# jurgisp/pydreamer

Hardware: AMD Instinct MI355X
Metric: grad-steps/sec (world-model+AC) at B=50,T=50,H=15, 64×64 obs, 1/2/4/8 GPU (higher is better)
Workload: dtype f32

## Files before the change

pydreamer_amd/csrc/common.h:

```cpp
#pragma once
#include <hip/hip_runtime.h>
#include <stdint.h>
#include <stddef.h>
#include "dreamer_hip.h"

int dm_fail(int code, const char* fmt, ...);

#define DM_MAX_DEVICES 16

#ifndef DM_CHAIN_SETPRIO
#define DM_CHAIN_SETPRIO 0
#endif
#define DM_CHAIN_PRIO() do { if (DM_CHAIN_SETPRIO > 0) __builtin_amdgcn_s_setprio(DM_CHAIN_SETPRIO); } while (0)
#define DM_LAUNCH_CHECK()                                                                      \
  do {                                                                                         \
    hipError_t e__ = hipGetLastError();                                                        \
    if (e__ != hipSuccess) return dm_fail(DM_E_HIP, "%s:%d: %s", __FILE__, __LINE__, hipGetErrorString(e__)); \
  } while (0)

#define DM_TRY(expr)                 \
  do {                               \
    int rc__ = (expr);               \
    if (rc__ != DM_OK) return rc__;  \
  } while (0)

#define DM_REQUIRE(cond, code, ...)                     \
  do {                                                  \
    if (!(cond)) return dm_fail(code, __VA_ARGS__);     \
  } while (0)

static inline int dm_cdiv(int64_t a, int64_t b) { return (int)((a + b - 1) / b); }
static inline size_t dm_align_up(size_t x, size_t a) { return (x + a - 1) / a * a; }

struct DmArena {
  float* base;
  size_t cap;
  size_t off;
  bool ok;
  DmArena(void* p, size_t bytes) : base((float*)p), cap(bytes / sizeof(float)), off(0), ok(true) {}
  float* take(size_t nfloats) {
    size_t n = dm_align_up(nfloats, 64);
    if (base == nullptr || off + n > cap) { ok = false; off += n; return nullptr; }
    float* r = base + off;
    off += n;
    return r;
  }
};

hipStream_t dm_wgrad_side_stream(hipStream_t st);
int dm_wgrad_side_fork(hipStream_t st, hipStream_t sw);
int dm_wgrad_side_mark(hipStream_t sw, hipStream_t st);

int dm_cur_precision();
struct DmPrecisionScope {
  int prev;
  explicit DmPrecisionScope(int p);
  ~DmPrecisionScope();
};

struct DmTwinScope {
  bool active, opened;
  explicit DmTwinScope(bool bf16_mode);
  ~DmTwinScope();
};
bool dm_twins_on();
void dm_twin_add(const float* base, size_t n, unsigned short* twin, bool valid);
void dm_twin_mark(const float* p);
unsigned short* dm_twin_of(const float* p, bool need_valid);
void dm_twin_arena_note(const void* acts, bool written);
bool dm_twin_arena_valid(const void* acts);
struct DmCvtSeg { const float* src; unsigned short* dst; size_t n; };
int dm_to_bf16_multi_launch(const DmCvtSeg* segs, int count, hipStream_t st);
static inline size_t dm_half_floats(size_t elems) { return (elems + 1) / 2; }
constexpr int DM_HSTORE_MIN_K = 1024;
constexpr int DM_HSTORE_MIN_K_DENSE = 400;

struct DmGatesBwd;
struct DmGemm {
  int bf16 = dm_cur_precision();
  int a_layout = 0, b_layout = 0;
  int M = 0, N = 0, K = 0;
  const float* A = nullptr; int lda = 0;
  const float* B = nullptr; int ldb = 0;
  float* C = nullptr; int ldc = 0;
  const float* bias = nullptr;
  const float* add = nullptr; int ldadd = 0;
  const float* mulref = nullptr; int ldmul = 0;
  const uint8_t* row_zero = nullptr;
  const int* a_maj = nullptr; const int* a_min = nullptr; int a_tab_vec = 0;
  const int* b_maj = nullptr; const int* b_min = nullptr; int b_tab_vec = 0;
  int a_tab_vec8 = 0, b_tab_vec8 = 0;
  int flags = 0;
  const int2* c_tab = nullptr; int sc_cout = 0, sc_wpitch = 0;
  int bias_mod = 0;
  const float* ln_g = nullptr; const float* ln_b = nullptr; float ln_eps = 1e-3f;
  const float* lnb_x = nullptr; int lnb_ldx = 0; const float* lnb_stats = nullptr;
  const float* eg_x = nullptr; int eg_ldx = 0; const float* eg_stats = nullptr; const float* eg_gamma = nullptr; const float* eg_beta = nullptr;
  float* eg_G = nullptr; int eg_ldg = 0; float* eg_Gf = nullptr; float* eg_ps = nullptr;
  const float* lnf_ps = nullptr; int lnf_nps = 0; const float* lnf_stats = nullptr;
  const float* lnf_xw = nullptr; int lnf_ldxw = 0; const float* lnf_cs = nullptr;
  const float* sm_logits = nullptr; int sm_ld = 0; float* sm_dlogits = nullptr; int sm_ldd = 0;
  const struct DmGatesBwd* gates = nullptr;
  const float* A_frag = nullptr;
  float* C_frag = nullptr;
  const unsigned short* A_h = nullptr;
  const unsigned short* B_h = nullptr;
  unsigned short* C_h = nullptr;
  bool no_twin = false;
};
__host__ __device__ __forceinline__ size_t dm_frag_off(int row, int k) {
  return ((((size_t)(k >> 4) * 4 + (row >> 4)) * 4 + ((k >> 2) & 3)) * 16 + (row & 15)) * 4 + (k & 3);
}
static inline size_t dm_frag_floats(int K) { return (size_t)dm_cdiv(K, 16) * 1024; }
int dm_frag_pack_launch(int rows, int K, const float* X, int ldx, float* Xf, hipStream_t st);
struct DmRssmLds {
  int B, D, Hd, S, C, F, t_begin, t_end;
  const float *wzt, *zb, *wih, *bih, *whh, *bhh, *wph, *bph, *wpo, *bpo, *in_g, *in_b, *post_g, *post_b, *ea, *ee;
  const uint8_t* reset; const float* u; const int32_t* forced;
  float *x1, *gi, *gh, *hin, *zin, *feat, *x2, *post; int32_t* idx;
  float* ws; size_t ws_floats;
};
bool dm_rssm_lds_ok(int B, int D, int Hd, int S, int C);
size_t dm_rssm_lds_ws_floats(int B, int D, int Hd, int S, int C, int steps);
int dm_rssm_lds_launch(const DmRssmLds& q, hipStream_t st);
extern "C" int dm_rssm_lds_enable(int on);
bool dm_z_embed_ok(int n);
int dm_sparse_rows_launch(int rows, int n, int Zc, const float* z, int ldz, const float* Wt, float* x, int ldx,
                          hipStream_t st);
int dm_z_embed_launch(int rows, int n, int S, int C, const int32_t* idx, const uint8_t* row_zero, const float* Wt,
                      const float* bias, const float* add, int ldadd, const int32_t* idx2, const float* Wt2, float* x, int ldx,
                      float* x_frag, const float* gamma, const float* beta, float eps, float* y, int ldy, hipStream_t st,
                      float* y_frag = nullptr, float* stats = nullptr);
struct DmGatesBwd {
  const float* gi; const float* gh; const float* h_in; int ldh, D;
  float* dgi; float* dgh; float* dprev; int ldp; const uint8_t* row_zero;
  float* dgi_frag = nullptr; float* dgh_frag = nullptr;
};
struct DmSample {
  const float* u = nullptr; const int32_t* forced = nullptr;
  float* onehot = nullptr; int ldo = 0;
  int32_t* idx = nullptr;
  float* z_next = nullptr; const uint8_t* next_reset = nullptr;
  float* z_next_frag = nullptr;
};
bool dm_skinny_ln_ok(int M, int N, int K);
int dm_gemm_sample_launch(const DmGemm& q, const DmSample& sm, hipStream_t stream);
int dm_gemm_launch(const DmGemm& g, void* ws, size_t ws_bytes, hipStream_t stream);
int dm_gemm_skinny_try(const DmGemm& g, hipStream_t stream);
int dm_gemm_pair_launch(const DmGemm& g0, const DmGemm& g1, void* ws, size_t ws_bytes, hipStream_t stream);

int dm_colsum_launch(int rows, int n, const float* x, int ld, float* out, void* ws, size_t ws_bytes, hipStream_t st);
int dm_elu_fwd_launch(int rows, int n, const float* x, int ldx, float* y, int ldy, hipStream_t st);
int dm_elu_bwd_launch(int rows, int n, const float* y, int ldy, const float* dy, int lddy, float* dx, int lddx,
                      hipStream_t st);
int dm_ln_elu_fwd_launch(int rows, int n, const float* x, int ldx, const float* gamma, const float* beta, float eps,
                         float* y, int ldy, float* stats, hipStream_t st);
int dm_ln_elu_bwd_dx_launch(int rows, int n, const float* x, int ldx, const float* y, int ldy, const float* stats,
                            const float* gamma, const float* dy, int lddy, float* dx, int lddx, hipStream_t st);
int dm_ln_elu_bwd_params_launch(int rows, int n, const float* x, int ldx, const float* y, int ldy, const float* stats,
                                const float* dy, int lddy, float* dgamma, float* dbeta, void* ws, size_t ws_bytes,
                                hipStream_t st);
int dm_gru_norm_fwd_launch(int kind, int rows, int D, const float* gi, const float* gh, const float* h_in, int ldh,
                           const float* const* ln_g, const float* const* ln_b, float* h_out, int ldo, float* gs, float* gst,
                           float* h_next, const uint8_t* next_reset, hipStream_t st, int ldg = 0, int ldst = 0, int ldn = 0);
int dm_gru_norm_bwd_launch(int kind, int rows, int D, const float* gh, const float* h_in, int ldh, const float* gs,
                           const float* gst, const float* const* ln_g, const float* const* ln_b, const float* dh_out, int lddh,
                           float* dgi, float* dgh, float* dg, float* dh_in, int lddi, const uint8_t* row_zero, hipStream_t st,
                           int ldg = 0, int ldst = 0);
int dm_gru_norm_param_grads_launch(int kind, int rows, int D, const float* gs, const float* gst, const float* dg, float* dgam,
                                   float* dbet, hipStream_t st, int ldg = 0, int ldst = 0);
int dm_gru_gates_fwd_launch(int rows, int D, const float* gi, const float* gh, const float* h_in, int ldh, float* h_out,
                            int ldo, float* h_next, const uint8_t* next_reset, float* h_frag, float* h_next_frag,
                            hipStream_t st, int ldg = 0, int ldn = 0);
int dm_gru_gates_bwd_launch(int rows, int D, const float* gi, const float* gh, const float* h_in, int ldh,
                            const float* dh_out, int lddh, float* dgi, float* dgh, float* dh_in, int lddi, int accum,
                            const uint8_t* row_zero, hipStream_t st, int ldg = 0);
int dm_sample_onehot_launch(int rows, int groups, int C, const float* logits, int ldl, const float* u,
                            const int32_t* forced, float* onehot, int ldo, int32_t* idx, float* z_next,
                            const uint8_t* next_reset, hipStream_t st);
int dm_gauss_sample_bwd_launch(int rows, int S, const float* par, int ldp, const float* z, int ldz, const float* dz,
                               int lddz, float* dpar, int lddp, int accum, hipStream_t st);
int dm_kl_fwd_launch(int rows, int S, int C, const float* post, const float* prior, float* kl, float* ep, float* eq,
                     hipStream_t st);
int dm_kl_bwd_launch(int rows, int S, int C, const float* post, const float* prior, float sp, float sq, float* dpost,
                     float* dprior, hipStream_t st);
int dm_st_softmax_bwd_launch(int rows, int groups, int C, const float* logits, int ldl, const float* dz, int lddz,
                             float* dlogits, int lddl, int accum, hipStream_t st);
int dm_mask_rows_launch(int rows, int n, const float* x, int ldx, const uint8_t* reset, float* y, int ldy, hipStream_t st);
int dm_mask_rows2_launch(int rows, int n1, const float* x1, int ldx1, float* y1, int ldy1, int n2, const float* x2,
                         int ldx2, float* y2, int ldy2, const uint8_t* reset, hipStream_t st);
int dm_sample_continuous_launch(int kind, int rows, int A, const float* params, const float* eps, float* action,
                                hipStream_t st);
int dm_mul_elu_grad_launch(size_t n, const float* dy, const float* yact, float* out, hipStream_t st);

int dm_im2col_s2_launch(int n, int hb, int wb, int c, int k, const float* big, int big_nchw, float* col, hipStream_t st);
int dm_col2im_s2_launch(int n, int hb, int wb, int c, int k, const float* col, const float* bias, int flags,
                        const float* elu_ref, float* big, hipStream_t st);
int dm_permute4_launch(const float* src, float* dst, int d0, int d1, int d2, int d3, int p0, int p1, int p2, int p3,
                       hipStream_t st);

bool dm_enc_l1_direct_ok(int ch, int d, int img);
int dm_enc_l1_fwd_launch(int frames, int d, int u8, const void* image, const float* w, const float* bias, float* wt, float* y,
                         unsigned short* y_h, hipStream_t st);
size_t dm_enc_l1_wgrad_part_floats(int frames, int d);
int dm_enc_l1_wgrad_launch(int frames, int d, int u8, const void* image, const float* G, float* part, float* dW, void* ws,
                           size_t ws_bytes, hipStream_t st);
bool dm_dec_l4_direct_ok(int ch, int d, int hs, int k);
size_t dm_dec_l4_w4_floats(int d);
int dm_dec_l4_fwd_launch(int frames, int d, const float* x, const float* w, const float* bias, float* w4, float* out,
                         hipStream_t st);
bool dm_dec_l4_bwd_direct_ok(int ch, int d, int hs, int k);
size_t dm_dec_l4_wp_floats(int d);
size_t dm_dec_l4_wgrad_part_floats(int frames, int d);
int dm_dec_l4_dgrad_launch(int frames, int d, const float* G4, const float* w, float* wp, const float* x3, float* dx,
                           unsigned short* dx_h, hipStream_t st);
int dm_dec_l4_wgrad_launch(int frames, int d, const float* G4, const float* x3, float* part, float* dW, void* ws,
                           size_t ws_bytes, hipStream_t st);

struct DmChainSample {
  const float* u;
  float* onehot;
  int ldo;
  int32_t* idx;
};
int dm_mlp_fwd_launch(int rows, int in_dim, int hidden, int layers, int out_dim, const float* x, int ldx,
                      const dm_mlp_params* p, float* acts, int acts_total_rows, int acts_row_off, float* out, int ldout,
                      void* ws, size_t ws_bytes, hipStream_t st, const float* chain_wpack = nullptr, int sparse_cols = 0,
                      const float* chain_add0 = nullptr, const DmChainSample* chain_sample = nullptr);

bool dm_panel_ok(int rows, int hidden);
int dm_panel_count(int rows);
int dm_panel_ln_fwd_launch(int rows, int hidden, int kin, const float* x, int ldx, const float* W, const float* b,
                           const float* gamma, const float* beta, float eps, float* xpre, float* stats, float* y,
                           const float* wout, const float* bout, float* out, int out_dim, int ldout, hipStream_t st,
// ... 51 lines not shown
```

pydreamer_amd/csrc/conv.hip:

```cpp
#include "common.h"
#include <stdlib.h>

template <int VEC>
__global__ void __launch_bounds__(256) im2col_s2_nhwc_kernel(int n, int hb, int wb, int c, int k, int hs, int ws,
                                                             const float* __restrict__ big, float* __restrict__ col) {
  const int cv = c / VEC;
  const size_t total = (size_t)n * hs * ws * k * k * cv;
  for (size_t e = (size_t)blockIdx.x * 256 + threadIdx.x; e < total; e += (size_t)gridDim.x * 256) {
    size_t t = e;
    const int c4 = (int)(t % cv); t /= cv;
    const int kx = (int)(t % k); t /= k;
    const int ky = (int)(t % k); t /= k;
    const int xs = (int)(t % ws); t /= ws;
    const int ys = (int)(t % hs); t /= hs;
    const int i = (int)t;
    const size_t src = (((size_t)i * hb + (2 * ys + ky)) * wb + (2 * xs + kx)) * c + (size_t)c4 * VEC;
    if constexpr (VEC == 4) {
      reinterpret_cast<float4*>(col)[e] = *reinterpret_cast<const float4*>(big + src);
    } else {
      col[e] = big[src];
    }
  }
}

// ... 457 lines not shown
        hipLaunchKernelGGL(im2col_s2_u8hwc_kernel, dim3(grid_for(total)), dim3(256), 0, st, g.N, g.hb[0], g.hb[0], g.cin[0], 4,
                           g.hs[0], g.hs[0], (const uint8_t*)image, a.xcol[0]);
        DM_LAUNCH_CHECK();
      } else {
        DM_TRY(dm_im2col_s2_launch(g.N, g.hb[0], g.hb[0], g.cin[0], 4, image, 1, a.xcol[0], st));
      }
    }
    DmGemm q;
    q.a_layout = 0; q.b_layout = 0;
    q.M = g.N * g.hs[l] * g.hs[l]; q.N = g.cout[l]; q.K = (int)g.kdim[l];
    if (l == 0) { q.A = a.xcol[0]; q.lda = q.K; }
    else {
      q.A = a.y[l - 1]; q.a_maj = a.rowoff[l]; q.a_min = a.koff[l];
      q.a_tab_vec = (g.cin[l] & 3) == 0; q.a_tab_vec8 = (g.cin[l] & 7) == 0;
    }
    q.B = l == 0 ? p->w[0] : a.wr[l]; q.ldb = q.K;
    q.C = a.y[l]; q.ldc = q.N;
    q.bias = p->b[l];
    q.flags = DM_GEMM_ELU;
    DM_TRY(dm_gemm_launch(q, ws, DM_SPLITK_FLOATS * sizeof(float), st));
  }
  const size_t tot = (size_t)g.N * 4 * g.cout[3];
  hipLaunchKernelGGL(nhwc_to_chw_flat_kernel, dim3(grid_for(tot)), dim3(256), 0, st, (size_t)g.N, 4, g.cout[3], a.y[3], embed, 1);
  DM_LAUNCH_CHECK();
  return DM_OK;
}

extern "C" int dm_conv_encoder_bwd(const dm_shape* shp, const float* image, const dm_conv_params* p, const float* acts,
                                   const float* dembed, const dm_conv_grads* gr, void* ws, size_t ws_bytes, void* stream) {
  DM_REQUIRE(shp && p && acts && dembed && gr && ws, DM_E_NULL, "conv_encoder_bwd: null pointer");
  DmPrecisionScope prec(shp->flags & DM_FLAG_BF16);
  EncGeom g(shp);
  DM_REQUIRE(g.valid(shp), DM_E_SHAPE, "conv_encoder: unsupported geometry");
  hipStream_t st = (hipStream_t)stream;
  EncActs a;
  enc_carve(g, const_cast<float*>(acts), (size_t)1 << 60, &a);
  DmArena ar(ws, ws_bytes);
  float* splitk = ar.take(DM_SPLITK_FLOATS);
  const size_t gmax = g.rows[0] * g.cout[0];
  float* ga = ar.take(gmax);
  float* gb = ar.take(g.rows[1] * g.cout[1]);
  float* dwr = ar.take((size_t)g.cout[3] * g.kdim[3]);
  size_t xcmax = 0;
  for (int l = 1; l < 4; ++l) if (g.rows[l] * g.kdim[l] > xcmax) xcmax = g.rows[l] * g.kdim[l];
  float* dxcol = ar.take(xcmax);
  size_t padmax = 0, tabmax = 0, wcmax = 0;
  for (int l = 1; l < 4; ++l)
    if (convt_gather_ok(4, g.cout[l], g.cin[l], g.hs[l], (size_t)g.N)) {
      const size_t hp = g.hs[l] + 2, Hc = g.hs[l] + 1;
      if ((size_t)g.N * hp * hp * g.cout[l] > padmax) padmax = (size_t)g.N * hp * hp * g.cout[l];
      if ((size_t)g.N * Hc * Hc > tabmax) tabmax = (size_t)g.N * Hc * Hc;
      if ((size_t)16 * g.cin[l] * g.cout[l] > wcmax) wcmax = (size_t)16 * g.cin[l] * g.cout[l];
    }
  float* gpad = ar.take(padmax);
  int* t_rowoff = (int*)ar.take(tabmax);
  int2* t_ctab = (int2*)ar.take(2 * tabmax);
  int* t_koff = (int*)ar.take(wcmax ? 4 * 1024 : 0);
  float* wcat = ar.take(wcmax);
  DmTwinScope tw((shp->flags & DM_FLAG_BF16) != 0);
  const bool tw_on = dm_twins_on();
  unsigned short* ga_h = (unsigned short*)ar.take(tw_on ? dm_half_floats(gmax) : 0);
  unsigned short* gb_h = (unsigned short*)ar.take(tw_on ? dm_half_floats(g.rows[1] * g.cout[1]) : 0);
  unsigned short* wcat_h = (unsigned short*)ar.take(tw_on ? dm_half_floats(wcmax) : 0);
  DM_REQUIRE(ar.ok, DM_E_WORKSPACE, "conv_encoder_bwd: workspace too small (need %zu floats)", ar.off);
  const size_t skb = DM_SPLITK_FLOATS * sizeof(float);
  const bool arena_tw = dm_twin_arena_valid(acts);
  enc_register_twins(g, a, arena_tw, arena_tw);
  dm_twin_add(ga, gmax, ga_h, false);
  dm_twin_add(gb, g.rows[1] * g.cout[1], gb_h, false);

  float* G = gb;
  const size_t tot3 = (size_t)g.N * 4 * g.cout[3];
  hipLaunchKernelGGL(nhwc_to_chw_flat_kernel, dim3(grid_for(tot3)), dim3(256), 0, st, (size_t)g.N, 4, g.cout[3], dembed, G,
                     0);
  DM_LAUNCH_CHECK();
  DM_TRY(dm_mul_elu_grad_launch(tot3, G, a.y[3], G, st));
  if (tw_on) {
    const DmCvtSeg sg = {G, dm_twin_of(G, false), tot3};
    DM_TRY(dm_to_bf16_multi_launch(&sg, 1, st));
    dm_twin_mark(G);
  }
  for (int l = 3; l >= 0; --l) {
    const int rows = (int)g.rows[l], co = g.cout[l], kd = (int)g.kdim[l];
    DM_TRY(dm_colsum_launch(rows, co, G, co, gr->b[l], splitk, skb, st));
    if (l == 0 && g.direct0) {
      DM_REQUIRE(image, DM_E_NULL, "conv_encoder_bwd: the direct layer-1 weight gradient reads the image");
      DM_REQUIRE(dm_enc_l1_wgrad_part_floats(g.N, g.d) <= xcmax, DM_E_WORKSPACE, "conv_encoder_bwd: partial buffer too small");
      DM_TRY(dm_enc_l1_wgrad_launch(g.N, g.d, shape_u8(shp) ? 1 : 0, image, G, dxcol, gr->w[0], splitk, skb, st));
      continue;
    }
    DmGemm q;
    q.a_layout = 1; q.b_layout = 1;
    q.M = co; q.N = kd; q.K = rows;
    q.A = G; q.lda = co;
    if (l == 0) { q.B = a.xcol[0]; q.ldb = kd; }
    else {
      q.B = a.y[l - 1]; q.b_maj = a.rowoff[l]; q.b_min = a.koff[l];
      q.b_tab_vec = (g.cin[l] & 3) == 0; q.b_tab_vec8 = (g.cin[l] & 7) == 0;
    }
    q.C = (l == 0) ? gr->w[0] : dwr; q.ldc = kd;
    DM_TRY(dm_gemm_launch(q, splitk, skb, st));
    if (l > 0 && convt_gather_ok(4, co, g.cin[l], g.hs[l], (size_t)g.N)) {
      DM_TRY(dm_permute4_launch(dwr, gr->w[l], co, 4, 4, g.cin[l], 0, 3, 1, 2, st));
      const int hs = g.hs[l], hb = g.hb[l], Hc = hs + 1, kdim4 = 4 * co, ci = g.cin[l];
      DM_REQUIRE(kdim4 <= 4 * 1024, DM_E_SHAPE, "conv_encoder_bwd: gather-form K %d exceeds the offset table", kdim4);
      float* Gn = (G == ga) ? gb : ga;
      if (l == 1) Gn = ga;
      const size_t padn = (size_t)g.N * (hs + 2) * (hs + 2) * (co / 4);
      const bool hpath = tw_on && (co & 7) == 0 && kdim4 >= DM_HSTORE_MIN_K;
      if (hpath) hipLaunchKernelGGL(convt_pad_h_kernel, dim3(grid_for(padn)), dim3(256), 0, st, g.N, hs, hs, co / 4, 1, (const float4*)G,
                                    (uint2*)gpad);
      else hipLaunchKernelGGL(convt_pad_kernel, dim3(grid_for(padn)), dim3(256), 0, st, g.N, hs, hs, co / 4, 1, (const float4*)G,
                              (float4*)gpad);
      DM_LAUNCH_CHECK();
      hipLaunchKernelGGL(convt_tables_kernel, dim3(grid_for((size_t)g.N * Hc * Hc + kdim4)), dim3(256), 0, st, g.N, hs, hs, co, 2,
                         hb, hb, ci, t_rowoff, t_koff, t_ctab);
      DM_LAUNCH_CHECK();
      hipLaunchKernelGGL(convt_repack_kernel, dim3(grid_for((size_t)4 * ci * kdim4)), dim3(256), 0, st, co, ci, 4, p->w[l], wcat);
      DM_LAUNCH_CHECK();
      if (hpath) {
        const DmCvtSeg sg = {wcat, wcat_h, (size_t)4 * ci * kdim4};
        DM_TRY(dm_to_bf16_multi_launch(&sg, 1, st));
      }
      if (2 * Hc != hb) {
        hipError_t e = hipMemsetAsync(Gn, 0, (size_t)g.N * hb * hb * ci * sizeof(float), st);
        if (e == hipSuccess && dm_twin_of(Gn, false))
          e = hipMemsetAsync(dm_twin_of(Gn, false), 0, (size_t)g.N * hb * hb * ci * sizeof(unsigned short), st);
        if (e != hipSuccess) return dm_fail(DM_E_HIP, "conv_encoder_bwd: %s", hipGetErrorString(e));
      }
      DmGemm d;
      d.M = g.N * Hc * Hc; d.N = 4 * ci; d.K = kdim4;
      d.A = gpad; d.a_maj = t_rowoff; d.a_min = t_koff; d.a_tab_vec = 1; d.a_tab_vec8 = 1;
      if (hpath) { d.A = nullptr; d.A_h = (const unsigned short*)gpad; d.B_h = wcat_h; }
      d.B = wcat; d.ldb = kdim4;
      d.C = Gn;
      d.c_tab = t_ctab; d.sc_cout = ci; d.sc_wpitch = hb * ci;
      d.mulref = a.y[l - 1];
      d.no_twin = l == 1;
      DM_TRY(dm_gemm_launch(d, splitk, skb, st));
      G = Gn;
    } else if (l > 0) {
      DM_TRY(dm_permute4_launch(dwr, gr->w[l], co, 4, 4, g.cin[l], 0, 3, 1, 2, st));
      DmGemm d;
      d.a_layout = 0; d.b_layout = 1;
      d.M = rows; d.N = kd; d.K = co;
      d.A = G; d.lda = co;
      d.B = a.wr[l]; d.ldb = kd;
      d.C = dxcol; d.ldc = kd;
      DM_TRY(dm_gemm_launch(d, splitk, skb, st));
      float* Gn = (G == ga) ? gb : ga;
      if (l == 1) Gn = ga;
      DM_TRY(dm_col2im_s2_launch(g.N, g.hb[l], g.hb[l], g.cin[l], 4, dxcol, nullptr, 0, a.y[l - 1], Gn, st));
      G = Gn;
    }
  }
  return DM_OK;
}

__global__ void __launch_bounds__(256) convt_pad_cout_kernel(int I, int O, int O4, int k, const float* __restrict__ src,
                                                             float* __restrict__ dst) {
  const int total = I * k * k * O4;
  for (int e = blockIdx.x * 256 + threadIdx.x; e < total; e += gridDim.x * 256) {
    const int o = e % O4, kx = (e / O4) % k, ky = (e / (O4 * k)) % k, i = e / (O4 * k * k);
    dst[e] = o < O ? src[(((size_t)i * O + o) * k + ky) * k + kx] : 0.f;
  }
}
__global__ void __launch_bounds__(256) convt_unpad_cout_kernel(int I, int O, int O4, int k, const float* __restrict__ src,
                                                               float* __restrict__ dst) {
  const int total = I * O * k * k;
  for (int e = blockIdx.x * 256 + threadIdx.x; e < total; e += gridDim.x * 256) {
    const int kx = e % k, ky = (e / k) % k, o = (e / (k * k)) % O, i = e / (k * k * O);
    dst[e] = src[(((size_t)i * k + ky) * k + kx) * O4 + o];
  }
}

struct DecActs {
  float* wr[5];
// ... 236 lines not shown
  float* G = Gl[4];
  DM_TRY(mse_launch(shape_u8(shp), g.N, g.hbg[4] * g.hbg[4], g.ch, a.x[4], (const void*)target, shp->I > 0 ? shp->I : 1, scale,
                    row_scale, nullptr, G, co4[4], nullptr, st));
  for (int l = 4; l >= 1; --l) {
    const int kk = g.k[l] * g.k[l];
    const int co = co4[l];
    const bool padded = co != g.cout[l];
    const int ncol = kk * co;
    const int rows_s = (int)g.rows_s[l];
    int* rowoff = rowoff_l[l];
    int* koff = koff_l[l];
    float* Gn = Gl[l - 1];
    if (direct4 && l == 4) {
      DM_TRY(dm_wgrad_side_fork(st, sw));
      unsigned short* gnh = dm_twin_of(Gn, false);
      DM_TRY(dm_dec_l4_dgrad_launch(g.N, g.d, G, p->w[4], l4_wp, a.x[3], Gn, gnh, st));
      if (gnh) dm_twin_mark(Gn);
      DM_TRY(dm_colsum_launch((int)g.rows_b[l], co, G, co, bsum, splitk_w, skb, sw));
      hipError_t e = hipMemcpyAsync(gr->b[l], bsum, (size_t)g.cout[l] * sizeof(float), hipMemcpyDeviceToDevice, sw);
      if (e != hipSuccess) return dm_fail(DM_E_HIP, "conv_decoder_bwd: %s", hipGetErrorString(e));
      DM_TRY(dm_dec_l4_wgrad_launch(g.N, g.d, G, a.x[3], l4_part, gr->w[4], splitk_w, skb, sw));
      G = Gn;
      continue;
    }
    DM_TRY(conv_tables_launch(g.N, g.hbg[l], g.hbg[l], co, g.k[l], rowoff, koff, st));
    DM_TRY(dm_wgrad_side_fork(st, sw));
    if (padded) {
      hipLaunchKernelGGL(convt_pad_cout_kernel, dim3(grid_for((size_t)g.cin[l] * ncol)), dim3(256), 0, st, g.cin[l], g.cout[l], co,
                         g.k[l], p->w[l], wpad);
      DM_LAUNCH_CHECK();
      if (tw_on) {
        const DmCvtSeg sg = {wpad, wpad_h, (size_t)g.cin[l] * ncol};
        DM_TRY(dm_to_bf16_multi_launch(&sg, 1, st));
        dm_twin_mark(wpad);
      }
    }
    {
      DmGemm d;
      d.a_layout = 0; d.b_layout = 0;
      d.M = rows_s; d.N = g.cin[l]; d.K = ncol;
      d.A = G; d.a_maj = rowoff; d.a_min = koff; d.a_tab_vec = 1;
      d.a_tab_vec8 = (co & 7) == 0 || (co == 4 && (g.k[l] & 1) == 0);
      d.B = padded ? wpad : a.wr[l]; d.ldb = ncol;
      d.C = Gn; d.ldc = g.cin[l];
      if (l - 1 >= 1) { d.mulref = a.x[l - 1]; d.ldmul = g.cin[l]; }
      DM_TRY(dm_gemm_launch(d, splitk, skb, st));
    }
    if (padded) {
      DM_TRY(dm_colsum_launch((int)g.rows_b[l], co, G, co, bsum, splitk_w, skb, sw));
      hipError_t e = hipMemcpyAsync(gr->b[l], bsum, (size_t)g.cout[l] * sizeof(float), hipMemcpyDeviceToDevice, sw);
      if (e != hipSuccess) return dm_fail(DM_E_HIP, "conv_decoder_bwd: %s", hipGetErrorString(e));
    } else {
      DM_TRY(dm_colsum_launch((int)g.rows_b[l], co, G, co, gr->b[l], splitk_w, skb, sw));
    }
    DmGemm q;
    q.a_layout = 1; q.b_layout = 1;
    q.M = g.cin[l]; q.N = ncol; q.K = rows_s;
    q.A = a.x[l - 1]; q.lda = g.cin[l];
    q.B = G; q.b_maj = rowoff; q.b_min = koff; q.b_tab_vec = 1;
    q.b_tab_vec8 = (co & 7) == 0 || (co == 4 && (g.k[l] & 1) == 0);
    q.C = dwr; q.ldc = ncol;
    DM_TRY(dm_gemm_launch(q, splitk_w, skb, sw));
    if (padded) {
      hipLaunchKernelGGL(convt_unpad_cout_kernel, dim3(grid_for((size_t)g.cin[l] * kk * g.cout[l])), dim3(256), 0, sw, g.cin[l],
                         g.cout[l], co, g.k[l], dwr, gr->w[l]);
      DM_LAUNCH_CHECK();
    } else {
      DM_TRY(dm_permute4_launch(dwr, gr->w[l], g.cin[l], g.k[l], g.k[l], g.cout[l], 0, 3, 1, 2, sw));
    }
    G = Gn;
  }
  const int O = g.cin[1];
  DM_TRY(dm_wgrad_side_fork(st, sw));
  if (dfeat) {
    DmGemm d;
    d.a_layout = 0; d.b_layout = 1;
    d.M = g.N; d.N = g.F; d.K = O;
    d.A = G; d.lda = O;
    d.B = p->w[0]; d.ldb = g.F;
    d.C = dfeat; d.ldc = lddf;
    d.flags = DM_GEMM_ACCUM;
    DM_TRY(dm_gemm_launch(d, splitk, skb, st));
  }
  DM_TRY(dm_colsum_launch(g.N, O, G, O, gr->b[0], splitk_w, skb, sw));
  {
    DmGemm q;
    q.a_layout = 1; q.b_layout = 1;
    q.M = O; q.N = g.F; q.K = g.N;
    q.A = G; q.lda = O;
    q.B = feat; q.ldb = ldf;
    q.C = gr->w[0]; q.ldc = g.F;
    DM_TRY(dm_gemm_launch(q, splitk_w, skb, sw));
  }
  DM_TRY(dm_wgrad_side_mark(sw, st));
  return DM_OK;
}
```

pydreamer_amd/csrc/elementwise.hip:

```cpp
#include "common.h"

template <bool CACHE>
__global__ void __launch_bounds__(256) ln_elu_fwd_kernel(int rows, int n, const float* __restrict__ x, int ldx,
                                                         const float* __restrict__ gamma, const float* __restrict__ beta,
                                                         float eps, float* __restrict__ y, int ldy, float* __restrict__ stats,
                                                         unsigned short* __restrict__ y_h) {
  const int row = blockIdx.x * 4 + (threadIdx.x >> 6);
  const int lane = threadIdx.x & 63;
  if (row >= rows) return;
  const float* xr = x + (size_t)row * ldx;
  unsigned short* yh = y_h ? y_h + (size_t)row * ldy : nullptr;
  float xc[16];
  float s = 0.f;
  if (CACHE) {
#pragma unroll
    for (int j = 0; j < 16; ++j) {
      const int c = lane + 64 * j;
      xc[j] = c < n ? xr[c] : 0.f;
      s += xc[j];
    }
  } else {
    for (int c = lane; c < n; c += 64) s += xr[c];
  }
  const float mean = dm_wave_sum(s) / (float)n;
// ... 84 lines not shown
    for (int c = lane; c < n; c += 64) {
      const float g = dyr[c] * dm_elu_grad_from_y(yr[c]) * gamma[c];
      const float xh = (xr[c] - mean) * rstd;
      dxr[c] = rstd * (g - sg - xh * sgx);
    }
  }
}

template <int MODE>
__global__ void __launch_bounds__(256) colsum_partial_kernel(int rows, int n, int rows_per_chunk,
                                                             const float* __restrict__ x, int ldx,
                                                             const float* __restrict__ y, int ldy,
                                                             const float* __restrict__ stats,
                                                             const float* __restrict__ dy, int lddy,
                                                             float* __restrict__ partial) {
  __shared__ float red[2][4][64];
  const int cx = threadIdx.x & 63, ry = threadIdx.x >> 6;
  const int col = blockIdx.x * 64 + cx;
  const int chunk = blockIdx.y;
  const int r0 = chunk * rows_per_chunk;
  const int r1 = min(rows, r0 + rows_per_chunk);
  float a0 = 0.f, a1 = 0.f;
  if (col < n) {
    if (MODE == 0) {
      float b0 = 0.f, b1 = 0.f, b2 = 0.f, b3 = 0.f;
      int r = r0 + ry;
      for (; r + 12 < r1; r += 16) {
        b0 += x[(size_t)r * ldx + col];
        b1 += x[(size_t)(r + 4) * ldx + col];
        b2 += x[(size_t)(r + 8) * ldx + col];
        b3 += x[(size_t)(r + 12) * ldx + col];
      }
      for (; r < r1; r += 4) b0 += x[(size_t)r * ldx + col];
      a0 = (b0 + b1) + (b2 + b3);
    } else {
      for (int r = r0 + ry; r < r1; r += 4) {
        const float dl = dy[(size_t)r * lddy + col] * dm_elu_grad_from_y(y[(size_t)r * ldy + col]);
        const float xh = (x[(size_t)r * ldx + col] - stats[2 * r]) * stats[2 * r + 1];
        a0 += dl * xh;
        a1 += dl;
      }
    }
  }
  red[0][ry][cx] = a0;
  red[1][ry][cx] = a1;
  __syncthreads();
  if (ry == 0 && col < n) {
    const int nq = (MODE == 0) ? 1 : 2;
    float s0 = red[0][0][cx] + red[0][1][cx] + red[0][2][cx] + red[0][3][cx];
    partial[((size_t)chunk * nq + 0) * n + col] = s0;
    if (MODE == 1) {
      float s1 = red[1][0][cx] + red[1][1][cx] + red[1][2][cx] + red[1][3][cx];
      partial[((size_t)chunk * nq + 1) * n + col] = s1;
    }
  }
}

__global__ void __launch_bounds__(256) colsum_flat_kernel(long long total, int n, int W, long long chunk_elems,
                                                          const float* __restrict__ x, float* __restrict__ partial) {
  __shared__ float sh[256];
  const long long base = (long long)blockIdx.x * chunk_elems;
  const long long end = min(total, base + chunk_elems);
  float b0 = 0.f, b1 = 0.f, b2 = 0.f, b3 = 0.f;
  if ((int)threadIdx.x < W) {
    long long i = base + threadIdx.x;
    for (; i + 3LL * W < end; i += 4LL * W) {
      b0 += x[i];
      b1 += x[i + W];
      b2 += x[i + 2LL * W];
      b3 += x[i + 3LL * W];
    }
    for (; i < end; i += W) b0 += x[i];
  }
  sh[threadIdx.x] = (b0 + b1) + (b2 + b3);
  __syncthreads();
  if ((int)threadIdx.x < n) {
    float s = 0.f;
    for (int t = threadIdx.x; t < W; t += n) s += sh[t];
    partial[(size_t)blockIdx.x * n + threadIdx.x] = s;
  }
}

__global__ void __launch_bounds__(256) colsum_final_kernel(int n, int chunks, int nq, const float* __restrict__ partial,
                                                           float* __restrict__ out0, float* __restrict__ out1) {
  __shared__ float red[8][32];
  const int cx = threadIdx.x & 31, cy = threadIdx.x >> 5;
  const int col = blockIdx.x * 32 + cx;
  for (int q = 0; q < nq; ++q) {
    float s = 0.f;
    if (col < n) {
      const float* p = partial + (size_t)q * n + col;
      const size_t st = (size_t)nq * n;
      int c = cy;
      for (; c + 24 < chunks; c += 32) {
        const float v0 = p[(size_t)c * st], v1 = p[(size_t)(c + 8) * st], v2 = p[(size_t)(c + 16) * st], v3 = p[(size_t)(c + 24) * st];
        s += v0; s += v1; s += v2; s += v3;
      }
      for (; c < chunks; c += 8) s += p[(size_t)c * st];
    }
    red[cy][cx] = s;
    __syncthreads();
    if (cy == 0 && col < n) {
      float t = 0.f;
#pragma unroll
      for (int k = 0; k < 8; ++k) t += red[k][cx];
      (q == 0 ? out0 : out1)[col] = t;
    }
    __syncthreads();
  }
}

static int colsum_plan(int rows, size_t budget_floats, int n, int nq, int* rows_per_chunk) {
  int chunks = dm_cdiv(rows, 64);
  if (chunks > 1024) chunks = 1024;
  const size_t per = (size_t)n * nq;
  if (per > 0 && (size_t)chunks * per > budget_floats) chunks = (int)(budget_floats / per);
  if (chunks < 1) chunks = 1;
  *rows_per_chunk = dm_cdiv(rows, chunks);
  return dm_cdiv(rows, *rows_per_chunk);
}

int dm_colsum_launch(int rows, int n, const float* x, int ld, float* out, void* ws, size_t ws_bytes, hipStream_t st) {
  if (n <= 0) return DM_OK;
  if (rows <= 0) {
    (void)hipMemsetAsync(out, 0, (size_t)n * sizeof(float), st);
    return DM_OK;
  }
  DM_REQUIRE(ws && ws_bytes >= (size_t)n * sizeof(float), DM_E_WORKSPACE, "colsum: workspace too small");
  const size_t budget = ws_bytes / sizeof(float);
  int chunks;
  if (n <= 64 && ld == n && (long long)rows * n >= (1 << 16)) {
    const long long total = (long long)rows * n;
    const int W = 256 - 256 % n;
    long long want = total / ((long long)W * 16);
    if (want > 2048) want = 2048;
    if (want < 1) want = 1;
    if ((size_t)want * n > budget) want = (long long)(budget / n);
    long long chunk_elems = (total + want - 1) / want;
    chunk_elems = (chunk_elems + W - 1) / W * W;
    chunks = (int)((total + chunk_elems - 1) / chunk_elems);
    hipLaunchKernelGGL(colsum_flat_kernel, dim3(chunks), dim3(256), 0, st, total, n, W, chunk_elems, x, (float*)ws);
  } else {
    int rpc;
    chunks = colsum_plan(rows, budget, n, 1, &rpc);
    hipLaunchKernelGGL((colsum_partial_kernel<0>), dim3(dm_cdiv(n, 64), chunks), dim3(256), 0, st, rows, n, rpc, x, ld,
                       nullptr, 0, nullptr, nullptr, 0, (float*)ws);
  }
  DM_LAUNCH_CHECK();
  hipLaunchKernelGGL(colsum_final_kernel, dim3(dm_cdiv(n, 32)), dim3(256), 0, st, n, chunks, 1, (const float*)ws, out,
                     nullptr);
  DM_LAUNCH_CHECK();
  return DM_OK;
}

int dm_ln_elu_fwd_launch(int rows, int n, const float* x, int ldx, const float* gamma, const float* beta, float eps,
                         float* y, int ldy, float* stats, hipStream_t st) {
  if (rows <= 0) return DM_OK;
  unsigned short* y_h = dm_twin_of(y, false);
  if (y_h) dm_twin_mark(y);
  if (n <= 1024)
    hipLaunchKernelGGL((ln_elu_fwd_kernel<true>), dim3(dm_cdiv(rows, 4)), dim3(256), 0, st, rows, n, x, ldx, gamma, beta,
                       eps, y, ldy, stats, y_h);
  else
    hipLaunchKernelGGL((ln_elu_fwd_kernel<false>), dim3(dm_cdiv(rows, 4)), dim3(256), 0, st, rows, n, x, ldx, gamma, beta,
                       eps, y, ldy, stats, y_h);
  DM_LAUNCH_CHECK();
  return DM_OK;
}

__global__ void __launch_bounds__(256) elu_fwd_kernel(int rows, int n, const float* __restrict__ x, int ldx,
                                                      float* __restrict__ y, int ldy) {
  const size_t total = (size_t)rows * n;
  for (size_t i = (size_t)blockIdx.x * 256 + threadIdx.x; i < total; i += (size_t)gridDim.x * 256) {
    const size_t r = i / n, c = i % n;
    y[r * ldy + c] = dm_elu(x[r * ldx + c]);
  }
}
__global__ void __launch_bounds__(256) elu_bwd_kernel(int rows, int n, const float* __restrict__ y, int ldy,
                                                      const float* __restrict__ dy, int lddy, float* __restrict__ dx,
                                                      int lddx) {
  const size_t total = (size_t)rows * n;
  for (size_t i = (size_t)blockIdx.x * 256 + threadIdx.x; i < total; i += (size_t)gridDim.x * 256) {
    const size_t r = i / n, c = i % n;
    dx[r * lddx + c] = dy[r * lddy + c] * dm_elu_grad_from_y(y[r * ldy + c]);
  }
}
int dm_elu_fwd_launch(int rows, int n, const float* x, int ldx, float* y, int ldy, hipStream_t st) {
  if (rows <= 0) return DM_OK;
  const size_t total = (size_t)rows * n;
  hipLaunchKernelGGL(elu_fwd_kernel, dim3((unsigned)((total + 255) / 256 < 65536 ? (total + 255) / 256 : 65536)), dim3(256), 0,
                     st, rows, n, x, ldx, y, ldy);
  DM_LAUNCH_CHECK();
  return DM_OK;
}
int dm_elu_bwd_launch(int rows, int n, const float* y, int ldy, const float* dy, int lddy, float* dx, int lddx,
                      hipStream_t st) {
  if (rows <= 0) return DM_OK;
  const size_t total = (size_t)rows * n;
  hipLaunchKernelGGL(elu_bwd_kernel, dim3((unsigned)((total + 255) / 256 < 65536 ? (total + 255) / 256 : 65536)), dim3(256), 0,
                     st, rows, n, y, ldy, dy, lddy, dx, lddx);
  DM_LAUNCH_CHECK();
  return DM_OK;
}

int dm_ln_elu_bwd_dx_launch(int rows, int n, const float* x, int ldx, const float* y, int ldy, const float* stats,
                            const float* gamma, const float* dy, int lddy, float* dx, int lddx, hipStream_t st) {
  if (rows <= 0) return DM_OK;
  if (n <= 1024)
    hipLaunchKernelGGL((ln_elu_bwd_dx_kernel<true>), dim3(dm_cdiv(rows, 4)), dim3(256), 0, st, rows, n, x, ldx, y, ldy,
                       stats, gamma, dy, lddy, dx, lddx);
  else
    hipLaunchKernelGGL((ln_elu_bwd_dx_kernel<false>), dim3(dm_cdiv(rows, 4)), dim3(256), 0, st, rows, n, x, ldx, y, ldy,
                       stats, gamma, dy, lddy, dx, lddx);
  DM_LAUNCH_CHECK();
  return DM_OK;
}

int dm_ln_elu_bwd_params_launch(int rows, int n, const float* x, int ldx, const float* y, int ldy, const float* stats,
                                const float* dy, int lddy, float* dgamma, float* dbeta, void* ws, size_t ws_bytes,
                                hipStream_t st) {
  int rpc;
  DM_REQUIRE(ws && ws_bytes >= (size_t)2 * n * sizeof(float), DM_E_WORKSPACE, "ln_bwd: workspace too small");
  const int chunks = colsum_plan(rows, ws_bytes / sizeof(float), n, 2, &rpc);
  hipLaunchKernelGGL((colsum_partial_kernel<1>), dim3(dm_cdiv(n, 64), chunks), dim3(256), 0, st, rows, n, rpc, x, ldx, y,
                     ldy, stats, dy, lddy, (float*)ws);
  DM_LAUNCH_CHECK();
  hipLaunchKernelGGL(colsum_final_kernel, dim3(dm_cdiv(n, 32)), dim3(256), 0, st, n, chunks, 2, (const float*)ws, dgamma,
                     dbeta);
  DM_LAUNCH_CHECK();
  return DM_OK;
}

extern "C" int dm_ln_elu_fwd(int rows, int n, const float* x, int ldx, const float* gamma, const float* beta, float eps,
                             float* y, int ldy, float* stats, void* stream) {
  DM_REQUIRE(x && gamma && beta && y && stats, DM_E_NULL, "ln_elu_fwd: null pointer");
  return dm_ln_elu_fwd_launch(rows, n, x, ldx, gamma, beta, eps, y, ldy, stats, (hipStream_t)stream);
}

extern "C" int dm_ln_elu_bwd(int rows, int n, const float* x, int ldx, const float* y, int ldy, const float* stats,
                             const float* gamma, const float* dy, int lddy, float* dx, int lddx, float* dgamma,
                             float* dbeta, void* ws, size_t ws_bytes, void* stream) {
  DM_REQUIRE(x && y && stats && gamma && dy && dx && dgamma && dbeta, DM_E_NULL, "ln_elu_bwd: null pointer");
  DM_TRY(dm_ln_elu_bwd_dx_launch(rows, n, x, ldx, y, ldy, stats, gamma, dy, lddy, dx, lddx, (hipStream_t)stream));
  return dm_ln_elu_bwd_params_launch(rows, n, x, ldx, y, ldy, stats, dy, lddy, dgamma, dbeta, ws, ws_bytes,
                                     (hipStream_t)stream);
}

extern "C" int dm_colsum(int rows, int n, const float* x, int ld, float* out, void* ws, size_t ws_bytes, void* stream) {
  DM_REQUIRE(x && out, DM_E_NULL, "colsum: null pointer");
  return dm_colsum_launch(rows, n, x, ld, out, ws, ws_bytes, (hipStream_t)stream);
}

__device__ __forceinline__ float dm_sigmoid(float v) { return 1.0f / (1.0f + expf(-v)); }

__global__ void __launch_bounds__(256) gru_gates_fwd_kernel(int rows, int D, const float* __restrict__ gi,
                                                            const float* __restrict__ gh, const float* __restrict__ h_in,
                                                            int ldh, float* __restrict__ h_out, int ldo,
                                                            float* __restrict__ h_next,
                                                            const uint8_t* __restrict__ next_reset,
                                                            float* __restrict__ h_frag, float* __restrict__ h_next_frag,
                                                            int ldg, int ldn, unsigned short* __restrict__ h_out_h) {
  const size_t total = (size_t)rows * D;
  for (size_t i = (size_t)blockIdx.x * 256 + threadIdx.x; i < total; i += (size_t)gridDim.x * 256) {
    const int r = (int)(i / D), d = (int)(i % D);
    const float* gir = gi + (size_t)r * ldg;
    const float* ghr = gh + (size_t)r * ldg;
    const float rg = dm_sigmoid(gir[d] + ghr[d]);
    const float ug = dm_sigmoid(gir[D + d] + ghr[D + d]);
    const float ng = tanhf(gir[2 * D + d] + rg * ghr[2 * D + d]);
    const float h = h_in[(size_t)r * ldh + d];
    const float ho = (h - ng) * ug + ng;
    h_out[(size_t)r * ldo + d] = ho;
    if (h_out_h) h_out_h[(size_t)r * ldo + d] = (unsigned short)dm_f2bf(ho);
    const float hn = (next_reset && next_reset[r]) ? 0.f : ho;
    if (h_next) h_next[(size_t)r * ldn + d] = hn;
    if (h_frag) h_frag[dm_frag_off(r, d)] = ho;
    if (h_next_frag) h_next_frag[dm_frag_off(r, d)] = hn;
  }
}
__global__ void __launch_bounds__(256) frag_pack_kernel(int rows, int K, const float* __restrict__ X, int ldx,
                                                        float* __restrict__ Xf) {
  const int total = rows * K;
  for (int i = blockIdx.x * 256 + threadIdx.x; i < total; i += gridDim.x * 256) {
    const int r = i / K, k = i % K;
    Xf[dm_frag_off(r, k)] = X[(size_t)r * ldx + k];
  }
}

__global__ void __launch_bounds__(256) gru_gates_bwd_kernel(int rows, int D, const float* __restrict__ gi,
                                                            const float* __restrict__ gh, const float* __restrict__ h_in,
                                                            int ldh, const float* __restrict__ dh_out, int lddh,
                                                            float* __restrict__ dgi, float* __restrict__ dgh,
                                                            float* __restrict__ dh_in, int lddi, int accum,
                                                            const uint8_t* __restrict__ row_zero, int ldg) {
  const size_t total = (size_t)rows * D;
  for (size_t i = (size_t)blockIdx.x * 256 + threadIdx.x; i < total; i += (size_t)gridDim.x * 256) {
    const int r = (int)(i / D), d = (int)(i % D);
    const size_t g0 = (size_t)r * ldg;
    const float ghn = gh[g0 + 2 * D + d];
    const float rg = dm_sigmoid(gi[g0 + d] + gh[g0 + d]);
    const float ug = dm_sigmoid(gi[g0 + D + d] + gh[g0 + D + d]);
    const float ng = tanhf(gi[g0 + 2 * D + d] + rg * ghn);
    const float h = h_in[(size_t)r * ldh + d];
    const float dh = dh_out[(size_t)r * lddh + d];
    const float dn = dh * (1.f - ug);
    const float du = dh * (h - ng);
    const float dpn = dn * (1.f - ng * ng);
    const float dpr = dpn * ghn * rg * (1.f - rg);
    const float dpu = du * ug * (1.f - ug);
    dgi[g0 + d] = dpr;
    dgi[g0 + D + d] = dpu;
// ... 1566 lines not shown
```

pydreamer_amd/csrc/gemm.hip:

```cpp
#include "common.h"
#include "dma_loop.h"
#include <stdlib.h>
#include <math.h>
#include <type_traits>
#include <mutex>
#include <atomic>


struct GemmKArgs {
  const float* A;
  const float* B;
  float* C;
  const float* bias;
  const float* add;
  const float* mulref;
  const uint8_t* row_zero;
  const int* a_maj; const int* a_min;
  const int* b_maj; const int* b_min;
  float* partial;
  const int2* c_tab;
  int sc_cout, sc_wpitch;
  int bias_mod;
  int M, N, K;
  int lda, ldb, ldc, ldadd, ldmul;
  int flags;
  int k_per_split;
  int nsplit;
  int tiles_m;
  int n_tiles, n_items;
  int tiles_n, n_fast;
  int n_groups;
  int a_vec, b_vec;
  unsigned short* Ch;
  int use_dma;
};

template <int ROWS, int LAYOUT, int NF4, bool GATHER, bool VEC, bool KSEQ = false>
__device__ __forceinline__ void gemm_load_tile(float4 (&r)[NF4], const float* __restrict__ P, int ld, int row0,
                                               int nrows, int k0, int kend, const int* __restrict__ tmaj,
                                               const int* __restrict__ tmin, int tid, unsigned& mask) {
  mask = 0u;
#pragma unroll
  for (int i = 0; i < NF4; ++i) {
    const int f = tid + i * 256;
    int major, minor, major_end, minor_end;
    if (LAYOUT == 0) {
      major = row0 + (f >> 3);
      minor = k0 + ((f & 7) << 2);
      major_end = nrows;
      minor_end = kend;
    } else {
      constexpr int F4_PER_K = ROWS / 4;
      if (KSEQ) {
        major = k0 + (tid / F4_PER_K) * NF4 + i;
        minor = row0 + ((tid % F4_PER_K) << 2);
      } else {
        major = k0 + f / F4_PER_K;
        minor = row0 + ((f % F4_PER_K) << 2);
      }
      major_end = kend;
      minor_end = nrows;
    }
    const bool okm = major < major_end;
    const int mj = okm ? major : 0;
    float4 v;
    if (VEC) {
      const bool ok = okm && minor < minor_end;
      const int mn = ok ? minor : 0;
      const size_t off = GATHER ? (size_t)(tmaj[mj] + tmin[mn]) : (size_t)mj * ld + mn;
      v = *reinterpret_cast<const float4*>(P + (ok ? off : 0));
      mask |= ok ? (0xFu << (4 * i)) : 0u;
    } else {
      float e[4];
#pragma unroll
      for (int j = 0; j < 4; ++j) {
        const bool ok = okm && minor + j < minor_end;
        const int mn = ok ? minor + j : 0;
        const size_t off = GATHER ? (size_t)(tmaj[mj] + tmin[mn]) : (size_t)mj * ld + mn;
        e[j] = P[ok ? off : 0];
        mask |= ok ? (1u << (4 * i + j)) : 0u;
      }
      v = make_float4(e[0], e[1], e[2], e[3]);
    }
    r[i] = v;
  }
}

template <int ROWS, int LAYOUT, int NF4>
__device__ __forceinline__ void gemm_store_tile(const float4 (&rr)[NF4], unsigned mask, float* S, int tid) {
  constexpr int LDK = 36;
  constexpr int LDM = ROWS + 4;
  float4 r[NF4];
#pragma unroll
  for (int i = 0; i < NF4; ++i) {
    r[i].x = (mask >> (4 * i + 0)) & 1u ? rr[i].x : 0.f;
    r[i].y = (mask >> (4 * i + 1)) & 1u ? rr[i].y : 0.f;
    r[i].z = (mask >> (4 * i + 2)) & 1u ? rr[i].z : 0.f;
    r[i].w = (mask >> (4 * i + 3)) & 1u ? rr[i].w : 0.f;
  }
#pragma unroll
  for (int i = 0; i < NF4; ++i) {
    const int f = tid + i * 256;
    if (LAYOUT == 0) {
      const int row = f >> 3;
      const int kq = (f & 7) << 2;
      *reinterpret_cast<float4*>(&S[row * LDK + kq]) = r[i];
    } else {
      constexpr int F4_PER_K = ROWS / 4;
      const int kr = f / F4_PER_K;
      const int r4 = (f % F4_PER_K) << 2;
      *reinterpret_cast<float4*>(&S[kr * LDM + r4]) = r[i];
    }
  }
}

constexpr int LDKB = 40;
template <int ROWS, int LAYOUT, int NF4, bool KSEQ = false>
// ... 84 lines not shown
    it.n0 = fast * BN;
    it.m0 = slow * BM;
  } else {
    it.m0 = fast * BM;
    it.n0 = slow * BN;
  }
  it.kbeg = it.split * g.k_per_split;
  it.kend = min(g.K, it.kbeg + g.k_per_split);
  it.nkt = (it.kend > it.kbeg) ? (it.kend - it.kbeg + 31) / 32 : 0;
  return it;
}

constexpr int EPI_STAGE_LD = 40;
template <int BM, int BN, int WGM, int WGN, bool SC, int MB, int NB>
__device__ __forceinline__ void gemm_epilogue(f32x16 (&acc)[MB][NB], const GemmKArgs& g, const GemmItem& cur, int wm, int wn,
                                              int l31, int half, unsigned short* stage = nullptr) {
  const bool staged = !SC && stage && g.Ch && g.nsplit <= 1 && (g.ldc & 7) == 0 && (((uintptr_t)g.Ch) & 15) == 0;
#pragma unroll
  for (int mb = 0; mb < MB; ++mb) {
#pragma unroll
    for (int nb = 0; nb < NB; ++nb) {
      const int col = cur.n0 + wn * (BN / WGN) + nb * 32 + l31;
      int sc_off = 0, sc_need = 0, sc_o = 0;
      if (SC) {
        const int cls = col / g.sc_cout;
        sc_o = col - cls * g.sc_cout;
        sc_off = (cls >> 1) * g.sc_wpitch + (cls & 1) * g.sc_cout + sc_o;
        sc_need = cls;
      }
#pragma unroll
      for (int r = 0; r < 16; ++r) {
        const int row = cur.m0 + wm * (BM / WGM) + mb * 32 + (r & 3) + 8 * (r >> 2) + 4 * half;
        if (row < g.M && col < g.N) {
          float v = acc[mb][nb][r];
          if (SC) {
            const int2 ct = g.c_tab[row];
            if ((sc_need & ~ct.y) == 0) {
              const size_t at = (size_t)ct.x + sc_off;
              if (g.bias) v += g.bias[sc_o];
              if (g.flags & DM_GEMM_ELU) v = dm_elu(v);
              if (g.mulref) v *= dm_elu_grad_from_y(g.mulref[at]);
              g.C[at] = v;
              if (g.Ch) g.Ch[at] = (unsigned short)dm_f2bf(v);
            }
          } else if (g.nsplit > 1) {
            g.partial[((size_t)cur.split * g.M + row) * g.N + col] = v;
          } else {
            if (g.row_zero && g.row_zero[row]) v = 0.f;
            if (g.bias) v += g.bias[g.bias_mod > 0 ? col % g.bias_mod : col];
            if (g.add) v += g.add[(size_t)row * g.ldadd + col];
            float* c = g.C + (size_t)row * g.ldc + col;
            if (g.flags & DM_GEMM_ACCUM) v += *c;
            if (g.flags & DM_GEMM_ELU) v = dm_elu(v);
            if (g.mulref) v *= dm_elu_grad_from_y(g.mulref[(size_t)row * g.ldmul + col]);
            *c = v;
            if (staged) stage[((r & 3) + 8 * (r >> 2) + 4 * half) * EPI_STAGE_LD + l31] = (unsigned short)dm_f2bf(v);
            else if (g.Ch) g.Ch[(size_t)row * g.ldc + col] = (unsigned short)dm_f2bf(v);
          }
        }
      }
      if (staged) {
        __builtin_amdgcn_wave_barrier();
        const int lane = half * 32 + l31;
        const int rl = lane >> 1, c0 = (lane & 1) * 16;
        const int row = cur.m0 + wm * (BM / WGM) + mb * 32 + rl;
        const int colb = cur.n0 + wn * (BN / WGN) + nb * 32 + c0;
        if (row < g.M) {
#pragma unroll
          for (int h8 = 0; h8 < 2; ++h8) {
            const int cc = colb + h8 * 8;
            const unsigned short* sp = &stage[rl * EPI_STAGE_LD + c0 + h8 * 8];
            unsigned short* dp = g.Ch + (size_t)row * g.ldc + cc;
            if (cc + 8 <= g.N) *reinterpret_cast<uint4*>(dp) = *reinterpret_cast<const uint4*>(sp);
            else
              for (int j = 0; j < 8 && cc + j < g.N; ++j) dp[j] = sp[j];
          }
        }
        __builtin_amdgcn_wave_barrier();
      }
    }
  }
}

template <int BM, int BN, int AL, int BL, bool VEC, bool GA = false, bool GB = false, int WGM = 2, int WGN = 2,
          int BF = 0, bool SC = false>
__global__ void __launch_bounds__(256) gemm_f32_kernel(const GemmKArgs g) {
  static_assert(WGM * WGN == 4 && BM % (32 * WGM) == 0 && BN % (32 * WGN) == 0, "wave grid must tile the block tile");
  constexpr int BK = 32;
  constexpr int LDK = 36;
  constexpr int LDMA = BM + 4, LDMB = BN + 4;
  constexpr int A_FLOATS = (AL == 0) ? BM * LDK : BK * LDMA;
  constexpr int B_FLOATS = (BL == 0) ? BN * LDK : BK * LDMB;
  constexpr int MB = BM / (32 * WGM), NB = BN / (32 * WGN);
  constexpr int A_F4 = BM * BK / 4 / 256, B_F4 = BN * BK / 4 / 256;
  constexpr bool A_KSEQ = BF != 0 && AL == 1 && 256 % (BM / 4) == 0, B_KSEQ = BF != 0 && BL == 1 && 256 % (BN / 4) == 0;
  constexpr int SMEM_FLOATS = A_FLOATS + B_FLOATS;
  __shared__ __attribute__((aligned(16))) float smem[SMEM_FLOATS];
  float* As = smem;
  float* Bs = smem + A_FLOATS;

  const int tid = threadIdx.x;
  const int lane = tid & 63;
  const int wave = tid >> 6;
  const int half = lane >> 5;
  const int l31 = lane & 31;
  const int wm = wave / WGN, wn = wave % WGN;

  const GemmItem cur = gemm_decode<BM, BN>(g, blockIdx.x);

  f32x16 acc[MB][NB];
#pragma unroll
  for (int i = 0; i < MB; ++i)
#pragma unroll
    for (int j = 0; j < NB; ++j)
#pragma unroll
      for (int r = 0; r < 16; ++r) acc[i][j][r] = 0.f;

  float4 ra[A_F4], rb[B_F4];
  unsigned ma = 0u, mb_ = 0u;
  if (cur.nkt > 0) {
    gemm_load_tile<BM, AL, A_F4, GA, VEC, A_KSEQ>(ra, g.A, g.lda, cur.m0, g.M, cur.kbeg, cur.kend, g.a_maj, g.a_min, tid, ma);
    gemm_load_tile<BN, BL, B_F4, GB, VEC, B_KSEQ>(rb, g.B, g.ldb, cur.n0, g.N, cur.kbeg, cur.kend, g.b_maj, g.b_min, tid, mb_);
  }
  for (int kt = 0; kt < cur.nkt; ++kt) {
    unsigned short* Ah = reinterpret_cast<unsigned short*>(smem);
    unsigned short* Bh = Ah + BM * LDKB;
    if (BF == 1) {
      gemm_store_tile_bf16<BM, AL, A_F4, A_KSEQ>(ra, ma, Ah, tid);
      gemm_store_tile_bf16<BN, BL, B_F4, B_KSEQ>(rb, mb_, Bh, tid);
    } else {
      gemm_store_tile<BM, AL, A_F4>(ra, ma, As, tid);
      gemm_store_tile<BN, BL, B_F4>(rb, mb_, Bs, tid);
    }
    __syncthreads();
    if (kt + 1 < cur.nkt) {
      const int k0 = cur.kbeg + (kt + 1) * BK;
      gemm_load_tile<BM, AL, A_F4, GA, VEC, A_KSEQ>(ra, g.A, g.lda, cur.m0, g.M, k0, cur.kend, g.a_maj, g.a_min, tid, ma);
      gemm_load_tile<BN, BL, B_F4, GB, VEC, B_KSEQ>(rb, g.B, g.ldb, cur.n0, g.N, k0, cur.kend, g.b_maj, g.b_min, tid, mb_);
    }
    __builtin_amdgcn_sched_barrier(0);
    if (BF == 1) {
#pragma unroll
      for (int ks = 0; ks < 2; ++ks) {
        bf16x8 a8[MB], b8[NB];
#pragma unroll
        for (int mb = 0; mb < MB; ++mb)
          a8[mb] = *reinterpret_cast<const bf16x8*>(&Ah[(wm * (BM / WGM) + mb * 32 + l31) * LDKB + ks * 16 + half * 8]);
#pragma unroll
        for (int nb = 0; nb < NB; ++nb)
          b8[nb] = *reinterpret_cast<const bf16x8*>(&Bh[(wn * (BN / WGN) + nb * 32 + l31) * LDKB + ks * 16 + half * 8]);
#pragma unroll
        for (int mb = 0; mb < MB; ++mb)
#pragma unroll
          for (int nb = 0; nb < NB; ++nb)
            acc[mb][nb] = __builtin_amdgcn_mfma_f32_32x32x16_bf16(a8[mb], b8[nb], acc[mb][nb], 0, 0, 0);
      }
    } else
#pragma unroll
    for (int kg = 0; kg < 4; ++kg) {
      float a[MB][4], b[NB][4];
#pragma unroll
      for (int mb = 0; mb < MB; ++mb) {
        const int row = wm * (BM / WGM) + mb * 32 + l31;
        if (AL == 0) {
          const float4 t = *reinterpret_cast<const float4*>(&As[row * LDK + kg * 8 + half * 4]);
          a[mb][0] = t.x; a[mb][1] = t.y; a[mb][2] = t.z; a[mb][3] = t.w;
        } else {
#pragma unroll
          for (int j = 0; j < 4; ++j) a[mb][j] = As[(kg * 8 + half * 4 + j) * LDMA + row];
        }
      }
#pragma unroll
      for (int nb = 0; nb < NB; ++nb) {
        const int row = wn * (BN / WGN) + nb * 32 + l31;
        if (BL == 0) {
          const float4 t = *reinterpret_cast<const float4*>(&Bs[row * LDK + kg * 8 + half * 4]);
          b[nb][0] = t.x; b[nb][1] = t.y; b[nb][2] = t.z; b[nb][3] = t.w;
        } else {
#pragma unroll
          for (int j = 0; j < 4; ++j) b[nb][j] = Bs[(kg * 8 + half * 4 + j) * LDMB + row];
        }
      }
#pragma unroll
      for (int j = 0; j < 4; ++j)
#pragma unroll
        for (int mb = 0; mb < MB; ++mb)
#pragma unroll
          for (int nb = 0; nb < NB; ++nb)
            acc[mb][nb] = __builtin_amdgcn_mfma_f32_32x32x2f32(a[mb][j], b[nb][j], acc[mb][nb], 0, 0, 0);
    }
    __syncthreads();
  }

  gemm_epilogue<BM, BN, WGM, WGN, SC, MB, NB>(acc, g, cur, wm, wn, l31, half,
                                              reinterpret_cast<unsigned short*>(smem) + wave * 32 * EPI_STAGE_LD);
}

template <int BM, int BN, int AL, int BL, bool GA, bool GB, int WGM, int WGN, bool SC, int NS>
__global__ void __launch_bounds__(256) gemm_dma_kernel(const GemmKArgs g) {
  static_assert(WGM * WGN == 4 && BM % (32 * WGM) == 0 && BN % (32 * WGN) == 0, "wave grid must tile the block tile");
  static_assert(NS >= 2 && NS <= 3, "two or three LDS stages");
  constexpr int WM = BM / WGM, WN = BN / WGN;
  constexpr int MB = WM / 32, NB = WN / 32;
  constexpr int A_BYTES = BM * 128, B_BYTES = BN * 128, STAGE = A_BYTES + B_BYTES;
  constexpr int RD = MB * DmaFrag<AL>::READS + NB * DmaFrag<BL>::READS;
  static_assert(RD <= 15, "lgkmcnt is a 4-bit counter");
  static_assert((AL == 0 || (MB - 1) * 32 + BM <= 255) && (BL == 0 || (NB - 1) * 32 + BN <= 255), "ds_read2_b32 offsets are 8 bits");
  extern __shared__ __attribute__((aligned(1024))) unsigned char dma_smem[];
  const unsigned lds0 = (unsigned)(size_t)(__attribute__((address_space(3))) unsigned char*)dma_smem;

  const int tid = threadIdx.x;
  const int lane = tid & 63, wave = tid >> 6, half = lane >> 5, l31 = lane & 31;
  const int wm = wave / WGN, wn = wave % WGN;
  const GemmItem cur = gemm_decode<BM, BN>(g, blockIdx.x);

  f32x16 acc[MB][NB];
#pragma unroll
  for (int i = 0; i < MB; ++i)
#pragma unroll
    for (int j = 0; j < NB; ++j)
#pragma unroll
      for (int r = 0; r < 16; ++r) acc[i][j][r] = 0.f;

  if (cur.nkt > 0) {
    DmaOperand<BM, AL, GA> sa;
    DmaOperand<BN, BL, GB> sb;
    sa.init(g.A, g.lda, cur.m0, g.M, g.a_maj, g.a_min, wave, lane);
    sb.init(g.B, g.ldb, cur.n0, g.N, g.b_maj, g.b_min, wave, lane);
    constexpr int NPT = DmaOperand<BM, AL, GA>::NP + DmaOperand<BN, BL, GB>::NP;

    const int swz = (l31 >> 1) & 7;
    unsigned fa[4], fb[4];
#pragma unroll
    for (int kg = 0; kg < 4; ++kg) {
      fa[kg] = AL == 0 ? lds0 + (wm * WM + l31) * 128 + (((2 * kg + half) ^ swz) << 4)
                       : lds0 + (((8 * kg + 4 * half) * BM + wm * WM + l31) << 2);
      fb[kg] = BL == 0 ? lds0 + A_BYTES + (wn * WN + l31) * 128 + (((2 * kg + half) ^ swz) << 4)
                       : lds0 + A_BYTES + (((8 * kg + 4 * half) * BN + wn * WN + l31) << 2);
    }
    auto read_frags = [&](DmaFrag<AL> (&a)[MB], DmaFrag<BL> (&b)[NB], int kg, unsigned so) {
#pragma unroll
      for (int mb = 0; mb < MB; ++mb) {
        if constexpr (AL == 0) {
          asm volatile("ds_read_b128 %0, %1 offset:%2" : "=v"(a[mb].v) : "v"(fa[kg] + so), "n"(mb * 32 * 128));
        } else {
          asm volatile("ds_read2_b32 %0, %1 offset0:%2 offset1:%3" : "=v"(a[mb].lo) : "v"(fa[kg] + so), "n"(mb * 32), "n"(mb * 32 + BM));
          asm volatile("ds_read2_b32 %0, %1 offset0:%2 offset1:%3" : "=v"(a[mb].hi) : "v"(fa[kg] + so + 8 * BM), "n"(mb * 32), "n"(mb * 32 + BM));
        }
      }
#pragma unroll
      for (int nb = 0; nb < NB; ++nb) {
        if constexpr (BL == 0) {
          asm volatile("ds_read_b128 %0, %1 offset:%2" : "=v"(b[nb].v) : "v"(fb[kg] + so), "n"(nb * 32 * 128));
        } else {
          asm volatile("ds_read2_b32 %0, %1 offset0:%2 offset1:%3" : "=v"(b[nb].lo) : "v"(fb[kg] + so), "n"(nb * 32), "n"(nb * 32 + BN));
          asm volatile("ds_read2_b32 %0, %1 offset0:%2 offset1:%3" : "=v"(b[nb].hi) : "v"(fb[kg] + so + 8 * BN), "n"(nb * 32), "n"(nb * 32 + BN));
        }
      }
    };

    static_assert(!(GA || GB) || NS == 2, "gathered operands take the two-stage ring");
    sa.fetch_tab(cur.kbeg, cur.kend);
    sb.fetch_tab(cur.kbeg, cur.kend);
#pragma unroll
    for (int s = 0; s < NS - 1; ++s) {
      if (s < cur.nkt) {
        sa.issue(cur.kbeg + s * 32, cur.kend, dma_smem + s * STAGE, wave);
        sb.issue(cur.kbeg + s * 32, cur.kend, dma_smem + s * STAGE + A_BYTES, wave);
      }
    }
    sa.fetch_tab(cur.kbeg + 32, cur.kend);
    sb.fetch_tab(cur.kbeg + 32, cur.kend);

    int stage = 0;
    for (int kt = 0; kt < cur.nkt; ++kt) {
      if (NS == 3 && kt + 1 < cur.nkt) dma_wait_vm<NPT>();
      else dma_wait_vm<0>();
      __builtin_amdgcn_s_barrier();
      const unsigned so = (unsigned)stage * STAGE;
      DmaFrag<AL> a[2][MB];
      DmaFrag<BL> b[2][NB];
      read_frags(a[0], b[0], 0, so);
      const int nt = kt + NS - 1;
      int ns = stage + NS - 1;
      if (ns >= NS) ns -= NS;
      if (nt < cur.nkt) {
        sa.issue(cur.kbeg + nt * 32, cur.kend, dma_smem + ns * STAGE, wave);
        sb.issue(cur.kbeg + nt * 32, cur.kend, dma_smem + ns * STAGE + A_BYTES, wave);
      }
#pragma unroll
      for (int kg = 0; kg < 4; ++kg) {
        const int c = kg & 1, n = c ^ 1;
        if (kg < 3) {
          read_frags(a[n], b[n], kg + 1, so);
          dma_wait_lgkm<RD>();
        } else dma_wait_lgkm<0>();
        __builtin_amdgcn_sched_barrier(0);
#pragma unroll
        for (int j = 0; j < 4; ++j)
#pragma unroll
          for (int mb = 0; mb < MB; ++mb)
#pragma unroll
            for (int nb = 0; nb < NB; ++nb)
              acc[mb][nb] = __builtin_amdgcn_mfma_f32_32x32x2f32(a[c][mb].get(j), b[c][nb].get(j), acc[mb][nb], 0, 0, 0);
        __builtin_amdgcn_sched_barrier(0);
      }
      if ((GA || GB) && nt + 1 < cur.nkt) {
        sa.fetch_tab(cur.kbeg + (nt + 1) * 32, cur.kend);
        sb.fetch_tab(cur.kbeg + (nt + 1) * 32, cur.kend);
      }
      if (++stage == NS) stage = 0;
    }
  }
  unsigned short* stg = nullptr;
  if (g.Ch) {
    __syncthreads();
    stg = reinterpret_cast<unsigned short*>(dma_smem) + wave * 32 * EPI_STAGE_LD;
  }
  gemm_epilogue<BM, BN, WGM, WGN, SC, MB, NB>(acc, g, cur, wm, wn, l31, half, stg);
}

template <int ROWS, int LAYOUT, int NF4, bool GATHER, bool KSEQ>
struct PipeOperand {
  const float* P;
  const int* tvar;
  int ld;
  int off[NF4];
  int kin[NF4];
  __device__ __forceinline__ void init(const float* P_, int ld_, int row0, int nrows, const int* tmaj, const int* tmin, int tid) {
    P = P_; ld = ld_;
    tvar = LAYOUT == 0 ? tmin : tmaj;
#pragma unroll
    for (int i = 0; i < NF4; ++i) {
      const int f = tid + i * 256;
      if (LAYOUT == 0) {
        const int row = min(row0 + (f >> 3), nrows - 1);
        kin[i] = (f & 7) << 2;
        off[i] = GATHER ? tmaj[row] : row * ld + kin[i];
      } else {
        constexpr int F4_PER_K = ROWS / 4;
        kin[i] = KSEQ ? (tid / F4_PER_K) * NF4 + i : f / F4_PER_K;
        const int col = min(row0 + (((KSEQ ? tid : f) % F4_PER_K) << 2), nrows - 4);
        off[i] = GATHER ? tmin[col] : kin[i] * ld + col;
      }
    }
  }
  __device__ __forceinline__ void load(float4 (&r)[NF4], int k0, int kend) const {
#pragma unroll
    for (int i = 0; i < NF4; ++i) {
      const bool ok = k0 + kin[i] < kend;
      size_t at;
      if (LAYOUT == 0) at = GATHER ? (size_t)off[i] + (size_t)tvar[ok ? k0 + kin[i] : 0] : (size_t)off[i] + (size_t)k0;
      else at = GATHER ? (size_t)off[i] + (size_t)tvar[ok ? k0 + kin[i] : 0] : (size_t)k0 * ld + (size_t)off[i];
      typedef float f32x4n __attribute__((ext_vector_type(4)));
      typedef const __attribute__((address_space(1))) f32x4n* gptr4;
      const uintptr_t src = ok ? (uintptr_t)(P + at) : (uintptr_t)dm_zero_page;
      const f32x4n v = *reinterpret_cast<gptr4>(src);
      r[i] = make_float4(v.x, v.y, v.z, v.w);
    }
  }
};

template <int ROWS, int LAYOUT, int NF4, bool KSEQ>
struct PipeStash {
  static constexpr bool ROWWISE = LAYOUT == 1 && KSEQ;
  static constexpr int UNITS = ROWWISE ? (NF4 == 4 ? 8 : 4) : 2 * NF4;
  static __device__ __forceinline__ float comp(const float4& v, int j) { return j == 0 ? v.x : j == 1 ? v.y : j == 2 ? v.z : v.w; }
  static __device__ __forceinline__ unsigned pack(float x, float y) { return dm_pack_bf16x2(x, y); }
  static __device__ __forceinline__ void unit(const float4 (&rr)[NF4], int u, unsigned short* S, int tid, unsigned& hold) {
    if (ROWWISE) {
      static_assert(!ROWWISE || NF4 == 4 || NF4 == 2, "row-wise packing covers 64- and 128-row operands");
      constexpr int F4_PER_K = ROWS / 4;
      const int kq = (tid / F4_PER_K) * NF4, r4 = (tid % F4_PER_K) << 2;
      if (NF4 == 4) {
        const int j = u >> 1;
        if ((u & 1) == 0) { hold = pack(comp(rr[0], j), comp(rr[1], j)); return; }
        const unsigned q = pack(comp(rr[NF4 > 2 ? 2 : 0], j), comp(rr[NF4 - 1], j));
        unsigned short* d = &S[(r4 + j) * LDKB + kq];
        *reinterpret_cast<uint2*>(d) = make_uint2(hold, q);
      } else {
        const unsigned q = pack(comp(rr[0], u), comp(rr[NF4 - 1], u));
        unsigned short* d = &S[(r4 + u) * LDKB + kq];
        *reinterpret_cast<unsigned*>(d) = q;
      }
      return;
    }
    const int i = u >> 1, f = tid + i * 256;
    if (LAYOUT == 0) {
      if ((u & 1) == 0) { hold = pack(rr[i].x, rr[i].y); return; }
      const unsigned q = pack(rr[i].z, rr[i].w);
      unsigned short* d = &S[(f >> 3) * LDKB + ((f & 7) << 2)];
      *reinterpret_cast<uint2*>(d) = make_uint2(hold, q);
    } else {
      constexpr int F4_PER_K = ROWS / 4;
      const int kr = f / F4_PER_K, r4 = ((f % F4_PER_K) << 2) + 2 * (u & 1);
      const unsigned q = (u & 1) ? pack(rr[i].z, rr[i].w) : pack(rr[i].x, rr[i].y);
// ... 201 lines not shown
};

template <int BM, int BN, int AL, int BL, bool GA, bool GB, int WGM, int WGN, bool SC>
__global__ void __launch_bounds__(256, 2) gemm_h_kernel(const GemmKArgs g) {
  static_assert(WGM * WGN == 4 && BM % (32 * WGM) == 0 && BN % (32 * WGN) == 0, "wave grid must tile the block tile");
  constexpr int BK = 64;
  constexpr int MB = BM / (32 * WGM), NB = BN / (32 * WGN);
  constexpr int SLOT = (BM + BN) * LDH;
  __shared__ __attribute__((aligned(16))) unsigned short smem[2 * SLOT];
  const int tid = threadIdx.x;
  const int lane = tid & 63, wave = tid >> 6, half = lane >> 5, l31 = lane & 31;
  const int wm = wave / WGN, wn = wave % WGN;
  const GemmItem cur = gemm_decode<BM, BN>(g, blockIdx.x);
  const int nkt = cur.kend > cur.kbeg ? (cur.kend - cur.kbeg + BK - 1) / BK : 0;

  f32x16 acc[MB][NB];
#pragma unroll
  for (int i = 0; i < MB; ++i)
#pragma unroll
    for (int j = 0; j < NB; ++j)
#pragma unroll
      for (int r = 0; r < 16; ++r) acc[i][j][r] = 0.f;

  if (nkt > 0) {
    typedef HOperand<BM, AL, GA> OA;
    typedef HOperand<BN, BL, GB> OB;
    OA sa;
    OB sb;
    sa.init(reinterpret_cast<const unsigned short*>(g.A), g.lda, cur.m0, g.M, g.a_maj, g.a_min, tid);
    sb.init(reinterpret_cast<const unsigned short*>(g.B), g.ldb, cur.n0, g.N, g.b_maj, g.b_min, tid);
    dm_u32x4 ra[OA::NCH], rb[OB::NCH];
    const bool nt = (g.flags & (1 << 20)) != 0;
    sa.load(ra, cur.kbeg, cur.kend, nt);
    sb.load(rb, cur.kbeg, cur.kend, nt);
    sa.stash(ra, smem, tid);
    sb.stash(rb, smem + BM * LDH, tid);
    if (nkt > 1) {
      sa.load(ra, cur.kbeg + BK, cur.kend, nt);
      sb.load(rb, cur.kbeg + BK, cur.kend, nt);
    }
    __syncthreads();
    for (int kt = 0; kt < nkt; ++kt) {
      const unsigned short* Ah = smem + (kt & 1) * SLOT;
      const unsigned short* Bh = Ah + BM * LDH;
      unsigned short* Aw = smem + ((kt & 1) ^ 1) * SLOT;
      unsigned short* Bw = Aw + BM * LDH;
#pragma unroll
      for (int ks = 0; ks < 4; ++ks) {
        bf16x8 a8[MB], b8[NB];
#pragma unroll
        for (int mb = 0; mb < MB; ++mb)
          a8[mb] = *reinterpret_cast<const bf16x8*>(&Ah[(wm * (BM / WGM) + mb * 32 + l31) * LDH +
                                                        hswz(wm * (BM / WGM) + mb * 32 + l31, ks * 16 + half * 8)]);
#pragma unroll
        for (int nb = 0; nb < NB; ++nb)
          b8[nb] = *reinterpret_cast<const bf16x8*>(&Bh[(wn * (BN / WGN) + nb * 32 + l31) * LDH +
                                                        hswz(wn * (BN / WGN) + nb * 32 + l31, ks * 16 + half * 8)]);
#pragma unroll
        for (int mb = 0; mb < MB; ++mb)
#pragma unroll
          for (int nb = 0; nb < NB; ++nb)
            acc[mb][nb] = __builtin_amdgcn_mfma_f32_32x32x16_bf16(a8[mb], b8[nb], acc[mb][nb], 0, 0, 0);
        if (ks == 1) {
          __builtin_amdgcn_sched_barrier(0);
          if (kt + 1 < nkt) {
            sa.stash(ra, Aw, tid);
            sb.stash(rb, Bw, tid);
          }
          if (kt + 2 < nkt) {
            sa.load(ra, cur.kbeg + (kt + 2) * BK, cur.kend, nt);
            sb.load(rb, cur.kbeg + (kt + 2) * BK, cur.kend, nt);
          }
          __builtin_amdgcn_sched_barrier(0);
        }
      }
      __syncthreads();
    }
  }
  gemm_epilogue<BM, BN, WGM, WGN, SC, MB, NB>(acc, g, cur, wm, wn, l31, half, smem + wave * 32 * EPI_STAGE_LD);
}

__global__ void __launch_bounds__(256) gemm_splitk_reduce_kernel(const GemmKArgs g) {
  const size_t total = (size_t)g.M * g.N;
  for (size_t i = (size_t)blockIdx.x * 256 + threadIdx.x; i < total; i += (size_t)gridDim.x * 256) {
    const int row = (int)(i / g.N);
    const int col = (int)(i % g.N);
    const float* __restrict__ pp = g.partial + i;
    float v = 0.f;
    int s = 0;
    for (; s + 8 <= g.nsplit; s += 8) {
      float t[8];
#pragma unroll
      for (int u = 0; u < 8; ++u) t[u] = pp[(size_t)(s + u) * total];
#pragma unroll
      for (int u = 0; u < 8; ++u) v += t[u];
    }
    for (; s < g.nsplit; ++s) v += pp[(size_t)s * total];
    if (g.row_zero && g.row_zero[row]) v = 0.f;
    if (g.bias) v += g.bias[g.bias_mod > 0 ? col % g.bias_mod : col];
    if (g.add) v += g.add[(size_t)row * g.ldadd + col];
    float* c = g.C + (size_t)row * g.ldc + col;
    if (g.flags & DM_GEMM_ACCUM) v += *c;
    if (g.flags & DM_GEMM_ELU) v = dm_elu(v);
    if (g.mulref) v *= dm_elu_grad_from_y(g.mulref[(size_t)row * g.ldmul + col]);
    *c = v;
    if (g.Ch) g.Ch[(size_t)row * g.ldc + col] = (unsigned short)dm_f2bf(v);
  }
}

#include <vector>
struct GemmProf {
  bool on = false;
  size_t cap = 0, n = 0;
  std::vector<hipEvent_t> ev;
  std::vector<long long> shape;
  std::vector<double> flops, bytes;
  std::vector<int> kind;
};
static GemmProf g_prof;
static int prof_before(int kind, double flops, double bytes, hipStream_t st) {
  if (!g_prof.on || g_prof.n >= g_prof.cap) return -1;
  const int slot = (int)g_prof.n++;
  g_prof.flops[slot] = flops;
  g_prof.bytes[slot] = bytes;
  g_prof.kind[slot] = kind;
  (void)hipEventRecord(g_prof.ev[2 * slot], st);
  return slot;
}
static void prof_after(int slot, hipStream_t st) {
  if (slot >= 0) (void)hipEventRecord(g_prof.ev[2 * slot + 1], st);
}
bool dm_prof_active() { return g_prof.on; }
int dm_prof_slot_begin(int kind, double flops, double bytes, hipStream_t st) { return prof_before(kind, flops, bytes, st); }
void dm_prof_slot_end(int slot, hipStream_t st) { prof_after(slot, st); }
extern "C" int dm_prof_begin(int max_launches) {
  DM_REQUIRE(max_launches > 0 && max_launches <= (1 << 20), DM_E_SHAPE, "prof_begin: max_launches %d", max_launches);
  if ((size_t)max_launches > g_prof.ev.size() / 2) {
    const size_t have = g_prof.ev.size();
    g_prof.ev.resize(2 * (size_t)max_launches);
    for (size_t i = have; i < g_prof.ev.size(); ++i)
      if (hipEventCreate(&g_prof.ev[i]) != hipSuccess) return dm_fail(DM_E_HIP, "prof_begin: hipEventCreate failed");
  }
  g_prof.flops.assign(max_launches, 0.0);
  g_prof.bytes.assign(max_launches, 0.0);
  g_prof.kind.assign(max_launches, 0);
  g_prof.shape.assign(5 * (size_t)max_launches, 0);
  g_prof.cap = max_launches;
  g_prof.n = 0;
  g_prof.on = true;
  return DM_OK;
}
extern "C" int dm_prof_rows(double* rows, int max_rows) {
  DM_REQUIRE(rows && max_rows > 0, DM_E_NULL, "prof_rows: null output");
  int n = 0;
  for (size_t i = 0; i < g_prof.n && n < max_rows; ++i, ++n) {
    if (hipEventSynchronize(g_prof.ev[2 * i + 1]) != hipSuccess) return dm_fail(DM_E_HIP, "prof_rows: event sync failed");
    float ms = 0.f;
    if (hipEventElapsedTime(&ms, g_prof.ev[2 * i], g_prof.ev[2 * i + 1]) != hipSuccess)
      return dm_fail(DM_E_HIP, "prof_rows: hipEventElapsedTime failed");
    double* r = rows + 8 * (size_t)n;
    r[0] = g_prof.kind[i];
    for (int j = 0; j < 5; ++j) r[1 + j] = (double)g_prof.shape[5 * i + j];
    r[6] = g_prof.flops[i]; r[7] = ms;
  }
  return n;
}
extern "C" int dm_prof_end(double* out, int nkinds) {
  DM_REQUIRE(out && nkinds >= 44, DM_E_SHAPE, "prof_end: need room for 44 kinds");
  g_prof.on = false;
  for (int i = 0; i < nkinds * 4; ++i) out[i] = 0.0;
  for (size_t i = 0; i < g_prof.n; ++i) {
    if (hipEventSynchronize(g_prof.ev[2 * i + 1]) != hipSuccess) return dm_fail(DM_E_HIP, "prof_end: event sync failed");
    float ms = 0.f;
    if (hipEventElapsedTime(&ms, g_prof.ev[2 * i], g_prof.ev[2 * i + 1]) != hipSuccess)
      return dm_fail(DM_E_HIP, "prof_end: hipEventElapsedTime failed");
    const int k = g_prof.kind[i];
    out[k * 4 + 0] += 1.0;
    out[k * 4 + 1] += g_prof.flops[i];
    out[k * 4 + 2] += ms;
    out[k * 4 + 3] += g_prof.bytes[i];
  }
  return (int)g_prof.n;
}

template <int BM, int BN, int WGM, int WGN>
static int gemm_pipe_dispatch(const GemmKArgs& a, int al, int bl, int gather, dim3 grid, hipStream_t stream) {
  if (a.c_tab) {
    if (gather != 1 || al != 0 || bl != 0) return dm_fail(DM_E_SHAPE, "gemm: the scatter epilogue is built for a gathered A, layout (0,0), 16-byte loads");
    hipLaunchKernelGGL((gemm_pipe_kernel<BM, BN, 0, 0, true, false, WGM, WGN, true>), grid, dim3(256), 0, stream, a);
  } else if (gather == 1) {
    if (al != 0 || bl != 0) return dm_fail(DM_E_SHAPE, "gemm: gathered A is built for layout (0,0) only");
    hipLaunchKernelGGL((gemm_pipe_kernel<BM, BN, 0, 0, true, false, WGM, WGN, false>), grid, dim3(256), 0, stream, a);
  } else if (gather == 2) {
    if (al != 1 || bl != 1) return dm_fail(DM_E_SHAPE, "gemm: gathered B is built for layout (1,1) only");
    hipLaunchKernelGGL((gemm_pipe_kernel<BM, BN, 1, 1, false, true, WGM, WGN, false>), grid, dim3(256), 0, stream, a);
  } else if (al == 0 && bl == 0) hipLaunchKernelGGL((gemm_pipe_kernel<BM, BN, 0, 0, false, false, WGM, WGN, false>), grid, dim3(256), 0, stream, a);
  else if (al == 0 && bl == 1) hipLaunchKernelGGL((gemm_pipe_kernel<BM, BN, 0, 1, false, false, WGM, WGN, false>), grid, dim3(256), 0, stream, a);
  else if (al == 1 && bl == 0) hipLaunchKernelGGL((gemm_pipe_kernel<BM, BN, 1, 0, false, false, WGM, WGN, false>), grid, dim3(256), 0, stream, a);
  else hipLaunchKernelGGL((gemm_pipe_kernel<BM, BN, 1, 1, false, false, WGM, WGN, false>), grid, dim3(256), 0, stream, a);
  return DM_OK;
}
static int gemm_pipe_tiles(int tc, const GemmKArgs& a, int al, int bl, int gather, dim3 grid, hipStream_t stream) {
  if (tc == 0) return gemm_pipe_dispatch<128, 128, 2, 2>(a, al, bl, gather, grid, stream);
  if (tc == 1) return gemm_pipe_dispatch<128, 64, 2, 2>(a, al, bl, gather, grid, stream);
  if (tc == 3) return gemm_pipe_dispatch<128, 96, 4, 1>(a, al, bl, gather, grid, stream);
  if (tc == 4) return gemm_pipe_dispatch<96, 128, 1, 4>(a, al, bl, gather, grid, stream);
  return gemm_pipe_dispatch<64, 64, 2, 2>(a, al, bl, gather, grid, stream);
}

template <int BM, int BN, int WGM, int WGN>
static int gemm_h_dispatch(const GemmKArgs& a, int al, int bl, int gather, dim3 grid, hipStream_t stream) {
  if (a.c_tab) {
    if (gather != 1 || al != 0 || bl != 0) return dm_fail(DM_E_SHAPE, "gemm: the scatter epilogue is built for a gathered A, layout (0,0)");
    hipLaunchKernelGGL((gemm_h_kernel<BM, BN, 0, 0, true, false, WGM, WGN, true>), grid, dim3(256), 0, stream, a);
  } else if (gather == 1) {
    if (al != 0 || bl != 0) return dm_fail(DM_E_SHAPE, "gemm: gathered A is built for layout (0,0) only");
    hipLaunchKernelGGL((gemm_h_kernel<BM, BN, 0, 0, true, false, WGM, WGN, false>), grid, dim3(256), 0, stream, a);
  } else if (gather == 2) {
    if (al != 1 || bl != 1) return dm_fail(DM_E_SHAPE, "gemm: gathered B is built for layout (1,1) only");
    hipLaunchKernelGGL((gemm_h_kernel<BM, BN, 1, 1, false, true, WGM, WGN, false>), grid, dim3(256), 0, stream, a);
  } else if (al == 0 && bl == 0) hipLaunchKernelGGL((gemm_h_kernel<BM, BN, 0, 0, false, false, WGM, WGN, false>), grid, dim3(256), 0, stream, a);
  else if (al == 0 && bl == 1) hipLaunchKernelGGL((gemm_h_kernel<BM, BN, 0, 1, false, false, WGM, WGN, false>), grid, dim3(256), 0, stream, a);
  else if (al == 1 && bl == 0) hipLaunchKernelGGL((gemm_h_kernel<BM, BN, 1, 0, false, false, WGM, WGN, false>), grid, dim3(256), 0, stream, a);
  else hipLaunchKernelGGL((gemm_h_kernel<BM, BN, 1, 1, false, false, WGM, WGN, false>), grid, dim3(256), 0, stream, a);
  return DM_OK;
}
static int gemm_h_tiles(int tc, const GemmKArgs& a, int al, int bl, int gather, dim3 grid, hipStream_t stream) {
  if (tc == 0) return gemm_h_dispatch<128, 128, 2, 2>(a, al, bl, gather, grid, stream);
  if (tc == 1) return gemm_h_dispatch<128, 64, 2, 2>(a, al, bl, gather, grid, stream);
  if (tc == 3) return gemm_h_dispatch<128, 96, 4, 1>(a, al, bl, gather, grid, stream);
  if (tc == 4) return gemm_h_dispatch<96, 128, 1, 4>(a, al, bl, gather, grid, stream);
  return gemm_h_dispatch<64, 64, 2, 2>(a, al, bl, gather, grid, stream);
}

static int g_dma_enabled = getenv("DM_GEMM_DMA") ? atoi(getenv("DM_GEMM_DMA")) : 1;
extern "C" int dm_gemm_dma_enable(int on) {
  if (on >= 0) g_dma_enabled = on > 2 ? 2 : on;
  return g_dma_enabled;
}
template <void (*KERN)(const GemmKArgs)>
static int dma_launch(int lds_bytes, const GemmKArgs& a, dim3 grid, hipStream_t stream) {
  static std::atomic<int> done[DM_MAX_DEVICES];
  int dev = 0;
  if (hipGetDevice(&dev) != hipSuccess || dev < 0 || dev >= DM_MAX_DEVICES) return dm_fail(DM_E_DEVICE, "gemm: hipGetDevice failed / device %d", dev);
  if (!done[dev].load(std::memory_order_acquire)) {
    hipError_t rc = hipFuncSetAttribute((const void*)KERN, hipFuncAttributeMaxDynamicSharedMemorySize, lds_bytes);
    if (rc != hipSuccess) return dm_fail(DM_E_HIP, "gemm: hipFuncSetAttribute(%d B of LDS): %s", lds_bytes, hipGetErrorString(rc));
    done[dev].store(1, std::memory_order_release);
  }
  hipLaunchKernelGGL(KERN, grid, dim3(256), (size_t)lds_bytes, stream, a);
  DM_LAUNCH_CHECK();
  return DM_OK;
}
template <int BM, int BN, int WGM, int WGN>
static int gemm_dma_dispatch(const GemmKArgs& a, int al, int bl, int gather, dim3 grid, hipStream_t stream) {
  constexpr int NS = (BM + BN) * 128 * 3 <= 72 * 1024 ? 3 : 2;
  constexpr int LDS = NS * (BM + BN) * 128;
  constexpr int LDS2 = 2 * (BM + BN) * 128;
  if (a.c_tab) {
    if (gather != 1 || al != 0 || bl != 0) return dm_fail(DM_E_SHAPE, "gemm: the scatter epilogue is built for a gathered A, layout (0,0), 16-byte loads");
    return dma_launch<gemm_dma_kernel<BM, BN, 0, 0, true, false, WGM, WGN, true, 2>>(LDS2, a, grid, stream);
  }
  if (gather == 1) {
    if (al != 0 || bl != 0) return dm_fail(DM_E_SHAPE, "gemm: gathered A is built for layout (0,0) only");
    return dma_launch<gemm_dma_kernel<BM, BN, 0, 0, true, false, WGM, WGN, false, 2>>(LDS2, a, grid, stream);
  }
  if (gather == 2) {
    if (al != 1 || bl != 1) return dm_fail(DM_E_SHAPE, "gemm: gathered B is built for layout (1,1) only");
    return dma_launch<gemm_dma_kernel<BM, BN, 1, 1, false, true, WGM, WGN, false, 2>>(LDS2, a, grid, stream);
  }
  if (al == 0 && bl == 0) return dma_launch<gemm_dma_kernel<BM, BN, 0, 0, false, false, WGM, WGN, false, NS>>(LDS, a, grid, stream);
  if (al == 0 && bl == 1) return dma_launch<gemm_dma_kernel<BM, BN, 0, 1, false, false, WGM, WGN, false, NS>>(LDS, a, grid, stream);
  if (al == 1 && bl == 0) return dma_launch<gemm_dma_kernel<BM, BN, 1, 0, false, false, WGM, WGN, false, NS>>(LDS, a, grid, stream);
  return dma_launch<gemm_dma_kernel<BM, BN, 1, 1, false, false, WGM, WGN, false, NS>>(LDS, a, grid, stream);
}

template <int BM, int BN, bool V, int WGM = 2, int WGN = 2, int BF = 0>
static int gemm_dispatch(const GemmKArgs& a, int al, int bl, int gather, dim3 grid, hipStream_t stream) {
  if constexpr (V && BF == 0) {
    if (a.use_dma) return gemm_dma_dispatch<BM, BN, WGM, WGN>(a, al, bl, gather, grid, stream);
  }
  if (a.c_tab) {
    if (gather != 1 || al != 0 || bl != 0 || !V) return dm_fail(DM_E_SHAPE, "gemm: the scatter epilogue is built for a gathered A, layout (0,0), 16-byte loads");
    hipLaunchKernelGGL((gemm_f32_kernel<BM, BN, 0, 0, true, true, false, WGM, WGN, BF, true>), grid, dim3(256), 0, stream, a);
  } else if (gather == 1) {
    if (al != 0 || bl != 0) return dm_fail(DM_E_SHAPE, "gemm: gathered A is built for layout (0,0) only");
    hipLaunchKernelGGL((gemm_f32_kernel<BM, BN, 0, 0, V, true, false, WGM, WGN, BF>), grid, dim3(256), 0, stream, a);
  } else if (gather == 2) {
    if (al != 1 || bl != 1) return dm_fail(DM_E_SHAPE, "gemm: gathered B is built for layout (1,1) only");
    hipLaunchKernelGGL((gemm_f32_kernel<BM, BN, 1, 1, V, false, true, WGM, WGN, BF>), grid, dim3(256), 0, stream, a);
  } else if (al == 0 && bl == 0) hipLaunchKernelGGL((gemm_f32_kernel<BM, BN, 0, 0, V, false, false, WGM, WGN, BF>), grid, dim3(256), 0, stream, a);
  else if (al == 0 && bl == 1) hipLaunchKernelGGL((gemm_f32_kernel<BM, BN, 0, 1, V, false, false, WGM, WGN, BF>), grid, dim3(256), 0, stream, a);
  else if (al == 1 && bl == 0) hipLaunchKernelGGL((gemm_f32_kernel<BM, BN, 1, 0, V, false, false, WGM, WGN, BF>), grid, dim3(256), 0, stream, a);
  else hipLaunchKernelGGL((gemm_f32_kernel<BM, BN, 1, 1, V, false, false, WGM, WGN, BF>), grid, dim3(256), 0, stream, a);
  return DM_OK;
}

struct TwinRange { const float* base; size_t n; unsigned short* twin; bool valid; };
static thread_local TwinRange tl_twins[48];
static thread_local int tl_ntwins = 0;
static thread_local bool tl_twins_on = false;
static int g_twins_enabled = getenv("DM_BF16_NO_TWINS") ? 0 : 1;
extern "C" int dm_bf16_twins_enable(int on) {
  if (on >= 0) g_twins_enabled = on ? 1 : 0;
  return g_twins_enabled;
}
DmTwinScope::DmTwinScope(bool bf16_mode) {
  opened = !tl_twins_on;
  active = bf16_mode && g_twins_enabled;
  if (opened) { tl_twins_on = active; tl_ntwins = 0; }
}
DmTwinScope::~DmTwinScope() {
  if (opened) { tl_twins_on = false; tl_ntwins = 0; }
}
bool dm_twins_on() { return tl_twins_on; }
void dm_twin_add(const float* base, size_t n, unsigned short* twin, bool valid) {
  if (!tl_twins_on || !base || !twin || n == 0 || tl_ntwins >= 48) return;
  tl_twins[tl_ntwins++] = TwinRange{base, n, twin, valid};
}
static TwinRange* twin_find(const float* p) {
  if (!tl_twins_on || !p) return nullptr;
  for (int i = tl_ntwins - 1; i >= 0; --i)
    if (p >= tl_twins[i].base && p < tl_twins[i].base + tl_twins[i].n) return &tl_twins[i];
  return nullptr;
}
void dm_twin_mark(const float* p) {
  TwinRange* r = twin_find(p);
  if (r) r->valid = true;
}
unsigned short* dm_twin_of(const float* p, bool need_valid) {
  TwinRange* r = twin_find(p);
  if (!r || (need_valid && !r->valid)) return nullptr;
  return r->twin + (p - r->base);
}

#include <mutex>
#include <unordered_map>
static std::mutex g_arena_mu;
static std::unordered_map<const void*, bool> g_arena_twins;
void dm_twin_arena_note(const void* acts, bool written) {
  std::lock_guard<std::mutex> lk(g_arena_mu);
  if (g_arena_twins.size() > 4096) g_arena_twins.clear();
  g_arena_twins[acts] = written;
}
bool dm_twin_arena_valid(const void* acts) {
  std::lock_guard<std::mutex> lk(g_arena_mu);
  auto it = g_arena_twins.find(acts);
  return it != g_arena_twins.end() && it->second;
}

static thread_local int tl_precision = 0;
int dm_cur_precision() { return tl_precision; }
DmPrecisionScope::DmPrecisionScope(int p) : prev(tl_precision) { tl_precision = p ? 1 : 0; }
DmPrecisionScope::~DmPrecisionScope() { tl_precision = prev; }


int dm_gemm_launch(const DmGemm& q, void* ws, size_t ws_bytes, hipStream_t stream) {
  DM_REQUIRE(q.M >= 0 && q.N >= 0 && q.K >= 1, DM_E_SHAPE, "gemm: bad dims M=%d N=%d K=%d (K must be >= 1)", q.M, q.N, q.K);
  if (q.M == 0 || q.N == 0) return DM_OK;
  DM_REQUIRE(((q.A && q.B) || (q.A_h && q.B_h)) && q.C, DM_E_NULL, "gemm: null operand");
  DM_REQUIRE((q.A_h == nullptr) == (q.B_h == nullptr), DM_E_NULL, "gemm: bf16-storage operands come in pairs");
  DM_REQUIRE((unsigned)q.a_layout < 2 && (unsigned)q.b_layout < 2, DM_E_SHAPE, "gemm: bad layout");
  DM_REQUIRE(q.a_maj || q.lda >= (q.a_layout == 0 ? q.K : q.M), DM_E_SHAPE, "gemm: lda %d too small", q.lda);
  DM_REQUIRE(q.b_maj || q.ldb >= (q.b_layout == 0 ? q.K : q.N), DM_E_SHAPE, "gemm: ldb %d too small", q.ldb);
  DM_REQUIRE((q.a_maj == nullptr) == (q.a_min == nullptr) && (q.b_maj == nullptr) == (q.b_min == nullptr), DM_E_NULL,
             "gemm: gather tables must come in (major, minor) pairs");
  DM_REQUIRE(q.c_tab || q.ldc >= q.N, DM_E_SHAPE, "gemm: ldc %d < N %d", q.ldc, q.N);
  DM_REQUIRE(!q.add || q.ldadd >= q.N, DM_E_SHAPE, "gemm: ldadd %d < N %d", q.ldadd, q.N);

  {
    const int sk = (q.A_h || q.C_h) ? 0 : dm_gemm_skinny_try(q, stream);
    if (sk < 0) return sk;
    if (sk == 1) {
      unsigned short* t = (q.bf16 && dm_twins_on()) ? dm_twin_of(q.C, false) : nullptr;
      if (t && q.ldc == q.N) {
        const DmCvtSeg sg = {q.C, t, (size_t)q.M * q.N};
        DM_TRY(dm_to_bf16_multi_launch(&sg, 1, stream));
        dm_twin_mark(q.C);
      }
      return DM_OK;
    }
  }
  DM_REQUIRE(!q.ln_g && !q.lnb_x && !q.gates && !q.eg_x && !q.lnf_ps && !q.sm_logits, DM_E_SHAPE,
             "gemm: LayerNorm prologues / the gates epilogue are built for the <= 64-row skinny products only (M=%d K=%d)", q.M, q.K);
  const unsigned short* Ah = q.A_h;
  const unsigned short* Bh = q.B_h;
  unsigned short* Chh = q.C_h;
  if (q.bf16 && dm_twins_on()) {
    if (!Ah && !Bh) {
      const unsigned short* ta = dm_twin_of(q.A, true);
      const unsigned short* tb = dm_twin_of(q.B, true);
      const bool fits = ta && tb && ((((uintptr_t)ta | (uintptr_t)tb) & 15) == 0) &&
                        ((q.K & 7) == 0 || (q.a_layout == 1 && q.b_layout == 1)) &&
                        (q.a_maj ? q.a_tab_vec8 != 0 : (q.lda & 7) == 0) && (q.b_maj ? q.b_tab_vec8 != 0 : (q.ldb & 7) == 0) &&
                        (q.a_layout == 0 || ((q.M & 7) == 0 && q.M >= 8)) && (q.b_layout == 0 || ((q.N & 7) == 0 && q.N >= 8));
      const int min_k = (q.a_maj || q.b_maj || q.c_tab) ? DM_HSTORE_MIN_K : DM_HSTORE_MIN_K_DENSE;
      if (fits && ((q.a_layout == 1 && q.b_layout == 1) || q.K >= min_k)) { Ah = ta; Bh = tb; }
    }
    if (!Chh && !q.no_twin) Chh = dm_twin_of(q.C, false);
    if (Chh) dm_twin_mark(q.C);
  }
  const bool hstore = Ah && Bh;
  DM_REQUIRE(!hstore || ((((uintptr_t)Ah | (uintptr_t)Bh) & 15) == 0 && ((q.K & 7) == 0 || (q.a_layout == 1 && q.b_layout == 1)) &&
                         (q.a_maj ? q.a_tab_vec8 != 0 : (q.lda & 7) == 0) && (q.b_maj ? q.b_tab_vec8 != 0 : (q.ldb & 7) == 0) &&
                         (q.a_layout == 0 || ((q.M & 7) == 0 && q.M >= 8)) && (q.b_layout == 0 || ((q.N & 7) == 0 && q.N >= 8))),
             DM_E_SHAPE, "gemm: bf16-storage operands need 16-byte aligned rows and extents in multiples of 8 (M=%d N=%d K=%d)",
             q.M, q.N, q.K);
  GemmKArgs a;
  a.Ch = Chh;
  a.A = q.A; a.B = q.B; a.C = q.C; a.bias = q.bias; a.add = q.add; a.mulref = q.mulref; a.row_zero = q.row_zero; a.partial = nullptr;
  a.M = q.M; a.N = q.N; a.K = q.K;
  a.lda = q.lda; a.ldb = q.ldb; a.ldc = q.ldc; a.ldadd = q.ldadd; a.ldmul = q.ldmul;
  a.flags = q.flags;
  a.a_maj = q.a_maj; a.a_min = q.a_min; a.b_maj = q.b_maj; a.b_min = q.b_min;
  a.c_tab = q.c_tab; a.sc_cout = q.sc_cout; a.sc_wpitch = q.sc_wpitch; a.bias_mod = q.bias_mod;
  DM_REQUIRE(!q.c_tab || (q.sc_cout > 0 && q.N % q.sc_cout == 0 && q.N / q.sc_cout == 4 && !q.add && !(q.flags & DM_GEMM_ACCUM)),
             DM_E_SHAPE, "gemm: scatter epilogue needs N = 4 * sc_cout, no addend, no accumulate");
  if (hstore) {
    a.A = reinterpret_cast<const float*>(Ah); a.B = reinterpret_cast<const float*>(Bh);
    static const int h_nt = getenv("DM_GEMM_H_NT") ? 1 : 0;
    if (h_nt) a.flags |= 1 << 20;
  }
  a.a_vec = hstore ? 1 : (((uintptr_t)q.A & 15) == 0 && (q.a_maj ? q.a_tab_vec != 0 : (q.lda & 3) == 0) &&
             (((q.a_layout == 0 ? q.K : q.M) & 3) == 0)) ? 1 : 0;
  a.b_vec = hstore ? 1 : (((uintptr_t)q.B & 15) == 0 && (q.b_maj ? q.b_tab_vec != 0 : (q.ldb & 3) == 0) &&
             (((q.b_layout == 0 ? q.K : q.N) & 3) == 0)) ? 1 : 0;

  const int ktiles = dm_cdiv(q.K, 32);
  const double out_elems = (double)q.M * q.N;
  int max_split = (int)(0.5 * ((double)q.M + q.N) * q.K / (out_elems > 0 ? out_elems : 1));
  if (max_split > ktiles / 2) max_split = ktiles / 2;
  if (max_split > 512) max_split = 512;
  {
    const size_t per = (size_t)q.M * q.N * sizeof(float);
    if (ws == nullptr || q.c_tab) max_split = 1;
    else if ((size_t)max_split * per > ws_bytes) max_split = (int)(ws_bytes / per);
  }
  if (max_split < 1) max_split = 1;
  static const int cand[5][2] = {{128, 128}, {128, 64}, {64, 64}, {128, 96}, {96, 128}};
  static const double keq[5] = {150.0, 60.0, 45.0, 45.0, 45.0};
  static const double rate[5] = {1.0, 0.9, 0.8, 0.75, 0.75};
  static const double resid[5] = {3.0, 4.0, 7.0, 4.0, 4.0};
  const double lat_macs = 1.0e6;
  static const int force_tile = getenv("DM_GEMM_TILE") ? atoi(getenv("DM_GEMM_TILE")) : 0;
  static const int force_split = getenv("DM_GEMM_SPLIT") ? atoi(getenv("DM_GEMM_SPLIT")) : 0;
  int BM = 64, BN = 64, nsplit = 1;
  double best_cost = -1.0;
  const int kt1 = ktiles > 0 ? ktiles : 1;
  const bool dma_shape_pre = !hstore && !q.bf16 && a.a_vec && a.b_vec;
  for (int c = 0; c < 5; ++c) {
    static const int sc_tile = getenv("DM_SC_TILE") ? atoi(getenv("DM_SC_TILE")) : 0;
    if (force_tile && c != force_tile - 1) continue;
    if (sc_tile && q.c_tab && c != sc_tile - 1) continue;
    static const int plain_tile = getenv("DM_PLAIN_TILE") ? atoi(getenv("DM_PLAIN_TILE")) : 0;
    if (plain_tile && !q.c_tab && !q.a_maj && !q.b_maj && c != plain_tile - 1) continue;
    static const int ga_tile = getenv("DM_GA_TILE") ? atoi(getenv("DM_GA_TILE")) : 0;
    if (ga_tile && !q.c_tab && (q.a_maj || q.b_maj) && c != ga_tile - 1) continue;
    if (!(a.a_vec && a.b_vec) && c != 2) continue;
    const int bm = cand[c][0], bn = cand[c][1];
    const int64_t t = (int64_t)dm_cdiv(q.M, bm) * dm_cdiv(q.N, bn);
    int sp_fill = 1;
    if (t < 256) {
      sp_fill = dm_cdiv(512, t);
      if (sp_fill > max_split) sp_fill = max_split;
    }
    if (sp_fill > kt1) sp_fill = kt1;
    if (sp_fill < 1) sp_fill = 1;
    static const int no_wide = getenv("DM_GEMM_NO_WIDE_SPLIT") ? 1 : 0;
    const bool wide = t < 16 && !no_wide;
    const int sp15 = wide ? sp_fill + sp_fill / 2 : sp_fill, sp20 = wide ? 2 * sp_fill : sp_fill;
    static const int balanced = getenv("DM_GEMM_NO_BALANCED_SPLIT") ? 0 : 1;
    int sps[10] = {1, sp_fill, t >= 256 ? 2 : sp_fill, t >= 256 ? 4 : sp_fill, sp15, sp20, sp_fill, sp_fill, sp_fill, sp_fill};
    if (balanced && t < 256)
      for (int k = 2; k <= 5; ++k) sps[4 + k] = (int)((256 * k) / t) > 0 ? (int)((256 * k) / t) : 1;
    for (int pass = 0; pass < 10; ++pass) {
      int sp = force_split > 0 ? force_split : sps[pass];
      if (force_split <= 0 && sp > max_split) sp = max_split;
      if (sp > kt1) sp = kt1;
      if (sp < 1) sp = 1;
      const double avg = (double)(t * sp) / 256.0;
      const double R = resid[c];
      const double waves = avg > R ? ceil(avg / R) : 1.0;
      const double conc = avg > R ? avg / waves : (avg > 1.0 ? (balanced ? ceil(avg - 1e-9) : avg) : 1.0);
      const double nkt = (double)dm_cdiv(kt1, sp);
      const double tm = (double)bm * bn * 32.0 / rate[c];
      const double per_kt = conc * tm > lat_macs ? conc * tm : lat_macs;
      double cost = waves * (nkt * per_kt + conc * bm * bn * keq[c] / rate[c]);
      if (sp > 1) cost += 0.4 * sp * out_elems + 1.2e6;
      if (q.a_maj && !q.c_tab && q.N <= 64 && c == 2) cost *= 0.8;
      if (q.c_tab) {
        if (c == 2 && q.K <= 800) cost *= 0.8;
        if (c == 3 && q.N % 96 == 0 && q.K > 800) cost *= 0.8;
      }
      if (!q.a_maj && !q.b_maj && !q.c_tab && dma_shape_pre && g_dma_enabled) {
        if (c == 0 && q.a_layout == 0 && q.b_layout == 1) cost *= 1.3;
        if (c == 2 && q.a_layout == 1 && q.b_layout == 1 && sp > 1 && t < 256 && dm_cdiv(kt1, sp) >= 14) cost *= 0.8;
      }
      if (best_cost < 0 || cost < best_cost) { best_cost = cost; BM = bm; BN = bn; nsplit = sp; }
    }
  }
  static const int dma_min_kt = getenv("DM_GEMM_DMA_MIN_KT") ? atoi(getenv("DM_GEMM_DMA_MIN_KT")) : 14;
  const bool dma_shape = !hstore && !q.bf16 && a.a_vec && a.b_vec && (q.a_layout == 0 ? q.M >= 1 : q.M >= 4) && (q.b_layout == 0 ? q.N >= 1 : q.N >= 4);
  auto dma_for = [&](int sp) { return g_dma_enabled && dma_shape && (dm_cdiv(kt1, sp) >= dma_min_kt || g_dma_enabled >= 2); };
  const int tiles_m = dm_cdiv(q.M, BM), tiles_n = dm_cdiv(q.N, BN);
  const int64_t tiles = (int64_t)tiles_m * tiles_n;
  int k_per_split = dm_cdiv(ktiles > 0 ? ktiles : 1, nsplit) * 32;
  nsplit = q.K > 0 ? dm_cdiv(q.K, k_per_split) : 1;
  a.k_per_split = k_per_split;
  a.nsplit = nsplit;
  a.tiles_m = tiles_m;
  a.partial = nsplit > 1 ? (float*)ws : nullptr;

  DM_REQUIRE(tiles * nsplit < (int64_t)1 << 30, DM_E_SHAPE, "gemm: too many work items");
  a.n_tiles = (int)tiles;
  a.tiles_n = tiles_n;
  a.n_fast = tiles_n <= tiles_m ? 1 : 0;
  a.n_items = (int)(tiles * nsplit);
  {
    static const int grp_env = getenv("DM_GEMM_XCD_GROUPS") ? atoi(getenv("DM_GEMM_XCD_GROUPS")) : 0;
    const int F = a.n_fast ? tiles_n : tiles_m, S = a.n_fast ? tiles_m : tiles_n;
    const int bf = a.n_fast ? BN : BM, bs = a.n_fast ? BM : BN;
    int best_g = 1;
    if (nsplit == 1 && tiles >= 64 && !q.c_tab) {
      double best = -1.0;
      for (int G = 1; G <= 4; G *= 2) {
        if (grp_env > 1 && G != grp_env) continue;
        if (F / G < 2) break;
        const double width = (double)F / G;
        double srows = ((double)tiles / 8.0) / width;
        if (srows > S) srows = S;
        if (srows < 1.0) srows = 1.0;
        const double cost = srows * bs + width * bf;
        if (best < 0 || cost < best * 0.95) { best = cost; best_g = G; }
      }
    }
    a.n_groups = grp_env == 1 ? 1 : best_g;
  }
  const int tc = (BM == 128 && BN == 128) ? 0 : (BM == 128 && BN == 64) ? 1 : (BM == 64 ? 2 : (BN == 96 ? 3 : 4));
  dim3 grid((unsigned)a.n_items);
  const int gather = q.a_maj ? 1 : (q.b_maj ? 2 : 0);
  DM_REQUIRE(!(q.a_maj && q.b_maj), DM_E_SHAPE, "gemm: only one gathered operand per call");
  a.use_dma = dma_for(nsplit) ? 1 : 0;
  const int kind = tc * 4 + q.a_layout * 2 + q.b_layout + (a.use_dma ? 24 : 0);
  const int slot = prof_before(kind, 2.0 * q.M * q.N * (double)q.K,
                               4.0 * ((double)q.M * q.K + (double)q.N * q.K + (double)q.M * q.N), stream);
  if (slot >= 0) {
    long long* sh = &g_prof.shape[5 * (size_t)slot];
    sh[0] = q.M; sh[1] = q.N; sh[2] = q.K; sh[3] = nsplit; sh[4] = (q.a_maj ? 1 : 0) | (q.b_maj ? 2 : 0) | (q.c_tab ? 4 : 0) | (q.bf16 ? 8 : 0) |
            (hstore ? 32 : 0);
  }
  int rc;
  const bool vec = a.a_vec && a.b_vec;
  static const int no_pipe = getenv("DM_GEMM_NO_PIPE") ? 1 : 0;
  const bool pipe_ok = vec && !no_pipe && (q.a_layout == 0 ? q.M >= 1 : q.M >= 4) && (q.b_layout == 0 ? q.N >= 1 : q.N >= 4);
  if (hstore) rc = gemm_h_tiles(tc, a, q.a_layout, q.b_layout, gather, grid, stream);
  else if (pipe_ok && q.bf16) rc = gemm_pipe_tiles(tc, a, q.a_layout, q.b_layout, gather, grid, stream);
  else if (vec && q.bf16) {
    if (tc == 0) rc = gemm_dispatch<128, 128, true, 2, 2, 1>(a, q.a_layout, q.b_layout, gather, grid, stream);
    else if (tc == 1) rc = gemm_dispatch<128, 64, true, 2, 2, 1>(a, q.a_layout, q.b_layout, gather, grid, stream);
    else if (tc == 3) rc = gemm_dispatch<128, 96, true, 4, 1, 1>(a, q.a_layout, q.b_layout, gather, grid, stream);
    else if (tc == 4) rc = gemm_dispatch<96, 128, true, 1, 4, 1>(a, q.a_layout, q.b_layout, gather, grid, stream);
    else rc = gemm_dispatch<64, 64, true, 2, 2, 1>(a, q.a_layout, q.b_layout, gather, grid, stream);
  } else if (vec) {
    if (tc == 0) rc = gemm_dispatch<128, 128, true>(a, q.a_layout, q.b_layout, gather, grid, stream);
    else if (tc == 1) rc = gemm_dispatch<128, 64, true>(a, q.a_layout, q.b_layout, gather, grid, stream);
    else if (tc == 3) rc = gemm_dispatch<128, 96, true, 4, 1>(a, q.a_layout, q.b_layout, gather, grid, stream);
    else if (tc == 4) rc = gemm_dispatch<96, 128, true, 1, 4>(a, q.a_layout, q.b_layout, gather, grid, stream);
    else rc = gemm_dispatch<64, 64, true>(a, q.a_layout, q.b_layout, gather, grid, stream);
  } else {
    rc = gemm_dispatch<64, 64, false>(a, q.a_layout, q.b_layout, gather, grid, stream);
  }
  if (rc != DM_OK) return rc;
  prof_after(slot, stream);
  DM_LAUNCH_CHECK();
  if (nsplit > 1) {
    const size_t total = (size_t)q.M * q.N;
    int blocks = dm_cdiv(total, 256);
    if (blocks > 2048) blocks = 2048;
    hipLaunchKernelGGL(gemm_splitk_reduce_kernel, dim3(blocks), dim3(256), 0, stream, a);
    DM_LAUNCH_CHECK();
  }
  if (q.C_frag) {
    DM_REQUIRE(q.M <= 64 && !q.c_tab, DM_E_SHAPE, "gemm: a fragment-major copy of C needs M <= 64 (M=%d)", q.M);
    DM_TRY(dm_frag_pack_launch(q.M, q.N, q.C, q.ldc, q.C_frag, stream));
  }
  return DM_OK;
}

extern "C" int dm_gemm_f32(int a_layout, int b_layout, int M, int N, int K, const float* A, int lda,
                           const float* B, int ldb, float* C, int ldc, const float* bias, const float* add,
                           int ldadd, int flags, void* ws, size_t ws_bytes, void* stream) {
  DmPrecisionScope prec(flags & DM_GEMM_BF16);
  DmGemm g;
  g.a_layout = a_layout; g.b_layout = b_layout;
  g.M = M; g.N = N; g.K = K;
  g.A = A; g.lda = lda; g.B = B; g.ldb = ldb; g.C = C; g.ldc = ldc;
  g.bias = bias; g.add = add; g.ldadd = ldadd; g.flags = flags & ~DM_GEMM_BF16;
  return dm_gemm_launch(g, ws, ws_bytes, (hipStream_t)stream);
}

extern "C" int dm_gemm_bf16h(int a_layout, int b_layout, int M, int N, int K, const uint16_t* A, int lda, const uint16_t* B,
                             int ldb, float* C, int ldc, uint16_t* C_h, const float* bias, int flags, void* ws, size_t ws_bytes,
                             void* stream) {
  DmPrecisionScope prec(1);
  DmGemm g;
  g.a_layout = a_layout; g.b_layout = b_layout;
  g.M = M; g.N = N; g.K = K;
  g.A_h = A; g.lda = lda; g.B_h = B; g.ldb = ldb; g.C = C; g.ldc = ldc; g.C_h = C_h;
  g.bias = bias;
  g.flags = flags & ~DM_GEMM_BF16;
  return dm_gemm_launch(g, ws, ws_bytes, (hipStream_t)stream);
}
```

pydreamer_amd/csrc/mlp.hip:

```cpp
#include "common.h"
#include <stdlib.h>

struct MlpActs {
  float* xpre[DM_MAX_MLP_LAYERS];
  float* stats[DM_MAX_MLP_LAYERS];
  float* y[DM_MAX_MLP_LAYERS];
};
static size_t mlp_carve(int rows, int hidden, int layers, float* base, MlpActs* a) {
  DmArena ar(base, (size_t)1 << 62);
  for (int l = 0; l < layers; ++l) {
    float* xp = ar.take((size_t)rows * hidden);
    float* st = ar.take((size_t)rows * 2);
    float* yy = ar.take((size_t)rows * hidden);
    if (a) { a->xpre[l] = xp; a->stats[l] = st; a->y[l] = yy; }
  }
  return ar.off;
}
extern "C" size_t dm_mlp_acts_floats(int rows, int hidden, int layers) {
  if (rows < 0 || hidden < 0 || layers < 0 || layers > DM_MAX_MLP_LAYERS) return 0;
  return mlp_carve(rows, hidden, layers, nullptr, nullptr);
}

static size_t mlp_ws_floats(int rows, int hidden, int layers) {
  const size_t rh = dm_align_up((size_t)rows * hidden, 64);
// ... 134 lines not shown
      in = a.y[l]; ldin = hidden; kin = hidden;
    }
  }
  DmGemm q;
  q.M = rows; q.N = out_dim; q.K = hidden;
  q.A = in; q.lda = hidden;
  q.B = p->w[layers]; q.ldb = hidden;
  q.C = out; q.ldc = ldout;
  q.bias = p->b[layers];
  return dm_gemm_launch(q, ws, skb, st);
}

extern "C" int dm_mlp_head_fwd(int rows, int in_dim, int hidden, int layers, int out_dim, const float* x, int ldx,
                               const dm_mlp_params* p, float* acts, float* out, void* ws, size_t ws_bytes, void* stream) {
  DM_REQUIRE(x && p && out && ws, DM_E_NULL, "mlp_head_fwd: null pointer");
  DmPrecisionScope prec(p->precision);
  return dm_mlp_fwd_launch(rows, in_dim, hidden, layers, out_dim, x, ldx, p, acts, rows, 0, out, out_dim, ws, ws_bytes,
                           (hipStream_t)stream);
}

extern "C" int dm_mlp_head_fwd_sparse(int rows, int in_dim, int sparse_cols, int hidden, int layers, int out_dim,
                                      const float* x, int ldx, const dm_mlp_params* p, float* acts, float* out, void* ws,
                                      size_t ws_bytes, void* stream) {
  DM_REQUIRE(x && p && out && ws, DM_E_NULL, "mlp_head_fwd_sparse: null pointer");
  DmPrecisionScope prec(p->precision);
  return dm_mlp_fwd_launch(rows, in_dim, hidden, layers, out_dim, x, ldx, p, acts, rows, 0, out, out_dim, ws, ws_bytes,
                           (hipStream_t)stream, nullptr, sparse_cols);
}

extern "C" int dm_mlp_head_fwd_rows(int rows_total, int row0, int rows, int in_dim, int sparse_cols, int hidden, int layers,
                                    int out_dim, const float* x, int ldx, const dm_mlp_params* p, float* acts, float* out,
                                    void* ws, size_t ws_bytes, void* stream) {
  DM_REQUIRE(x && p && out && ws, DM_E_NULL, "mlp_head_fwd_rows: null pointer");
  DM_REQUIRE(row0 >= 0 && rows >= 1 && row0 + rows <= rows_total, DM_E_SHAPE, "mlp_head_fwd_rows: window [%d, %d) of %d rows", row0,
             row0 + rows, rows_total);
  DmPrecisionScope prec(p->precision);
  return dm_mlp_fwd_launch(rows, in_dim, hidden, layers, out_dim, x + (size_t)row0 * ldx, ldx, p, acts, rows_total, row0,
                           out + (size_t)row0 * out_dim, out_dim, ws, ws_bytes, (hipStream_t)stream, nullptr, sparse_cols);
}

extern "C" int dm_mlp_head_bwd(int rows, int in_dim, int hidden, int layers, int out_dim, const float* x, int ldx,
                               const dm_mlp_params* p, const float* acts, const float* dout, const dm_mlp_grads* g,
                               float* dx, int lddx, int dx_accum, void* ws, size_t ws_bytes, void* stream) {
  DM_REQUIRE(x && p && acts && dout && g && ws, DM_E_NULL, "mlp_head_bwd: null pointer");
  DmPrecisionScope prec(p->precision);
  DM_REQUIRE(layers >= 1 && layers <= DM_MAX_MLP_LAYERS, DM_E_SHAPE, "mlp: layers=%d", layers);
  hipStream_t st = (hipStream_t)stream;
  MlpActs a;
  mlp_carve(rows, hidden, layers, const_cast<float*>(acts), &a);
  DmArena ar(ws, ws_bytes);
  float* splitk = ar.take(DM_SPLITK_FLOATS);
  float* dy = ar.take((size_t)rows * hidden);
  float* dxp = ar.take((size_t)rows * hidden);
  const bool normed = p->ln_g[0] != nullptr;
  const bool panel = normed && dm_panel_ok(rows, hidden) && ((uintptr_t)p->w[layers] & 15) == 0;
  const int npanels = dm_panel_count(rows);
  float* colpart = ar.take(panel ? (size_t)layers * npanels * 3 * hidden : 0);
  float* wt = (panel && dm_cur_precision()) ? ar.take((size_t)hidden * hidden) : nullptr;
  DM_REQUIRE(ar.ok, DM_E_WORKSPACE, "mlp_head_bwd: workspace too small (need %zu floats)", ar.off);
  const unsigned short* wth[DM_MAX_MLP_LAYERS] = {};
  if (panel && dm_cur_precision() && (hidden & 7) == 0 && layers > 1) {
    const float* src[DM_MAX_MLP_LAYERS];
    unsigned short* dst[DM_MAX_MLP_LAYERS];
    int rws[DM_MAX_MLP_LAYERS], cls[DM_MAX_MLP_LAYERS];
    for (int l = 1; l < layers; ++l) {
      src[l - 1] = p->w[l]; rws[l - 1] = hidden; cls[l - 1] = hidden;
      dst[l - 1] = (unsigned short*)ar.take(((size_t)hidden * hidden + 1) / 2);
    }
    if (ar.ok) {
      DM_TRY(dm_panel_bf16_weights_launch(layers - 1, src, dst, rws, cls, 1, st));
      for (int l = 1; l < layers; ++l) wth[l] = dst[l - 1];
    }
  }
  const size_t skb = DM_SPLITK_FLOATS * sizeof(float);

  if (panel) {
    {
      DmGemm q;
      q.a_layout = 1; q.b_layout = 1;
      q.M = out_dim; q.N = hidden; q.K = rows;
      q.A = dout; q.lda = out_dim;
      q.B = a.y[layers - 1]; q.ldb = hidden;
      q.C = g->w[layers]; q.ldc = hidden;
      DM_TRY(dm_gemm_launch(q, splitk, skb, st));
      DM_TRY(dm_colsum_launch(rows, out_dim, dout, out_dim, g->b[layers], splitk, skb, st));
    }
    float* cur = dxp;
    float* other = dy;
    DM_TRY(dm_panel_ln_bwd_launch(rows, hidden, out_dim, dout, out_dim, p->w[layers], a.xpre[layers - 1],
                                  a.stats[layers - 1], p->ln_g[layers - 1], p->ln_b[layers - 1], cur,
                                  colpart + (size_t)(layers - 1) * npanels * 3 * hidden, nullptr, st));
    for (int l = layers - 1; l >= 0; --l) {
      const float* in = l == 0 ? x : a.y[l - 1];
      const int ldin = l == 0 ? ldx : hidden;
      const int kin = l == 0 ? in_dim : hidden;
      DmGemm q;
      q.a_layout = 1; q.b_layout = 1;
      q.M = hidden; q.N = kin; q.K = rows;
      q.A = cur; q.lda = hidden;
      q.B = in; q.ldb = ldin;
      q.C = g->w[l]; q.ldc = kin;
      DM_TRY(dm_gemm_launch(q, splitk, skb, st));
      if (l > 0) {
        DM_TRY(dm_panel_ln_bwd_launch(rows, hidden, hidden, cur, hidden, p->w[l], a.xpre[l - 1], a.stats[l - 1],
                                      p->ln_g[l - 1], p->ln_b[l - 1], other, colpart + (size_t)(l - 1) * npanels * 3 * hidden,
                                      wt, st, wth[l]));
        float* t = cur; cur = other; other = t;
      } else if (dx) {
        DmGemm d;
        d.a_layout = 0; d.b_layout = 1;
        d.M = rows; d.N = kin; d.K = hidden;
        d.A = cur; d.lda = hidden;
        d.B = p->w[0]; d.ldb = kin;
        d.C = dx; d.ldc = lddx; d.flags = dx_accum ? DM_GEMM_ACCUM : 0;
        DM_TRY(dm_gemm_launch(d, splitk, skb, st));
      }
    }
    const float* parts[3 * DM_MAX_MLP_LAYERS];
    float* outs[3 * DM_MAX_MLP_LAYERS];
    for (int l = 0; l < layers; ++l) {
      const float* base = colpart + (size_t)l * npanels * 3 * hidden;
      parts[3 * l + 0] = base;              outs[3 * l + 0] = g->b[l];
      parts[3 * l + 1] = base + hidden;     outs[3 * l + 1] = g->ln_g[l];
      parts[3 * l + 2] = base + 2 * hidden; outs[3 * l + 2] = g->ln_b[l];
    }
    return dm_panel_colsum_final_launch(3 * layers, parts, outs, hidden, npanels, 3 * hidden, st);
  }

  {
    DmGemm q;
    q.a_layout = 1; q.b_layout = 1;
    q.M = out_dim; q.N = hidden; q.K = rows;
    q.A = dout; q.lda = out_dim;
    q.B = a.y[layers - 1]; q.ldb = hidden;
    q.C = g->w[layers]; q.ldc = hidden;
    DM_TRY(dm_gemm_launch(q, splitk, skb, st));
    DM_TRY(dm_colsum_launch(rows, out_dim, dout, out_dim, g->b[layers], splitk, skb, st));
    DmGemm d;
    d.a_layout = 0; d.b_layout = 1;
    d.M = rows; d.N = hidden; d.K = out_dim;
    d.A = dout; d.lda = out_dim;
    d.B = p->w[layers]; d.ldb = hidden;
    d.C = dy; d.ldc = hidden;
    DM_TRY(dm_gemm_launch(d, splitk, skb, st));
  }
  for (int l = layers - 1; l >= 0; --l) {
    const float* in = l == 0 ? x : a.y[l - 1];
    const int ldin = l == 0 ? ldx : hidden;
    const int kin = l == 0 ? in_dim : hidden;
    if (normed) {
      DM_TRY(dm_ln_elu_bwd_dx_launch(rows, hidden, a.xpre[l], hidden, a.y[l], hidden, a.stats[l], p->ln_g[l], dy, hidden,
                                     dxp, hidden, st));
      DM_TRY(dm_ln_elu_bwd_params_launch(rows, hidden, a.xpre[l], hidden, a.y[l], hidden, a.stats[l], dy, hidden,
                                         g->ln_g[l], g->ln_b[l], splitk, skb, st));
    } else {
      DM_TRY(dm_elu_bwd_launch(rows, hidden, a.y[l], hidden, dy, hidden, dxp, hidden, st));
    }
    DmGemm q;
    q.a_layout = 1; q.b_layout = 1;
    q.M = hidden; q.N = kin; q.K = rows;
    q.A = dxp; q.lda = hidden;
    q.B = in; q.ldb = ldin;
    q.C = g->w[l]; q.ldc = kin;
    DM_TRY(dm_gemm_launch(q, splitk, skb, st));
    DM_TRY(dm_colsum_launch(rows, hidden, dxp, hidden, g->b[l], splitk, skb, st));
    if (l > 0 || dx) {
      DmGemm d;
      d.a_layout = 0; d.b_layout = 1;
      d.M = rows; d.N = kin; d.K = hidden;
      d.A = dxp; d.lda = hidden;
      d.B = p->w[l]; d.ldb = kin;
      if (l > 0) { d.C = dy; d.ldc = hidden; }
      else { d.C = dx; d.ldc = lddx; d.flags = dx_accum ? DM_GEMM_ACCUM : 0; }
      DM_TRY(dm_gemm_launch(d, splitk, skb, st));
    }
  }
  return DM_OK;
}
```

pydreamer_amd/csrc/rssm.hip:

```cpp
#include "common.h"
#include <stdlib.h>

struct RssmActs {
  float *ea, *ee, *hin, *zin, *x1, *st1, *za, *gi, *gh, *x2, *st2, *pin, *x3, *st3, *prin;
  float *gs, *gst;
};
static const int g_fwd_ln_z = getenv("DM_FWD_LN_Z") ? atoi(getenv("DM_FWD_LN_Z")) : 1;
static inline int rssm_gru_kind(const dm_shape* s) { return (s->flags & DM_FLAG_GRU_MASK) >> DM_FLAG_GRU_SHIFT; }
static inline int rssm_gru_layers(const dm_shape* s) {
  return 1 + ((s->flags & DM_FLAG_GRU_LAYERS_MASK) >> DM_FLAG_GRU_LAYERS_SHIFT);
}
static size_t rssm_carve(const dm_shape* s, float* base, RssmActs* a) {
  const size_t N = (size_t)s->T * s->B, Hd = s->Hd, D = s->D, Z = (size_t)s->S * (s->C ? s->C : 1);
  DmArena ar(base, (size_t)1 << 62);
  RssmActs t;
  t.ea = ar.take(N * Hd); t.ee = ar.take(N * Hd);
  t.hin = ar.take(N * D); t.zin = ar.take(N * Z);
  t.x1 = ar.take(N * Hd); t.st1 = ar.take(N * 2); t.za = ar.take(N * Hd);
  t.gi = ar.take(N * 3 * D); t.gh = ar.take(N * 3 * D);
  t.x2 = ar.take(N * Hd); t.st2 = ar.take(N * 2); t.pin = ar.take(N * Hd);
  t.x3 = ar.take(N * Hd); t.st3 = ar.take(N * 2); t.prin = ar.take(N * Hd);
  const bool lncell = rssm_gru_kind(s) != 0;
  t.gs = ar.take(lncell ? N * 3 * D : 0); t.gst = ar.take(lncell ? N * 6 * rssm_gru_layers(s) : 0);
  if (a) *a = t;
  return ar.off;
}
extern "C" size_t dm_rssm_acts_floats(const dm_shape* shp) {
  if (!shp) return 0;
  return rssm_carve(shp, nullptr, nullptr);
}

static int rssm_check(const dm_shape* s) {
  DM_REQUIRE(s->I == 1, DM_E_SHAPE, "rssm: iwae_samples=%d unsupported (only 1)", s->I);
  DM_REQUIRE(s->T >= 1 && s->B >= 1 && s->D >= 4 && s->Hd >= 4 && s->S >= 1 && (s->C >= 2 || s->C == 0) && s->A >= 1 && s->E >= 1,
             DM_E_SHAPE, "rssm: bad shape");
  DM_REQUIRE((s->D & 3) == 0, DM_E_SHAPE, "rssm: deter_dim must be a multiple of 4 (got %d)", s->D);
  DM_REQUIRE(rssm_gru_kind(s) <= 2, DM_E_SHAPE, "rssm: unknown recurrent cell kind %d", rssm_gru_kind(s));
  const int GL = rssm_gru_layers(s);
  DM_REQUIRE(s->D % (4 * GL) == 0, DM_E_SHAPE, "rssm: deter_dim=%d must be a multiple of 4*gru_layers (%d)", s->D, 4 * GL);
  return DM_OK;
}

struct GruStack {
  int L, ls, kind;
  const float *wih[4], *whh[4], *bih[4], *bhh[4];
  float *g_wih[4], *g_whh[4], *g_bih[4], *g_bhh[4];
  const float *lng[4][3], *lnb[4][3];
  float *g_lng[4][3], *g_lnb[4][3];
};
static int gru_stack(const dm_shape* s, const float* const* p, float* const* g, GruStack* k) {
  k->L = rssm_gru_layers(s);
  k->ls = s->D / k->L;
  k->kind = rssm_gru_kind(s);
  for (int i = 0; i < k->L; ++i) {
    const int lb = i == 0 ? DM_RSSM_GRU_LN_G0 : DM_RSSM_GRU_L1_LN_G0 + 6 * (i - 1);
    for (int q = 0; q < 3; ++q) {
      k->lng[i][q] = p[lb + 2 * q]; k->lnb[i][q] = p[lb + 2 * q + 1];
      k->g_lng[i][q] = g ? g[lb + 2 * q] : nullptr; k->g_lnb[i][q] = g ? g[lb + 2 * q + 1] : nullptr;
      const bool need = k->kind == 1 || (k->kind == 2 && q == 0);
      DM_REQUIRE(!need || (k->lng[i][q] && k->lnb[i][q]), DM_E_NULL, "rssm: LayerNorm GRU layer %d without LayerNorm parameter %d",
                 i, q);
      DM_REQUIRE(!need || !g || (k->g_lng[i][q] && k->g_lnb[i][q]), DM_E_NULL,
                 "rssm: LayerNorm GRU layer %d without LayerNorm gradient slot %d", i, q);
    }
    const int b = i == 0 ? DM_RSSM_GRU_WIH : DM_RSSM_GRU_L1_WIH + 4 * (i - 1);
    k->wih[i] = p[b]; k->whh[i] = p[b + 1]; k->bih[i] = p[b + 2]; k->bhh[i] = p[b + 3];
    const bool biased = rssm_gru_kind(s) == 0;
    DM_REQUIRE(k->wih[i] && k->whh[i] && (!biased || (k->bih[i] && k->bhh[i])), DM_E_NULL,
               "rssm: GRU layer %d has a null parameter", i);
    if (g) {
      k->g_wih[i] = g[b]; k->g_whh[i] = g[b + 1]; k->g_bih[i] = g[b + 2]; k->g_bhh[i] = g[b + 3];
      DM_REQUIRE(k->g_wih[i] && k->g_whh[i] && (!biased || (k->g_bih[i] && k->g_bhh[i])), DM_E_NULL,
                 "rssm: GRU layer %d has a null gradient slot", i);
    }
  }
  return DM_OK;
}

static int norm_elu_fwd(int rows, int n, const float* x, int ldx, const float* gamma, const float* beta, float eps, float* y,
                        int ldy, float* stats, hipStream_t st) {
  if (gamma) return dm_ln_elu_fwd_launch(rows, n, x, ldx, gamma, beta, eps, y, ldy, stats, st);
  return dm_elu_fwd_launch(rows, n, x, ldx, y, ldy, st);
}
static int norm_elu_bwd_dx(int rows, int n, const float* x, int ldx, const float* y, int ldy, const float* stats,
                           const float* gamma, const float* dy, int lddy, float* dx, int lddx, hipStream_t st) {
  if (gamma) return dm_ln_elu_bwd_dx_launch(rows, n, x, ldx, y, ldy, stats, gamma, dy, lddy, dx, lddx, st);
  return dm_elu_bwd_launch(rows, n, y, ldy, dy, lddy, dx, lddx, st);
}
static int norm_elu_bwd_params(int rows, int n, const float* x, int ldx, const float* y, int ldy, const float* stats,
                               const float* dy, int lddy, float* dgamma, float* dbeta, void* ws, size_t ws_bytes,
                               hipStream_t st) {
  if (!dgamma && !dbeta) return DM_OK;
  return dm_ln_elu_bwd_params_launch(rows, n, x, ldx, y, ldy, stats, dy, lddy, dgamma, dbeta, ws, ws_bytes, st);
}

static int linear(hipStream_t st, void* sk, size_t skb, int rows, int nout, int kin, const float* x, int ldx,
                  const float* W, const float* bias, const float* add, int ldadd, float* y, int ldy) {
  DmGemm q;
  q.M = rows; q.N = nout; q.K = kin;
  q.A = x; q.lda = ldx;
  q.B = W; q.ldb = kin;
  q.C = y; q.ldc = ldy;
  q.bias = bias; q.add = add; q.ldadd = ldadd;
  return dm_gemm_launch(q, sk, skb, st);
}
static int wgrad(hipStream_t st, void* sk, size_t skb, int rows, int nout, int kin, const float* dy, int lddy,
                 const float* x, int ldx, float* dW, int accum = 0) {
  DmGemm q;
  q.a_layout = 1; q.b_layout = 1;
  q.M = nout; q.N = kin; q.K = rows;
  q.A = dy; q.lda = lddy;
  q.B = x; q.ldb = ldx;
  q.C = dW; q.ldc = kin;
  q.flags = accum ? DM_GEMM_ACCUM : 0;
  return dm_gemm_launch(q, sk, skb, st);
}
static int dgrad(hipStream_t st, void* sk, size_t skb, int rows, int nout, int kin, const float* dy, int lddy,
                 const float* W, float* dx, int lddx, int accum, const uint8_t* row_zero) {
  DmGemm q;
  q.a_layout = 0; q.b_layout = 1;
  q.M = rows; q.N = kin; q.K = nout;
  q.A = dy; q.lda = lddy;
  q.B = W; q.ldb = kin;
  q.C = dx; q.ldc = lddx;
  q.flags = accum ? DM_GEMM_ACCUM : 0;
  q.row_zero = row_zero;
  return dm_gemm_launch(q, sk, skb, st);
}

static int dgrad_t(hipStream_t st, void* sk, size_t skb, int rows, int nout, int kin, const float* dy, int lddy,
                   const float* Wt, float* dx, int lddx, int accum, const uint8_t* row_zero) {
  DmGemm q;
  q.M = rows; q.N = kin; q.K = nout;
  q.A = dy; q.lda = lddy;
  q.B = Wt; q.ldb = nout;
  q.C = dx; q.ldc = lddx;
  q.flags = accum ? DM_GEMM_ACCUM : 0;
  q.row_zero = row_zero;
  return dm_gemm_launch(q, sk, skb, st);
}
static int transpose(hipStream_t st, const float* W, float* Wt, int rows, int cols) {
  return dm_permute4_launch(W, Wt, 1, 1, rows, cols, 0, 1, 3, 2, st);
}

static int gru_stack_fwd(hipStream_t st, void* sk, size_t skb, const GruStack& k, int rows, int Hd, int D, const float* x0,
                         const float* hin, int ldh, float* gi, float* gh, float* hout, int ldo, float* h_next,
                         const uint8_t* next_reset, float* gs, float* gst) {
  const int ls = k.ls;
  for (int i = 0; i < k.L; ++i) {
    const float* x = i == 0 ? x0 : hout + (size_t)(i - 1) * ls;
    const int ldx = i == 0 ? Hd : ldo, kin = i == 0 ? Hd : ls;
    DM_TRY(linear(st, sk, skb, rows, 3 * ls, kin, x, ldx, k.wih[i], k.bih[i], nullptr, 0, gi + 3 * ls * i, 3 * D));
    DM_TRY(linear(st, sk, skb, rows, 3 * ls, ls, hin + i * ls, ldh, k.whh[i], k.bhh[i], nullptr, 0, gh + 3 * ls * i, 3 * D));
    if (k.kind == 0)
      DM_TRY(dm_gru_gates_fwd_launch(rows, ls, gi + 3 * ls * i, gh + 3 * ls * i, hin + i * ls, ldh, hout + i * ls, ldo,
                                     h_next ? h_next + i * ls : nullptr, next_reset, nullptr, nullptr, st, 3 * D, D));
    else
      DM_TRY(dm_gru_norm_fwd_launch(k.kind, rows, ls, gi + 3 * ls * i, gh + 3 * ls * i, hin + i * ls, ldh, k.lng[i], k.lnb[i],
                                    hout + i * ls, ldo, gs + 3 * ls * i, gst + 6 * i, h_next ? h_next + i * ls : nullptr,
                                    next_reset, st, 3 * D, 6 * k.L, D));
  }
  return DM_OK;
}

extern "C" int dm_rssm_sequence_fwd(const dm_shape* s, const float* embed, const float* action, const uint8_t* reset,
                                    const float* h0, const float* z0, const float* u, const int32_t* forced_idx,
                                    const dm_rssm_params* P, float* acts, float* feat, float* post, float* prior,
                                    int32_t* idx, void* ws, size_t ws_bytes, void* stream) {
  DM_REQUIRE(s && embed && action && reset && h0 && z0 && P && acts && feat && post && prior && ws, DM_E_NULL,
             "rssm_sequence_fwd: null pointer");
  DM_REQUIRE(u || forced_idx, DM_E_NULL, "rssm_sequence_fwd: need uniforms or forced indices");
  DmPrecisionScope prec(s->flags & DM_FLAG_BF16);
  DM_TRY(rssm_check(s));
  DM_REQUIRE(ws_bytes >= DM_SPLITK_FLOATS * sizeof(float), DM_E_WORKSPACE, "rssm_sequence_fwd: workspace too small");
  hipStream_t st = (hipStream_t)stream;
  const int T = s->T, B = s->B, D = s->D, Hd = s->Hd, S = s->S, C = s->C, Z = S * (C ? C : 1), ZP = S * (C ? C : 2);
  const int F = D + Z, E = s->E, A = s->A;
  const bool gauss = C == 0;
  const int N = T * B;
  const size_t skb = DM_SPLITK_FLOATS * sizeof(float);
  RssmActs a;
  rssm_carve(s, acts, &a);
  const float* const* p = P->p;

  DM_TRY(linear(st, ws, skb, N, Hd, A, action, A, p[DM_RSSM_A_W], nullptr, nullptr, 0, a.ea, Hd));
  DM_TRY(linear(st, ws, skb, N, Hd, E, embed, E, p[DM_RSSM_POST_E_W], nullptr, nullptr, 0, a.ee, Hd));

  const int kind = rssm_gru_kind(s);
  const float* lng[3] = {p[DM_RSSM_GRU_LN_G0], p[DM_RSSM_GRU_LN_G1], p[DM_RSSM_GRU_LN_G2]};
  const float* lnb[3] = {p[DM_RSSM_GRU_LN_B0], p[DM_RSSM_GRU_LN_B1], p[DM_RSSM_GRU_LN_B2]};
  DM_REQUIRE(kind == 0 || (lng[0] && lnb[0] && (kind == 2 || (lng[1] && lnb[1] && lng[2] && lnb[2]))), DM_E_NULL,
             "rssm_sequence_fwd: LayerNorm GRU cell without its LayerNorm parameters");
  GruStack gk;
  DM_TRY(gru_stack(s, p, nullptr, &gk));
  const bool stacked = gk.L > 1;
  const bool normed = p[DM_RSSM_IN_G] != nullptr;
  DM_REQUIRE((p[DM_RSSM_POST_G] != nullptr) == normed && (p[DM_RSSM_PRIOR_G] != nullptr) == normed, DM_E_NULL,
// ... 124 lines not shown
                                   forced_idx ? forced_idx + r0 * S : nullptr, feat + r0 * F + D, F,
                                   idx ? idx + r0 * S : nullptr, zin_next, reset_next, st));
  }
  if (psync) {
    DmRssmLds pq;
    pq.B = B; pq.D = D; pq.Hd = Hd; pq.S = S; pq.C = C; pq.F = F; pq.t_begin = 1; pq.t_end = T;
    pq.wzt = wzt; pq.zb = p[DM_RSSM_Z_B];
    pq.wih = p[DM_RSSM_GRU_WIH]; pq.bih = p[DM_RSSM_GRU_BIH]; pq.whh = p[DM_RSSM_GRU_WHH]; pq.bhh = p[DM_RSSM_GRU_BHH];
    pq.wph = p[DM_RSSM_POST_H_W]; pq.bph = p[DM_RSSM_POST_H_B]; pq.wpo = p[DM_RSSM_POST_W]; pq.bpo = p[DM_RSSM_POST_OB];
    pq.in_g = p[DM_RSSM_IN_G]; pq.in_b = p[DM_RSSM_IN_B]; pq.post_g = p[DM_RSSM_POST_G]; pq.post_b = p[DM_RSSM_POST_B];
    pq.ea = a.ea; pq.ee = a.ee; pq.reset = reset; pq.u = u; pq.forced = forced_idx;
    pq.x1 = a.x1; pq.gi = a.gi; pq.gh = a.gh; pq.hin = a.hin; pq.zin = a.zin; pq.feat = feat; pq.x2 = a.x2; pq.post = post;
    pq.idx = idx; pq.ws = psync; pq.ws_floats = psync_floats;
    DM_TRY(dm_rssm_lds_launch(pq, st));
  }
  if (fuse_ln || psync) {
    DM_TRY(norm_elu_fwd(N, Hd, a.x1, Hd, p[DM_RSSM_IN_G], p[DM_RSSM_IN_B], 1e-3f, a.za, Hd, a.st1, st));
    DM_TRY(norm_elu_fwd(N, Hd, a.x2, Hd, p[DM_RSSM_POST_G], p[DM_RSSM_POST_B], 1e-3f, a.pin, Hd, a.st2, st));
  }
  DM_TRY(linear(st, ws, skb, N, Hd, D, feat, F, p[DM_RSSM_PRIOR_H_W], p[DM_RSSM_PRIOR_H_B], nullptr, 0, a.x3, Hd));
  DM_TRY(norm_elu_fwd(N, Hd, a.x3, Hd, p[DM_RSSM_PRIOR_G], p[DM_RSSM_PRIOR_B], 1e-3f, a.prin, Hd, a.st3, st));
  DM_TRY(linear(st, ws, skb, N, ZP, Hd, a.prin, Hd, p[DM_RSSM_PRIOR_W], p[DM_RSSM_PRIOR_OB], nullptr, 0, prior, ZP));
  return DM_OK;
}

static int g_bptt_fold = getenv("DM_BPTT_FOLD") ? (atoi(getenv("DM_BPTT_FOLD")) ? 1 : 0) : 1;
extern "C" int dm_bptt_fold_enable(int on) {
  const int was = g_bptt_fold;
  if (on >= 0) g_bptt_fold = on ? 1 : 0;
  return was;
}
extern "C" int dm_rssm_sequence_bwd(const dm_shape* s, const float* embed, const float* action, const uint8_t* reset,
                                    const dm_rssm_params* P, const float* acts, const float* feat, const float* post,
                                    float* dfeat, float* dpost, float* dprior, const dm_rssm_grads* G, float* dembed,
                                    void* ws, size_t ws_bytes, void* stream) {
  DM_REQUIRE(s && embed && action && reset && P && acts && feat && post && dfeat && dpost && dprior && G && ws, DM_E_NULL,
             "rssm_sequence_bwd: null pointer");
  DmPrecisionScope prec(s->flags & DM_FLAG_BF16);
  DM_TRY(rssm_check(s));
  hipStream_t st = (hipStream_t)stream;
  const int T = s->T, B = s->B, D = s->D, Hd = s->Hd, S = s->S, C = s->C, Z = S * (C ? C : 1), ZP = S * (C ? C : 2);
  const int F = D + Z, E = s->E, A = s->A;
  const bool gauss = C == 0;
  const int N = T * B;
  RssmActs a;
  rssm_carve(s, const_cast<float*>(acts), &a);
  const float* const* p = P->p;
  float* const* g = G->p;

  DmArena ar(ws, ws_bytes);
  float* sk = ar.take(DM_SPLITK_FLOATS);
  float* dprin = ar.take((size_t)N * Hd);
  float* dx3 = ar.take((size_t)N * Hd);
  float* dpin = ar.take((size_t)N * Hd);
  float* dx2 = ar.take((size_t)N * Hd);
  float* dgi = ar.take((size_t)N * 3 * D);
  float* dgh = ar.take((size_t)N * 3 * D);
  float* dza = ar.take((size_t)N * Hd);
  float* dx1 = ar.take((size_t)N * Hd);
  float* wt_post = ar.take((size_t)ZP * Hd);
  float* wt_post_h = ar.take((size_t)Hd * D);
  float* wt_ih = ar.take((size_t)3 * D * Hd);
  float* wt_hh = ar.take((size_t)3 * D * D);
  float* wt_z = ar.take((size_t)Hd * Z);
  const int kind = rssm_gru_kind(s);
  float* dgl = ar.take(kind ? (size_t)N * 3 * D : 0);
  float* lnpg = ar.take(kind ? (size_t)3 * D : 0);
  float* lnpb = ar.take(kind ? (size_t)3 * D : 0);
  float* sk_w = ar.take(DM_SPLITK_FLOATS);
  float* dx2_w = ar.take((size_t)N * Hd);
  float* dx1_w = ar.take((size_t)N * Hd);
  const float* lng[3] = {p[DM_RSSM_GRU_LN_G0], p[DM_RSSM_GRU_LN_G1], p[DM_RSSM_GRU_LN_G2]};
  const float* lnb[3] = {p[DM_RSSM_GRU_LN_B0], p[DM_RSSM_GRU_LN_B1], p[DM_RSSM_GRU_LN_B2]};
  DM_REQUIRE(ar.ok, DM_E_WORKSPACE, "rssm_sequence_bwd: workspace too small (need %zu floats)", ar.off);
  const size_t skb = DM_SPLITK_FLOATS * sizeof(float);

  hipStream_t const st_main = st;
  hipStream_t sw = st == (hipStream_t)stream ? dm_wgrad_side_stream(st) : st;

  DM_TRY(dgrad(st, sk, skb, N, ZP, Hd, dprior, ZP, p[DM_RSSM_PRIOR_W], dprin, Hd, 0, nullptr));
  DM_TRY(norm_elu_bwd_dx(N, Hd, a.x3, Hd, a.prin, Hd, a.st3, p[DM_RSSM_PRIOR_G], dprin, Hd, dx3, Hd, st));
  DM_TRY(dgrad(st, sk, skb, N, Hd, D, dx3, Hd, p[DM_RSSM_PRIOR_H_W], dfeat, F, 1, nullptr));
  DM_TRY(dm_wgrad_side_fork(st, sw));
  DM_TRY(wgrad(sw, sk_w, skb, N, ZP, Hd, dprior, ZP, a.prin, Hd, g[DM_RSSM_PRIOR_W]));
  DM_TRY(dm_colsum_launch(N, ZP, dprior, ZP, g[DM_RSSM_PRIOR_OB], sk_w, skb, sw));
  DM_TRY(norm_elu_bwd_params(N, Hd, a.x3, Hd, a.prin, Hd, a.st3, dprin, Hd, g[DM_RSSM_PRIOR_G],
                                     g[DM_RSSM_PRIOR_B], sk_w, skb, sw));
  DM_TRY(wgrad(sw, sk_w, skb, N, Hd, D, dx3, Hd, feat, F, g[DM_RSSM_PRIOR_H_W]));
  DM_TRY(dm_colsum_launch(N, Hd, dx3, Hd, g[DM_RSSM_PRIOR_H_B], sk_w, skb, sw));

  DM_TRY(transpose(st, p[DM_RSSM_POST_W], wt_post, ZP, Hd));
  DM_TRY(transpose(st, p[DM_RSSM_POST_H_W], wt_post_h, Hd, D));
  GruStack gk;
  DM_TRY(gru_stack(s, p, g, &gk));
  const bool stacked = gk.L > 1;
  if (!stacked) {
    DM_TRY(transpose(st, p[DM_RSSM_GRU_WIH], wt_ih, 3 * D, Hd));
    DM_TRY(transpose(st, p[DM_RSSM_GRU_WHH], wt_hh, 3 * D, D));
  }
  DM_TRY(transpose(st, p[DM_RSSM_Z_W], wt_z, Hd, Z));
  const bool fuse_b = p[DM_RSSM_IN_G] != nullptr && !stacked && !gauss && kind == 0 && dm_skinny_ln_ok(B, D, Hd) &&
                      dm_skinny_ln_ok(B, Z, Hd) && (F & 3) == 0;
  bool fold = fuse_b && g_bptt_fold && B <= 64 && (int64_t)Hd * ZP >= (int64_t)64 * 1024 &&
              (int64_t)Hd * 3 * D >= (int64_t)64 * 1024 && (ZP & 3) == 0 && ((3 * D) & 3) == 0 && ZP >= 16;
  float *xw2 = nullptr, *xwz = nullptr, *cs2 = nullptr, *csz = nullptr, *eps2 = nullptr, *eps1 = nullptr;
  const int nstrip = (Hd + 15) / 16;
  if (fold) {
    const size_t mark = ar.off;
    xw2 = ar.take((size_t)N * D);
    xwz = ar.take((size_t)N * Z);
    cs2 = ar.take((size_t)D);
    csz = ar.take((size_t)Z);
    eps2 = ar.take((size_t)nstrip * 128);
    eps1 = ar.take((size_t)nstrip * 128);
    if (!ar.ok) { ar.off = mark; ar.ok = true; fold = false; }
  }
  static const int no_fold_sm = getenv("DM_BPTT_NO_FOLD_SM") ? 1 : 0;
  const bool fold_sm = fold && !gauss && C == 32 && Z == ZP && !no_fold_sm;
  if (fold) {
    DM_TRY(dgrad(st, sk, skb, N, Hd, D, a.x2, Hd, p[DM_RSSM_POST_H_W], xw2, D, 0, nullptr));
    DM_TRY(dgrad(st, sk, skb, N, Hd, Z, a.x1, Hd, p[DM_RSSM_Z_W], xwz, Z, 0, nullptr));
    DM_TRY(dm_colsum_launch(Hd, D, p[DM_RSSM_POST_H_W], D, cs2, sk, skb, st));
    DM_TRY(dm_colsum_launch(Hd, Z, p[DM_RSSM_Z_W], Z, csz, sk, skb, st));
  }
  static const int no_frag = getenv("DM_SKINNY_NO_FRAG") ? 1 : 0;
  float* dgif = (fuse_b && !no_frag && B <= 64) ? ar.take(dm_frag_floats(3 * D)) : nullptr;
  float* dghf = dgif ? ar.take(dm_frag_floats(3 * D)) : nullptr;
  float* dpinf = dgif ? ar.take(dm_frag_floats(Hd)) : nullptr;
  float* dzaf = dgif ? ar.take(dm_frag_floats(Hd)) : nullptr;
  if (!ar.ok) { dgif = nullptr; dghf = nullptr; dpinf = nullptr; dzaf = nullptr; }
  const int nchunk = (stacked || B < 16) ? 1 : (T >= 16 ? 4 : T >= 8 ? 2 : 1);
  int next_chunk = nchunk - 1;
  const float* dx2s = fuse_b ? dx2_w : dx2;
  const float* dx1s = fuse_b ? dx1_w : dx1;
  auto side_chunk = [&](int t) -> int {
    if (stacked || next_chunk < 0 || t != (int)((long long)T * next_chunk / nchunk)) return DM_OK;
    const int c = next_chunk--;
    const int t0 = (int)((long long)T * c / nchunk), t1 = (int)((long long)T * (c + 1) / nchunk);
    const size_t c0 = (size_t)t0 * B;
    const int rows = (t1 - t0) * B, acc = c != nchunk - 1;
    DM_TRY(dm_wgrad_side_fork(st, sw));
    if (fuse_b) {
      DM_TRY(norm_elu_bwd_dx(rows, Hd, a.x2 + c0 * Hd, Hd, a.pin + c0 * Hd, Hd, a.st2 + c0 * 2, p[DM_RSSM_POST_G], dpin + c0 * Hd, Hd,
                             dx2_w + c0 * Hd, Hd, sw));
      DM_TRY(norm_elu_bwd_dx(rows, Hd, a.x1 + c0 * Hd, Hd, a.za + c0 * Hd, Hd, a.st1 + c0 * 2, p[DM_RSSM_IN_G], dza + c0 * Hd, Hd,
                             dx1_w + c0 * Hd, Hd, sw));
    }
    DM_TRY(wgrad(sw, sk_w, skb, rows, ZP, Hd, dpost + c0 * ZP, ZP, a.pin + c0 * Hd, Hd, g[DM_RSSM_POST_W], acc));
    DM_TRY(wgrad(sw, sk_w, skb, rows, Hd, D, dx2s + c0 * Hd, Hd, feat + c0 * F, F, g[DM_RSSM_POST_H_W], acc));
    DM_TRY(wgrad(sw, sk_w, skb, rows, Hd, E, dx2s + c0 * Hd, Hd, embed + c0 * E, E, g[DM_RSSM_POST_E_W], acc));
    DM_TRY(wgrad(sw, sk_w, skb, rows, 3 * D, Hd, dgi + c0 * 3 * D, 3 * D, a.za + c0 * Hd, Hd, g[DM_RSSM_GRU_WIH], acc));
    DM_TRY(wgrad(sw, sk_w, skb, rows, 3 * D, D, dgh + c0 * 3 * D, 3 * D, a.hin + c0 * D, D, g[DM_RSSM_GRU_WHH], acc));
    DM_TRY(wgrad(sw, sk_w, skb, rows, Hd, Z, dx1s + c0 * Hd, Hd, a.zin + c0 * Z, Z, g[DM_RSSM_Z_W], acc));
    DM_TRY(wgrad(sw, sk_w, skb, rows, Hd, A, dx1s + c0 * Hd, Hd, action + c0 * A, A, g[DM_RSSM_A_W], acc));
    return DM_OK;
  };
  for (int t = T - 1; t >= 0; --t) {
    const size_t r0 = (size_t)t * B;
    float* dft = dfeat + r0 * F;
    float* dpt = dpost + r0 * ZP;
    if (gauss) DM_TRY(dm_gauss_sample_bwd_launch(B, S, post + r0 * ZP, ZP, feat + r0 * F + D, F, dft + D, F, dpt, ZP, 1, st));
    else if (!(fold_sm && t < T - 1)) DM_TRY(dm_st_softmax_bwd_launch(B, S, C, post + r0 * ZP, ZP, dft + D, F, dpt, ZP, 1, st));
    if (fuse_b) {
      DmGemm q3;
      q3.M = B; q3.N = Hd; q3.K = ZP; q3.A = dpt; q3.lda = ZP; q3.B = wt_post; q3.ldb = ZP; q3.C = dpin + r0 * Hd; q3.ldc = Hd;
      q3.C_frag = dpinf;
      if (fold) {
        q3.C_frag = nullptr;
        q3.eg_x = a.x2 + r0 * Hd; q3.eg_ldx = Hd; q3.eg_stats = a.st2 + r0 * 2; q3.eg_gamma = p[DM_RSSM_POST_G]; q3.eg_beta = p[DM_RSSM_POST_B];
        q3.eg_G = dx2 + r0 * Hd; q3.eg_ldg = Hd; q3.eg_Gf = dpinf; q3.eg_ps = eps2;
      }
      DM_TRY(dm_gemm_launch(q3, sk, skb, st));
    } else {
      DM_TRY(dgrad_t(st, sk, skb, B, ZP, Hd, dpt, ZP, wt_post, dpin + r0 * Hd, Hd, 0, nullptr));
    }
    if (fuse_b) {
      const uint8_t* rz = reset + r0;
      float* dprev = t > 0 ? dfeat + (r0 - B) * F : nullptr;
      DmGatesBwd gb;
      gb.gi = a.gi + r0 * 3 * D; gb.gh = a.gh + r0 * 3 * D; gb.h_in = a.hin + r0 * D; gb.ldh = D; gb.D = D;
      gb.dgi = dgi + r0 * 3 * D; gb.dgh = dgh + r0 * 3 * D; gb.dprev = dprev; gb.ldp = F; gb.row_zero = rz;
      gb.dgi_frag = dgif; gb.dgh_frag = dghf;
      DmGemm q4;
      q4.M = B; q4.N = D; q4.K = Hd; q4.A = dpin + r0 * Hd; q4.lda = Hd; q4.B = wt_post_h; q4.ldb = Hd;
      q4.C = dft; q4.ldc = F; q4.flags = DM_GEMM_ACCUM;
      q4.ln_g = p[DM_RSSM_POST_G]; q4.ln_b = p[DM_RSSM_POST_B]; q4.lnb_x = a.x2 + r0 * Hd; q4.lnb_ldx = Hd;
      q4.lnb_stats = a.st2 + r0 * 2; q4.gates = &gb; q4.A_frag = dpinf;
      if (fold) {
        q4.A = dx2 + r0 * Hd; q4.ln_g = nullptr; q4.ln_b = nullptr; q4.lnb_x = nullptr; q4.lnb_stats = nullptr;
        q4.lnf_ps = eps2; q4.lnf_nps = nstrip; q4.lnf_stats = a.st2 + r0 * 2; q4.lnf_xw = xw2 + r0 * D; q4.lnf_ldxw = D; q4.lnf_cs = cs2;
      }
      DM_TRY(dm_gemm_launch(q4, sk, skb, st));
      {
        DmGemm q5;
        q5.M = B; q5.N = Hd; q5.K = 3 * D; q5.A = dgi + r0 * 3 * D; q5.lda = 3 * D; q5.B = wt_ih; q5.ldb = 3 * D;
        q5.C = dza + r0 * Hd; q5.ldc = Hd; q5.A_frag = dgif; q5.C_frag = dzaf;
        if (fold) {
          q5.C_frag = nullptr;
          q5.eg_x = a.x1 + r0 * Hd; q5.eg_ldx = Hd; q5.eg_stats = a.st1 + r0 * 2; q5.eg_gamma = p[DM_RSSM_IN_G]; q5.eg_beta = p[DM_RSSM_IN_B];
          q5.eg_G = dx1 + r0 * Hd; q5.eg_ldg = Hd; q5.eg_Gf = dzaf; q5.eg_ps = eps1;
        }
        DM_TRY(dm_gemm_launch(q5, sk, skb, st));
      }
      if (t > 0) {
        DmGemm qh, qz;
        qh.M = B; qh.N = D; qh.K = 3 * D; qh.A = dgh + r0 * 3 * D; qh.lda = 3 * D; qh.B = wt_hh; qh.ldb = 3 * D;
        qh.A_frag = dghf;
        qh.C = dprev; qh.ldc = F; qh.flags = DM_GEMM_ACCUM; qh.row_zero = rz;
        qz.M = B; qz.N = Z; qz.K = Hd; qz.A = dza + r0 * Hd; qz.lda = Hd; qz.B = wt_z; qz.ldb = Hd;
        qz.C = dprev + D; qz.ldc = F; qz.flags = DM_GEMM_ACCUM; qz.row_zero = rz;
        qz.ln_g = p[DM_RSSM_IN_G]; qz.ln_b = p[DM_RSSM_IN_B]; qz.lnb_x = a.x1 + r0 * Hd; qz.lnb_ldx = Hd;
        qz.lnb_stats = a.st1 + r0 * 2; qz.A_frag = dzaf;
        if (fold) {
          qz.A = dx1 + r0 * Hd; qz.ln_g = nullptr; qz.ln_b = nullptr; qz.lnb_x = nullptr; qz.lnb_stats = nullptr;
          if (fold_sm) { qz.sm_logits = post + (r0 - B) * ZP; qz.sm_ld = ZP; qz.sm_dlogits = dpost + (r0 - B) * ZP; qz.sm_ldd = ZP; }
          qz.lnf_ps = eps1; qz.lnf_nps = nstrip; qz.lnf_stats = a.st1 + r0 * 2; qz.lnf_xw = xwz + r0 * Z; qz.lnf_ldxw = Z; qz.lnf_cs = csz;
        }
        DM_TRY(dm_gemm_pair_launch(qh, qz, sk, skb, st));
      }
      DM_TRY(side_chunk(t));
      continue;
    }
    DM_TRY(norm_elu_bwd_dx(B, Hd, a.x2 + r0 * Hd, Hd, a.pin + r0 * Hd, Hd, a.st2 + r0 * 2, p[DM_RSSM_POST_G],
                                   dpin + r0 * Hd, Hd, dx2 + r0 * Hd, Hd, st));
    DM_TRY(dgrad_t(st, sk, skb, B, Hd, D, dx2 + r0 * Hd, Hd, wt_post_h, dft, F, 1, nullptr));
    const uint8_t* rz = reset + r0;
    float* dprev = t > 0 ? dfeat + (r0 - B) * F : nullptr;
    if (stacked) {
      const int ls = gk.ls;
      for (int i = gk.L - 1; i >= 0; --i) {
        float* dgi_i = dgi + r0 * 3 * D + 3 * ls * i;
        float* dgh_i = dgh + r0 * 3 * D + 3 * ls * i;
        if (kind == 0)
          DM_TRY(dm_gru_gates_bwd_launch(B, ls, a.gi + r0 * 3 * D + 3 * ls * i, a.gh + r0 * 3 * D + 3 * ls * i,
                                         a.hin + r0 * D + i * ls, D, dft + i * ls, F, dgi_i, dgh_i,
                                         dprev ? dprev + i * ls : nullptr, F, 1, rz, st, 3 * D));
        else
          DM_TRY(dm_gru_norm_bwd_launch(kind, B, ls, a.gh + r0 * 3 * D + 3 * ls * i, a.hin + r0 * D + i * ls, D,
                                        a.gs + r0 * 3 * D + 3 * ls * i, a.gst + r0 * 6 * gk.L + 6 * i, gk.lng[i], gk.lnb[i],
                                        dft + i * ls, F, dgi_i, dgh_i, dgl + r0 * 3 * D + 3 * ls * i,
                                        dprev ? dprev + i * ls : nullptr, F, rz, st, 3 * D, 6 * gk.L));
        if (i > 0) DM_TRY(dgrad(st, sk, skb, B, 3 * ls, ls, dgi_i, 3 * D, gk.wih[i], dft + (i - 1) * ls, F, 1, nullptr));
        else DM_TRY(dgrad(st, sk, skb, B, 3 * ls, Hd, dgi_i, 3 * D, gk.wih[0], dza + r0 * Hd, Hd, 0, nullptr));
        if (dprev) DM_TRY(dgrad(st, sk, skb, B, 3 * ls, ls, dgh_i, 3 * D, gk.whh[i], dprev + i * ls, F, 1, rz));
      }
      DM_TRY(norm_elu_bwd_dx(B, Hd, a.x1 + r0 * Hd, Hd, a.za + r0 * Hd, Hd, a.st1 + r0 * 2, p[DM_RSSM_IN_G],
                                     dza + r0 * Hd, Hd, dx1 + r0 * Hd, Hd, st));
      if (t > 0) DM_TRY(dgrad_t(st, sk, skb, B, Hd, Z, dx1 + r0 * Hd, Hd, wt_z, dprev + D, F, 1, rz));
      continue;
    }
    if (kind == 0)
      DM_TRY(dm_gru_gates_bwd_launch(B, D, a.gi + r0 * 3 * D, a.gh + r0 * 3 * D, a.hin + r0 * D, D, dft, F,
                                     dgi + r0 * 3 * D, dgh + r0 * 3 * D, dprev, F, 1, rz, st));
    else
      DM_TRY(dm_gru_norm_bwd_launch(kind, B, D, a.gh + r0 * 3 * D, a.hin + r0 * D, D, a.gs + r0 * 3 * D, a.gst + r0 * 6, lng,
                                    lnb, dft, F, dgi + r0 * 3 * D, dgh + r0 * 3 * D, dgl + r0 * 3 * D, dprev, F, rz, st));
    DM_TRY(dgrad_t(st, sk, skb, B, 3 * D, Hd, dgi + r0 * 3 * D, 3 * D, wt_ih, dza + r0 * Hd, Hd, 0, nullptr));
    DM_TRY(norm_elu_bwd_dx(B, Hd, a.x1 + r0 * Hd, Hd, a.za + r0 * Hd, Hd, a.st1 + r0 * 2, p[DM_RSSM_IN_G],
                                   dza + r0 * Hd, Hd, dx1 + r0 * Hd, Hd, st));
    if (t > 0) {
      DmGemm qh, qz;
      qh.M = B; qh.N = D; qh.K = 3 * D; qh.A = dgh + r0 * 3 * D; qh.lda = 3 * D; qh.B = wt_hh; qh.ldb = 3 * D;
      qh.C = dprev; qh.ldc = F; qh.flags = DM_GEMM_ACCUM; qh.row_zero = rz;
      qz.M = B; qz.N = Z; qz.K = Hd; qz.A = dx1 + r0 * Hd; qz.lda = Hd; qz.B = wt_z; qz.ldb = Hd;
      qz.C = dprev + D; qz.ldc = F; qz.flags = DM_GEMM_ACCUM; qz.row_zero = rz;
      DM_TRY(dm_gemm_pair_launch(qh, qz, sk, skb, st));
    }
    DM_TRY(side_chunk(t));
  }

  if (fuse_b) DM_TRY(norm_elu_bwd_dx(N, Hd, a.x2, Hd, a.pin, Hd, a.st2, p[DM_RSSM_POST_G], dpin, Hd, dx2, Hd, st));
  if (dembed) DM_TRY(dgrad(st, sk, skb, N, Hd, E, dx2, Hd, p[DM_RSSM_POST_E_W], dembed, E, 0, nullptr));
  st = sw;
  sk = sk_w;
  if (stacked) DM_TRY(dm_wgrad_side_fork(st_main, sw));
  DM_TRY(dm_colsum_launch(N, ZP, dpost, ZP, g[DM_RSSM_POST_OB], sk, skb, st));
  DM_TRY(norm_elu_bwd_params(N, Hd, a.x2, Hd, a.pin, Hd, a.st2, dpin, Hd, g[DM_RSSM_POST_G], g[DM_RSSM_POST_B],
                                     sk, skb, st));
  DM_TRY(dm_colsum_launch(N, Hd, dx2s, Hd, g[DM_RSSM_POST_H_B], sk, skb, st));
  if (stacked) {
    DM_TRY(wgrad(st, sk, skb, N, ZP, Hd, dpost, ZP, a.pin, Hd, g[DM_RSSM_POST_W]));
    DM_TRY(wgrad(st, sk, skb, N, Hd, D, dx2, Hd, feat, F, g[DM_RSSM_POST_H_W]));
    DM_TRY(wgrad(st, sk, skb, N, Hd, E, dx2, Hd, embed, E, g[DM_RSSM_POST_E_W]));
  }
  if (stacked) {
    const int ls = gk.ls;
    for (int i = 0; i < gk.L; ++i) {
      const float* x = i == 0 ? a.za : feat + (size_t)(i - 1) * ls;
      const int ldx = i == 0 ? Hd : F, kin = i == 0 ? Hd : ls;
      DM_TRY(wgrad(st, sk, skb, N, 3 * ls, kin, dgi + 3 * ls * i, 3 * D, x, ldx, gk.g_wih[i]));
      DM_TRY(wgrad(st, sk, skb, N, 3 * ls, ls, dgh + 3 * ls * i, 3 * D, a.hin + i * ls, D, gk.g_whh[i]));
      if (kind == 0) {
        DM_TRY(dm_colsum_launch(N, 3 * ls, dgi + 3 * ls * i, 3 * D, gk.g_bih[i], sk, skb, st));
        DM_TRY(dm_colsum_launch(N, 3 * ls, dgh + 3 * ls * i, 3 * D, gk.g_bhh[i], sk, skb, st));
      } else {
        DM_TRY(dm_gru_norm_param_grads_launch(kind, N, ls, a.gs + 3 * ls * i, a.gst + 6 * i, dgl + 3 * ls * i, lnpg, lnpb, st,
                                              3 * D, 6 * gk.L));
        const int parts = kind == 1 ? 3 : 1;
        const size_t len = (size_t)(kind == 1 ? ls : 3 * ls) * sizeof(float);
        for (int q = 0; q < parts; ++q)
          if (hipMemcpyAsync(gk.g_lng[i][q], lnpg + (size_t)q * ls, len, hipMemcpyDeviceToDevice, st) != hipSuccess ||
              hipMemcpyAsync(gk.g_lnb[i][q], lnpb + (size_t)q * ls, len, hipMemcpyDeviceToDevice, st) != hipSuccess)
            return dm_fail(DM_E_HIP, "rssm_sequence_bwd: gradient copy failed");
      }
    }
  }
  if (stacked) {
  } else if (kind == 0) {
    DM_TRY(dm_colsum_launch(N, 3 * D, dgi, 3 * D, g[DM_RSSM_GRU_BIH], sk, skb, st));
    DM_TRY(dm_colsum_launch(N, 3 * D, dgh, 3 * D, g[DM_RSSM_GRU_BHH], sk, skb, st));
  } else {
    DM_TRY(dm_gru_norm_param_grads_launch(kind, N, D, a.gs, a.gst, dgl, lnpg, lnpb, st));
    const int parts = kind == 1 ? 3 : 1;
    const size_t len = (kind == 1 ? (size_t)D : (size_t)3 * D) * sizeof(float);
    float* const gdst[3] = {g[DM_RSSM_GRU_LN_G0], g[DM_RSSM_GRU_LN_G1], g[DM_RSSM_GRU_LN_G2]};
    float* const bdst[3] = {g[DM_RSSM_GRU_LN_B0], g[DM_RSSM_GRU_LN_B1], g[DM_RSSM_GRU_LN_B2]};
    for (int q = 0; q < parts; ++q) {
      DM_REQUIRE(gdst[q] && bdst[q], DM_E_NULL, "rssm_sequence_bwd: missing LayerNorm-GRU gradient slot %d", q);
      if (hipMemcpyAsync(gdst[q], lnpg + (size_t)q * D, len, hipMemcpyDeviceToDevice, st) != hipSuccess ||
          hipMemcpyAsync(bdst[q], lnpb + (size_t)q * D, len, hipMemcpyDeviceToDevice, st) != hipSuccess)
        return dm_fail(DM_E_HIP, "rssm_sequence_bwd: gradient copy failed");
    }
  }
  DM_TRY(norm_elu_bwd_params(N, Hd, a.x1, Hd, a.za, Hd, a.st1, dza, Hd, g[DM_RSSM_IN_G], g[DM_RSSM_IN_B], sk, skb,
                                     st));
  DM_TRY(dm_colsum_launch(N, Hd, dx1s, Hd, g[DM_RSSM_Z_B], sk, skb, st));
  if (stacked) {
    DM_TRY(wgrad(st, sk, skb, N, Hd, Z, dx1, Hd, a.zin, Z, g[DM_RSSM_Z_W]));
    DM_TRY(wgrad(st, sk, skb, N, Hd, A, dx1, Hd, action, A, g[DM_RSSM_A_W]));
  }
  DM_TRY(dm_wgrad_side_mark(sw, st_main));
  return DM_OK;
}

static thread_local int tl_marks_n = 0;
static thread_local int tl_mark_step[4];
static thread_local hipEvent_t tl_mark_ev[4];
extern "C" int dm_dream_rollout_marks(int n, const int* steps, void* const* events) {
  DM_REQUIRE(n >= 0 && n <= 4 && (n == 0 || (steps && events)), DM_E_SHAPE, "dream_rollout_marks: n=%d (0..4)", n);
  for (int i = 0; i < n; ++i) {
    DM_REQUIRE(events[i], DM_E_NULL, "dream_rollout_marks: null event %d", i);
    tl_mark_step[i] = steps[i];
    tl_mark_ev[i] = (hipEvent_t)events[i];
  }
  tl_marks_n = n;
  return DM_OK;
}
struct DmRolloutMarks {
  int n;
  bool done[4] = {false, false, false, false};
  hipStream_t caller;
  explicit DmRolloutMarks(hipStream_t st) : n(tl_marks_n), caller(st) { tl_marks_n = 0; }
  void at_step(int i, hipStream_t st, bool eager) {
    if (!eager) return;
    for (int k = 0; k < n; ++k)
      if (!done[k] && tl_mark_step[k] == i) { (void)hipEventRecord(tl_mark_ev[k], st); done[k] = true; }
  }
  ~DmRolloutMarks() {
    for (int k = 0; k < n; ++k)
      if (!done[k]) (void)hipEventRecord(tl_mark_ev[k], caller);
  }
};

static int g_rollout_fuse_act = getenv("DM_ROLLOUT_NO_FUSE_ACT") ? 0 : 1;
extern "C" int dm_rollout_fuse_act_enable(int on) {
  if (on >= 0) g_rollout_fuse_act = on ? 1 : 0;
  return g_rollout_fuse_act;
}

extern "C" int dm_dream_rollout(const dm_shape* s, int M, const float* start, const dm_rssm_params* P,
                                const dm_mlp_params* actor, const float* u_act, const float* u_prior, float* feats,
                                float* actions, int32_t* act_idx, float* actor_acts, float* actor_logits, void* ws,
                                size_t ws_bytes, void* stream) {
  DM_REQUIRE(s && start && P && actor && u_act && u_prior && feats && actions && ws, DM_E_NULL,
             "dream_rollout: null pointer");
  DmPrecisionScope prec(s->flags & DM_FLAG_BF16);
  DM_TRY(rssm_check(s));
  DM_REQUIRE(M >= 1 && s->H >= 1, DM_E_SHAPE, "dream_rollout: M=%d H=%d", M, s->H);
  hipStream_t st = (hipStream_t)stream;
  const int H = s->H, D = s->D, Hd = s->Hd, S = s->S, C = s->C, Z = S * (C ? C : 1), ZP = S * (C ? C : 2);
  const int F = D + Z, A = s->A;
  const int Hm = s->mlp_hidden, L = s->mlp_layers;
  const int adist = s->flags & 3;
  DM_REQUIRE(adist <= 2, DM_E_SHAPE, "dream_rollout: unknown actor distribution %d", adist);
  const int AO = adist == 0 ? A : 2 * A;
  const float* const* p = P->p;

  DmArena ar(ws, ws_bytes);
  float* sk = ar.take(DM_SPLITK_FLOATS);
  DM_REQUIRE((actor_acts == nullptr) == (actor_logits == nullptr), DM_E_NULL,
             "dream_rollout: actor_acts and actor_logits must be given together");
  float* macts = ar.take(actor_acts ? 0 : dm_mlp_acts_floats(M, Hm, L));
  float* logits_ws = ar.take(actor_acts ? 0 : (size_t)M * AO);
  float* ea = ar.take((size_t)M * Hd);
  float* x1 = ar.take((size_t)M * Hd);
  float* za = ar.take((size_t)M * Hd);
  float* stats = ar.take((size_t)M * 2);
  float* gi = ar.take((size_t)M * 3 * D);
  float* gh = ar.take((size_t)M * 3 * D);
  float* prior = ar.take((size_t)M * ZP);
  const int kind = rssm_gru_kind(s);
  float* gsw = ar.take(kind ? (size_t)M * 3 * D : 0);
  float* gstw = ar.take(kind ? (size_t)M * 6 * rssm_gru_layers(s) : 0);
  const float* lng[3] = {p[DM_RSSM_GRU_LN_G0], p[DM_RSSM_GRU_LN_G1], p[DM_RSSM_GRU_LN_G2]};
  const float* lnb[3] = {p[DM_RSSM_GRU_LN_B0], p[DM_RSSM_GRU_LN_B1], p[DM_RSSM_GRU_LN_B2]};
  DmTwinScope tw((s->flags & DM_FLAG_BF16) != 0);
  const bool tw_on = dm_twins_on() && kind == 0 && rssm_gru_layers(s) == 1 && p[DM_RSSM_IN_G] && p[DM_RSSM_PRIOR_G] && (F & 7) == 0;
  unsigned short* wih_h = (unsigned short*)ar.take(tw_on ? dm_half_floats((size_t)3 * D * Hd) : 0);
  unsigned short* whh_h = (unsigned short*)ar.take(tw_on ? dm_half_floats((size_t)3 * D * D) : 0);
  unsigned short* wph_h = (unsigned short*)ar.take(tw_on ? dm_half_floats((size_t)Hd * D) : 0);
  unsigned short* wp_h = (unsigned short*)ar.take(tw_on ? dm_half_floats((size_t)ZP * Hd) : 0);
// ... 114 lines not shown
```

Before: 30.24.

## Fuse bias-gradient column sums into weight-gradient GEMM kernels

Adds a dbias output to the GEMM descriptor. The weight-gradient kernels (fp32 and DMA variants) now accumulate the row sums of the A operand from the fragments they already load, write them per split, and reduce them in the split-K reduce kernel. Separate colsum launches in the MLP, conv encoder/decoder and RSSM backward passes are replaced by this fused path, with a colsum fallback for bf16 and half-store cases. This removes many small kernel launches and one extra read of the gradient tensors. The cost is extra register pressure and VALU adds inside the MFMA loop, plus more template instantiations.

Result: no change. 30.31, median of 6 (+0.2%).

```diff
diff --git a/pydreamer_amd/csrc/common.h b/pydreamer_amd/csrc/common.h
--- a/pydreamer_amd/csrc/common.h
+++ b/pydreamer_amd/csrc/common.h
@@ -93,6 +93,7 @@
   int flags = 0;
   const int2* c_tab = nullptr; int sc_cout = 0, sc_wpitch = 0;
   int bias_mod = 0;
+  float* dbias = nullptr;
   const float* ln_g = nullptr; const float* ln_b = nullptr; float ln_eps = 1e-3f;
   const float* lnb_x = nullptr; int lnb_ldx = 0; const float* lnb_stats = nullptr;
   const float* eg_x = nullptr; int eg_ldx = 0; const float* eg_stats = nullptr; const float* eg_gamma = nullptr; const float* eg_beta = nullptr;
@@ -149,7 +150,8 @@
 int dm_gemm_skinny_try(const DmGemm& g, hipStream_t stream);
 int dm_gemm_pair_launch(const DmGemm& g0, const DmGemm& g1, void* ws, size_t ws_bytes, hipStream_t stream);
 
-int dm_colsum_launch(int rows, int n, const float* x, int ld, float* out, void* ws, size_t ws_bytes, hipStream_t st);
+int dm_colsum_launch(int rows, int n, const float* x, int ld, float* out, void* ws, size_t ws_bytes, hipStream_t st,
+                     int accum = 0);
 int dm_elu_fwd_launch(int rows, int n, const float* x, int ldx, float* y, int ldy, hipStream_t st);
 int dm_elu_bwd_launch(int rows, int n, const float* y, int ldy, const float* dy, int lddy, float* dx, int lddx,
                       hipStream_t st);
diff --git a/pydreamer_amd/csrc/conv.hip b/pydreamer_amd/csrc/conv.hip
--- a/pydreamer_amd/csrc/conv.hip
+++ b/pydreamer_amd/csrc/conv.hip
@@ -563,8 +563,8 @@
   }
   for (int l = 3; l >= 0; --l) {
     const int rows = (int)g.rows[l], co = g.cout[l], kd = (int)g.kdim[l];
-    DM_TRY(dm_colsum_launch(rows, co, G, co, gr->b[l], splitk, skb, st));
     if (l == 0 && g.direct0) {
+      DM_TRY(dm_colsum_launch(rows, co, G, co, gr->b[l], splitk, skb, st));
       DM_REQUIRE(image, DM_E_NULL, "conv_encoder_bwd: the direct layer-1 weight gradient reads the image");
       DM_REQUIRE(dm_enc_l1_wgrad_part_floats(g.N, g.d) <= xcmax, DM_E_WORKSPACE, "conv_encoder_bwd: partial buffer too small");
       DM_TRY(dm_enc_l1_wgrad_launch(g.N, g.d, shape_u8(shp) ? 1 : 0, image, G, dxcol, gr->w[0], splitk, skb, st));
@@ -574,6 +574,7 @@
     q.a_layout = 1; q.b_layout = 1;
     q.M = co; q.N = kd; q.K = rows;
     q.A = G; q.lda = co;
+    q.dbias = gr->b[l];
     if (l == 0) { q.B = a.xcol[0]; q.ldb = kd; }
     else {
       q.B = a.y[l - 1]; q.b_maj = a.rowoff[l]; q.b_min = a.koff[l];
@@ -976,12 +977,12 @@
     d.flags = DM_GEMM_ACCUM;
     DM_TRY(dm_gemm_launch(d, splitk, skb, st));
   }
-  DM_TRY(dm_colsum_launch(g.N, O, G, O, gr->b[0], splitk_w, skb, sw));
   {
     DmGemm q;
     q.a_layout = 1; q.b_layout = 1;
     q.M = O; q.N = g.F; q.K = g.N;
     q.A = G; q.lda = O;
+    q.dbias = gr->b[0];
     q.B = feat; q.ldb = ldf;
     q.C = gr->w[0]; q.ldc = g.F;
     DM_TRY(dm_gemm_launch(q, splitk_w, skb, sw));
diff --git a/pydreamer_amd/csrc/elementwise.hip b/pydreamer_amd/csrc/elementwise.hip
--- a/pydreamer_amd/csrc/elementwise.hip
+++ b/pydreamer_amd/csrc/elementwise.hip
@@ -190,7 +190,7 @@
 }
 
 __global__ void __launch_bounds__(256) colsum_final_kernel(int n, int chunks, int nq, const float* __restrict__ partial,
-                                                           float* __restrict__ out0, float* __restrict__ out1) {
+                                                           float* __restrict__ out0, float* __restrict__ out1, int accum) {
   __shared__ float red[8][32];
   const int cx = threadIdx.x & 31, cy = threadIdx.x >> 5;
   const int col = blockIdx.x * 32 + cx;
@@ -212,7 +212,8 @@
       float t = 0.f;
 #pragma unroll
       for (int k = 0; k < 8; ++k) t += red[k][cx];
-      (q == 0 ? out0 : out1)[col] = t;
+      float* o = (q == 0 ? out0 : out1) + col;
+      *o = accum ? *o + t : t;
     }
     __syncthreads();
   }
@@ -228,8 +229,8 @@
   return dm_cdiv(rows, *rows_per_chunk);
 }
 
-int dm_colsum_launch(int rows, int n, const float* x, int ld, float* out, void* ws, size_t ws_bytes, hipStream_t st) {
-  if (n <= 0) return DM_OK;
+int dm_colsum_launch(int rows, int n, const float* x, int ld, float* out, void* ws, size_t ws_bytes, hipStream_t st, int accum) {
+  if (n <= 0 || (rows <= 0 && accum)) return DM_OK;
   if (rows <= 0) {
     (void)hipMemsetAsync(out, 0, (size_t)n * sizeof(float), st);
     return DM_OK;
@@ -256,7 +257,7 @@
   }
   DM_LAUNCH_CHECK();
   hipLaunchKernelGGL(colsum_final_kernel, dim3(dm_cdiv(n, 32)), dim3(256), 0, st, n, chunks, 1, (const float*)ws, out,
-                     nullptr);
+                     nullptr, accum);
   DM_LAUNCH_CHECK();
   return DM_OK;
 }
@@ -334,7 +335,7 @@
                      ldy, stats, dy, lddy, (float*)ws);
   DM_LAUNCH_CHECK();
   hipLaunchKernelGGL(colsum_final_kernel, dim3(dm_cdiv(n, 32)), dim3(256), 0, st, n, chunks, 2, (const float*)ws, dgamma,
-                     dbeta);
+                     dbeta, 0);
   DM_LAUNCH_CHECK();
   return DM_OK;
 }
diff --git a/pydreamer_amd/csrc/gemm.hip b/pydreamer_amd/csrc/gemm.hip
--- a/pydreamer_amd/csrc/gemm.hip
+++ b/pydreamer_amd/csrc/gemm.hip
@@ -33,6 +33,7 @@
   int a_vec, b_vec;
   unsigned short* Ch;
   int use_dma;
+  float* dbias;
 };
 
 template <int ROWS, int LAYOUT, int NF4, bool GATHER, bool VEC, bool KSEQ = false>
@@ -283,10 +284,26 @@
   }
 }
 
+template <int BM, int WGM, int MB>
+__device__ __forceinline__ void gemm_dbias_write(const float (&bs)[MB], const GemmKArgs& g, const GemmItem& cur, int wm, int wn,
+                                                 int l31, int half) {
+  if (cur.n0 != 0 || wn != 0) return;
+#pragma unroll
+  for (int mb = 0; mb < MB; ++mb) {
+    const float s = bs[mb] + __shfl_xor(bs[mb], 32);
+    const int row = cur.m0 + wm * (BM / WGM) + mb * 32 + l31;
+    if (half == 0 && row < g.M) {
+      if (g.nsplit > 1) g.partial[(size_t)g.nsplit * g.M * g.N + (size_t)cur.split * g.M + row] = s;
+      else g.dbias[row] = (g.flags & DM_GEMM_ACCUM) ? g.dbias[row] + s : s;
+    }
+  }
+}
+
 template <int BM, int BN, int AL, int BL, bool VEC, bool GA = false, bool GB = false, int WGM = 2, int WGN = 2,
-          int BF = 0, bool SC = false>
+          int BF = 0, bool SC = false, bool DB = false>
 __global__ void __launch_bounds__(256) gemm_f32_kernel(const GemmKArgs g) {
   static_assert(WGM * WGN == 4 && BM % (32 * WGM) == 0 && BN % (32 * WGN) == 0, "wave grid must tile the block tile");
+  static_assert(!DB || (BF == 0 && AL == 1 && !GA && !SC), "the fused bias gradient is built for fp32 weight-gradient products");
   constexpr int BK = 32;
   constexpr int LDK = 36;
   constexpr int LDMA = BM + 4, LDMB = BN + 4;
@@ -317,6 +334,10 @@
 #pragma unroll
       for (int r = 0; r < 16; ++r) acc[i][j][r] = 0.f;
 
+  float bs[MB];
+#pragma unroll
+  for (int i = 0; i < MB; ++i) bs[i] = 0.f;
+
   float4 ra[A_F4], rb[B_F4];
   unsigned ma = 0u, mb_ = 0u;
   if (cur.nkt > 0) {
@@ -389,17 +410,24 @@
 #pragma unroll
           for (int nb = 0; nb < NB; ++nb)
             acc[mb][nb] = __builtin_amdgcn_mfma_f32_32x32x2f32(a[mb][j], b[nb][j], acc[mb][nb], 0, 0, 0);
+      if constexpr (DB)
+#pragma unroll
+        for (int mb = 0; mb < MB; ++mb)
+#pragma unroll
+          for (int j = 0; j < 4; ++j) bs[mb] += a[mb][j];
     }
     __syncthreads();
   }
 
+  if constexpr (DB) gemm_dbias_write<BM, WGM, MB>(bs, g, cur, wm, wn, l31, half);
   gemm_epilogue<BM, BN, WGM, WGN, SC, MB, NB>(acc, g, cur, wm, wn, l31, half,
                                               reinterpret_cast<unsigned short*>(smem) + wave * 32 * EPI_STAGE_LD);
 }
 
-template <int BM, int BN, int AL, int BL, bool GA, bool GB, int WGM, int WGN, bool SC, int NS>
+template <int BM, int BN, int AL, int BL, bool GA, bool GB, int WGM, int WGN, bool SC, int NS, bool DB = false>
 __global__ void __launch_bounds__(256) gemm_dma_kernel(const GemmKArgs g) {
   static_assert(WGM * WGN == 4 && BM % (32 * WGM) == 0 && BN % (32 * WGN) == 0, "wave grid must tile the block tile");
+  static_assert(!DB || (AL == 1 && !GA && !SC), "the fused bias gradient is built for weight-gradient products");
   static_assert(NS >= 2 && NS <= 3, "two or three LDS stages");
   constexpr int WM = BM / WGM, WN = BN / WGN;
   constexpr int MB = WM / 32, NB = WN / 32;
@@ -422,6 +450,9 @@
     for (int j = 0; j < NB; ++j)
 #pragma unroll
       for (int r = 0; r < 16; ++r) acc[i][j][r] = 0.f;
+  float bs[MB];
+#pragma unroll
+  for (int i = 0; i < MB; ++i) bs[i] = 0.f;
 
   if (cur.nkt > 0) {
     DmaOperand<BM, AL, GA> sa;
@@ -504,6 +535,11 @@
 #pragma unroll
             for (int nb = 0; nb < NB; ++nb)
               acc[mb][nb] = __builtin_amdgcn_mfma_f32_32x32x2f32(a[c][mb].get(j), b[c][nb].get(j), acc[mb][nb], 0, 0, 0);
+        if constexpr (DB)
+#pragma unroll
+          for (int mb = 0; mb < MB; ++mb)
+#pragma unroll
+            for (int j = 0; j < 4; ++j) bs[mb] += a[c][mb].get(j);
         __builtin_amdgcn_sched_barrier(0);
       }
       if ((GA || GB) && nt + 1 < cur.nkt) {
@@ -513,6 +549,7 @@
       if (++stage == NS) stage = 0;
     }
   }
+  if constexpr (DB) gemm_dbias_write<BM, WGM, MB>(bs, g, cur, wm, wn, l31, half);
   unsigned short* stg = nullptr;
   if (g.Ch) {
     __syncthreads();
@@ -880,20 +917,28 @@
 
 __global__ void __launch_bounds__(256) gemm_splitk_reduce_kernel(const GemmKArgs g) {
   const size_t total = (size_t)g.M * g.N;
-  for (size_t i = (size_t)blockIdx.x * 256 + threadIdx.x; i < total; i += (size_t)gridDim.x * 256) {
-    const int row = (int)(i / g.N);
-    const int col = (int)(i % g.N);
-    const float* __restrict__ pp = g.partial + i;
+  const size_t all = total + (g.dbias ? (size_t)g.M : 0);
+  for (size_t i = (size_t)blockIdx.x * 256 + threadIdx.x; i < all; i += (size_t)gridDim.x * 256) {
+    const bool isb = i >= total;
+    const float* __restrict__ pp = isb ? g.partial + (size_t)g.nsplit * total + (i - total) : g.partial + i;
+    const size_t stride = isb ? (size_t)g.M : total;
     float v = 0.f;
     int s = 0;
     for (; s + 8 <= g.nsplit; s += 8) {
       float t[8];
 #pragma unroll
-      for (int u = 0; u < 8; ++u) t[u] = pp[(size_t)(s + u) * total];
+      for (int u = 0; u < 8; ++u) t[u] = pp[(size_t)(s + u) * stride];
 #pragma unroll
       for (int u = 0; u < 8; ++u) v += t[u];
     }
-    for (; s < g.nsplit; ++s) v += pp[(size_t)s * total];
+    for (; s < g.nsplit; ++s) v += pp[(size_t)s * stride];
+    if (isb) {
+      float* d = g.dbias + (i - total);
+      *d = (g.flags & DM_GEMM_ACCUM) ? *d + v : v;
+      continue;
+    }
+    const int row = (int)(i / g.N);
+    const int col = (int)(i % g.N);
     if (g.row_zero && g.row_zero[row]) v = 0.f;
     if (g.bias) v += g.bias[g.bias_mod > 0 ? col % g.bias_mod : col];
     if (g.add) v += g.add[(size_t)row * g.ldadd + col];
@@ -1055,6 +1100,10 @@
   constexpr int NS = (BM + BN) * 128 * 3 <= 72 * 1024 ? 3 : 2;
   constexpr int LDS = NS * (BM + BN) * 128;
   constexpr int LDS2 = 2 * (BM + BN) * 128;
+  if (a.dbias) {
+    if (gather == 2) return dma_launch<gemm_dma_kernel<BM, BN, 1, 1, false, true, WGM, WGN, false, 2, true>>(LDS2, a, grid, stream);
+    return dma_launch<gemm_dma_kernel<BM, BN, 1, 1, false, false, WGM, WGN, false, NS, true>>(LDS, a, grid, stream);
+  }
   if (a.c_tab) {
     if (gather != 1 || al != 0 || bl != 0) return dm_fail(DM_E_SHAPE, "gemm: the scatter epilogue is built for a gathered A, layout (0,0), 16-byte loads");
     return dma_launch<gemm_dma_kernel<BM, BN, 0, 0, true, false, WGM, WGN, true, 2>>(LDS2, a, grid, stream);
@@ -1077,6 +1126,13 @@
 static int gemm_dispatch(const GemmKArgs& a, int al, int bl, int gather, dim3 grid, hipStream_t stream) {
   if constexpr (V && BF == 0) {
     if (a.use_dma) return gemm_dma_dispatch<BM, BN, WGM, WGN>(a, al, bl, gather, grid, stream);
+  }
+  if constexpr (BF == 0) {
+    if (a.dbias) {
+      if (gather == 2) hipLaunchKernelGGL((gemm_f32_kernel<BM, BN, 1, 1, V, false, true, WGM, WGN, 0, false, true>), grid, dim3(256), 0, stream, a);
+      else hipLaunchKernelGGL((gemm_f32_kernel<BM, BN, 1, 1, V, false, false, WGM, WGN, 0, false, true>), grid, dim3(256), 0, stream, a);
+      return DM_OK;
+    }
   }
   if (a.c_tab) {
     if (gather != 1 || al != 0 || bl != 0 || !V) return dm_fail(DM_E_SHAPE, "gemm: the scatter epilogue is built for a gathered A, layout (0,0), 16-byte loads");
@@ -1165,6 +1221,9 @@
              "gemm: gather tables must come in (major, minor) pairs");
   DM_REQUIRE(q.c_tab || q.ldc >= q.N, DM_E_SHAPE, "gemm: ldc %d < N %d", q.ldc, q.N);
   DM_REQUIRE(!q.add || q.ldadd >= q.N, DM_E_SHAPE, "gemm: ldadd %d < N %d", q.ldadd, q.N);
+  DM_REQUIRE(!q.dbias || (q.a_layout == 1 && q.b_layout == 1 && q.A && !q.a_maj && !q.c_tab && !q.row_zero && !q.add &&
+                          !q.mulref && !(q.flags & DM_GEMM_ELU)),
+             DM_E_SHAPE, "gemm: the fused bias gradient needs layouts (1,1), a dense fp32 A and no row_zero / add / mulref / ELU");
 
   {
     const int sk = (q.A_h || q.C_h) ? 0 : dm_gemm_skinny_try(q, stream);
@@ -1212,6 +1271,8 @@
   a.flags = q.flags;
   a.a_maj = q.a_maj; a.a_min = q.a_min; a.b_maj = q.b_maj; a.b_min = q.b_min;
   a.c_tab = q.c_tab; a.sc_cout = q.sc_cout; a.sc_wpitch = q.sc_wpitch; a.bias_mod = q.bias_mod;
+  const bool dbias_fused = q.dbias && !hstore && !q.bf16;
+  a.dbias = dbias_fused ? q.dbias : nullptr;
   DM_REQUIRE(!q.c_tab || (q.sc_cout > 0 && q.N % q.sc_cout == 0 && q.N / q.sc_cout == 4 && !q.add && !(q.flags & DM_GEMM_ACCUM)),
              DM_E_SHAPE, "gemm: scatter epilogue needs N = 4 * sc_cout, no addend, no accumulate");
   if (hstore) {
@@ -1230,7 +1291,7 @@
   if (max_split > ktiles / 2) max_split = ktiles / 2;
   if (max_split > 512) max_split = 512;
   {
-    const size_t per = (size_t)q.M * q.N * sizeof(float);
+    const size_t per = ((size_t)q.M * q.N + (dbias_fused ? (size_t)q.M : 0)) * sizeof(float);
     if (ws == nullptr || q.c_tab) max_split = 1;
     else if ((size_t)max_split * per > ws_bytes) max_split = (int)(ws_bytes / per);
   }
@@ -1372,12 +1433,13 @@
   prof_after(slot, stream);
   DM_LAUNCH_CHECK();
   if (nsplit > 1) {
-    const size_t total = (size_t)q.M * q.N;
+    const size_t total = (size_t)q.M * q.N + (a.dbias ? (size_t)q.M : 0);
     int blocks = dm_cdiv(total, 256);
     if (blocks > 2048) blocks = 2048;
     hipLaunchKernelGGL(gemm_splitk_reduce_kernel, dim3(blocks), dim3(256), 0, stream, a);
     DM_LAUNCH_CHECK();
   }
+  if (q.dbias && !dbias_fused) DM_TRY(dm_colsum_launch(q.K, q.M, q.A, q.lda, q.dbias, ws, ws_bytes, stream, (q.flags & DM_GEMM_ACCUM) ? 1 : 0));
   if (q.C_frag) {
     DM_REQUIRE(q.M <= 64 && !q.c_tab, DM_E_SHAPE, "gemm: a fragment-major copy of C needs M <= 64 (M=%d)", q.M);
     DM_TRY(dm_frag_pack_launch(q.M, q.N, q.C, q.ldc, q.C_frag, stream));
diff --git a/pydreamer_amd/csrc/mlp.hip b/pydreamer_amd/csrc/mlp.hip
--- a/pydreamer_amd/csrc/mlp.hip
+++ b/pydreamer_amd/csrc/mlp.hip
@@ -240,8 +240,8 @@
       q.A = dout; q.lda = out_dim;
       q.B = a.y[layers - 1]; q.ldb = hidden;
       q.C = g->w[layers]; q.ldc = hidden;
+      q.dbias = g->b[layers];
       DM_TRY(dm_gemm_launch(q, splitk, skb, st));
-      DM_TRY(dm_colsum_launch(rows, out_dim, dout, out_dim, g->b[layers], splitk, skb, st));
     }
     float* cur = dxp;
     float* other = dy;
@@ -292,8 +292,8 @@
     q.A = dout; q.lda = out_dim;
     q.B = a.y[layers - 1]; q.ldb = hidden;
     q.C = g->w[layers]; q.ldc = hidden;
+    q.dbias = g->b[layers];
     DM_TRY(dm_gemm_launch(q, splitk, skb, st));
-    DM_TRY(dm_colsum_launch(rows, out_dim, dout, out_dim, g->b[layers], splitk, skb, st));
     DmGemm d;
     d.a_layout = 0; d.b_layout = 1;
     d.M = rows; d.N = hidden; d.K = out_dim;
@@ -320,8 +320,8 @@
     q.A = dxp; q.lda = hidden;
     q.B = in; q.ldb = ldin;
     q.C = g->w[l]; q.ldc = kin;
+    q.dbias = g->b[l];
     DM_TRY(dm_gemm_launch(q, splitk, skb, st));
-    DM_TRY(dm_colsum_launch(rows, hidden, dxp, hidden, g->b[l], splitk, skb, st));
     if (l > 0 || dx) {
       DmGemm d;
       d.a_layout = 0; d.b_layout = 1;
diff --git a/pydreamer_amd/csrc/rssm.hip b/pydreamer_amd/csrc/rssm.hip
--- a/pydreamer_amd/csrc/rssm.hip
+++ b/pydreamer_amd/csrc/rssm.hip
@@ -105,7 +105,7 @@
   return dm_gemm_launch(q, sk, skb, st);
 }
 static int wgrad(hipStream_t st, void* sk, size_t skb, int rows, int nout, int kin, const float* dy, int lddy,
-                 const float* x, int ldx, float* dW, int accum = 0) {
+                 const float* x, int ldx, float* dW, int accum = 0, float* db = nullptr) {
   DmGemm q;
   q.a_layout = 1; q.b_layout = 1;
   q.M = nout; q.N = kin; q.K = rows;
@@ -113,6 +113,7 @@
   q.B = x; q.ldb = ldx;
   q.C = dW; q.ldc = kin;
   q.flags = accum ? DM_GEMM_ACCUM : 0;
+  q.dbias = db;
   return dm_gemm_launch(q, sk, skb, st);
 }
 static int dgrad(hipStream_t st, void* sk, size_t skb, int rows, int nout, int kin, const float* dy, int lddy,
@@ -403,12 +404,10 @@
   DM_TRY(norm_elu_bwd_dx(N, Hd, a.x3, Hd, a.prin, Hd, a.st3, p[DM_RSSM_PRIOR_G], dprin, Hd, dx3, Hd, st));
   DM_TRY(dgrad(st, sk, skb, N, Hd, D, dx3, Hd, p[DM_RSSM_PRIOR_H_W], dfeat, F, 1, nullptr));
   DM_TRY(dm_wgrad_side_fork(st, sw));
-  DM_TRY(wgrad(sw, sk_w, skb, N, ZP, Hd, dprior, ZP, a.prin, Hd, g[DM_RSSM_PRIOR_W]));
-  DM_TRY(dm_colsum_launch(N, ZP, dprior, ZP, g[DM_RSSM_PRIOR_OB], sk_w, skb, sw));
+  DM_TRY(wgrad(sw, sk_w, skb, N, ZP, Hd, dprior, ZP, a.prin, Hd, g[DM_RSSM_PRIOR_W], 0, g[DM_RSSM_PRIOR_OB]));
   DM_TRY(norm_elu_bwd_params(N, Hd, a.x3, Hd, a.prin, Hd, a.st3, dprin, Hd, g[DM_RSSM_PRIOR_G],
                                      g[DM_RSSM_PRIOR_B], sk_w, skb, sw));
-  DM_TRY(wgrad(sw, sk_w, skb, N, Hd, D, dx3, Hd, feat, F, g[DM_RSSM_PRIOR_H_W]));
-  DM_TRY(dm_colsum_launch(N, Hd, dx3, Hd, g[DM_RSSM_PRIOR_H_B], sk_w, skb, sw));
+  DM_TRY(wgrad(sw, sk_w, skb, N, Hd, D, dx3, Hd, feat, F, g[DM_RSSM_PRIOR_H_W], 0, g[DM_RSSM_PRIOR_H_B]));
 
   DM_TRY(transpose(st, p[DM_RSSM_POST_W], wt_post, ZP, Hd));
   DM_TRY(transpose(st, p[DM_RSSM_POST_H_W], wt_post_h, Hd, D));
@@ -467,12 +466,14 @@
       DM_TRY(norm_elu_bwd_dx(rows, Hd, a.x1 + c0 * Hd, Hd, a.za + c0 * Hd, Hd, a.st1 + c0 * 2, p[DM_RSSM_IN_G], dza + c0 * Hd, Hd,
                              dx1_w + c0 * Hd, Hd, sw));
     }
-    DM_TRY(wgrad(sw, sk_w, skb, rows, ZP, Hd, dpost + c0 * ZP, ZP, a.pin + c0 * Hd, Hd, g[DM_RSSM_POST_W], acc));
-    DM_TRY(wgrad(sw, sk_w, skb, rows, Hd, D, dx2s + c0 * Hd, Hd, feat + c0 * F, F, g[DM_RSSM_POST_H_W], acc));
+    DM_TRY(wgrad(sw, sk_w, skb, rows, ZP, Hd, dpost + c0 * ZP, ZP, a.pin + c0 * Hd, Hd, g[DM_RSSM_POST_W], acc, g[DM_RSSM_POST_OB]));
+    DM_TRY(wgrad(sw, sk_w, skb, rows, Hd, D, dx2s + c0 * Hd, Hd, feat + c0 * F, F, g[DM_RSSM_POST_H_W], acc, g[DM_RSSM_POST_H_B]));
     DM_TRY(wgrad(sw, sk_w, skb, rows, Hd, E, dx2s + c0 * Hd, Hd, embed + c0 * E, E, g[DM_RSSM_POST_E_W], acc));
-    DM_TRY(wgrad(sw, sk_w, skb, rows, 3 * D, Hd, dgi + c0 * 3 * D, 3 * D, a.za + c0 * Hd, Hd, g[DM_RSSM_GRU_WIH], acc));
-    DM_TRY(wgrad(sw, sk_w, skb, rows, 3 * D, D, dgh + c0 * 3 * D, 3 * D, a.hin + c0 * D, D, g[DM_RSSM_GRU_WHH], acc));
-    DM_TRY(wgrad(sw, sk_w, skb, rows, Hd, Z, dx1s + c0 * Hd, Hd, a.zin + c0 * Z, Z, g[DM_RSSM_Z_W], acc));
+    DM_TRY(wgrad(sw, sk_w, skb, rows, 3 * D, Hd, dgi + c0 * 3 * D, 3 * D, a.za + c0 * Hd, Hd, g[DM_RSSM_GRU_WIH], acc,
+                 kind == 0 ? g[DM_RSSM_GRU_BIH] : nullptr));
+    DM_TRY(wgrad(sw, sk_w, skb, rows, 3 * D, D, dgh + c0 * 3 * D, 3 * D, a.hin + c0 * D, D, g[DM_RSSM_GRU_WHH], acc,
+                 kind == 0 ? g[DM_RSSM_GRU_BHH] : nullptr));
+    DM_TRY(wgrad(sw, sk_w, skb, rows, Hd, Z, dx1s + c0 * Hd, Hd, a.zin + c0 * Z, Z, g[DM_RSSM_Z_W], acc, g[DM_RSSM_Z_B]));
     DM_TRY(wgrad(sw, sk_w, skb, rows, Hd, A, dx1s + c0 * Hd, Hd, action + c0 * A, A, g[DM_RSSM_A_W], acc));
     return DM_OK;
   };
@@ -595,13 +596,11 @@
   st = sw;
   sk = sk_w;
   if (stacked) DM_TRY(dm_wgrad_side_fork(st_main, sw));
-  DM_TRY(dm_colsum_launch(N, ZP, dpost, ZP, g[DM_RSSM_POST_OB], sk, skb, st));
   DM_TRY(norm_elu_bwd_params(N, Hd, a.x2, Hd, a.pin, Hd, a.st2, dpin, Hd, g[DM_RSSM_POST_G], g[DM_RSSM_POST_B],
                                      sk, skb, st));
-  DM_TRY(dm_colsum_launch(N, Hd, dx2s, Hd, g[DM_RSSM_POST_H_B], sk, skb, st));
   if (stacked) {
-    DM_TRY(wgrad(st, sk, skb, N, ZP, Hd, dpost, ZP, a.pin, Hd, g[DM_RSSM_POST_W]));
-    DM_TRY(wgrad(st, sk, skb, N, Hd, D, dx2, Hd, feat, F, g[DM_RSSM_POST_H_W]));
+    DM_TRY(wgrad(st, sk, skb, N, ZP, Hd, dpost, ZP, a.pin, Hd, g[DM_RSSM_POST_W], 0, g[DM_RSSM_POST_OB]));
+    DM_TRY(wgrad(st, sk, skb, N, Hd, D, dx2, Hd, feat, F, g[DM_RSSM_POST_H_W], 0, g[DM_RSSM_POST_H_B]));
     DM_TRY(wgrad(st, sk, skb, N, Hd, E, dx2, Hd, embed, E, g[DM_RSSM_POST_E_W]));
   }
   if (stacked) {
@@ -609,12 +608,10 @@
     for (int i = 0; i < gk.L; ++i) {
       const float* x = i == 0 ? a.za : feat + (size_t)(i - 1) * ls;
       const int ldx = i == 0 ? Hd : F, kin = i == 0 ? Hd : ls;
-      DM_TRY(wgrad(st, sk, skb, N, 3 * ls, kin, dgi + 3 * ls * i, 3 * D, x, ldx, gk.g_wih[i]));
-      DM_TRY(wgrad(st, sk, skb, N, 3 * ls, ls, dgh + 3 * ls * i, 3 * D, a.hin + i * ls, D, gk.g_whh[i]));
-      if (kind == 0) {
-        DM_TRY(dm_colsum_launch(N, 3 * ls, dgi + 3 * ls * i, 3 * D, gk.g_bih[i], sk, skb, st));
-        DM_TRY(dm_colsum_launch(N, 3 * ls, dgh + 3 * ls * i, 3 * D, gk.g_bhh[i], sk, skb, st));
-      } else {
+      DM_TRY(wgrad(st, sk, skb, N, 3 * ls, kin, dgi + 3 * ls * i, 3 * D, x, ldx, gk.g_wih[i], 0, kind == 0 ? gk.g_bih[i] : nullptr));
+      DM_TRY(wgrad(st, sk, skb, N, 3 * ls, ls, dgh + 3 * ls * i, 3 * D, a.hin + i * ls, D, gk.g_whh[i], 0,
+                   kind == 0 ? gk.g_bhh[i] : nullptr));
+      if (kind != 0) {
         DM_TRY(dm_gru_norm_param_grads_launch(kind, N, ls, a.gs + 3 * ls * i, a.gst + 6 * i, dgl + 3 * ls * i, lnpg, lnpb, st,
                                               3 * D, 6 * gk.L));
         const int parts = kind == 1 ? 3 : 1;
@@ -626,10 +623,7 @@
       }
     }
   }
-  if (stacked) {
-  } else if (kind == 0) {
-    DM_TRY(dm_colsum_launch(N, 3 * D, dgi, 3 * D, g[DM_RSSM_GRU_BIH], sk, skb, st));
-    DM_TRY(dm_colsum_launch(N, 3 * D, dgh, 3 * D, g[DM_RSSM_GRU_BHH], sk, skb, st));
+  if (stacked || kind == 0) {
   } else {
     DM_TRY(dm_gru_norm_param_grads_launch(kind, N, D, a.gs, a.gst, dgl, lnpg, lnpb, st));
     const int parts = kind == 1 ? 3 : 1;
@@ -645,9 +639,8 @@
   }
   DM_TRY(norm_elu_bwd_params(N, Hd, a.x1, Hd, a.za, Hd, a.st1, dza, Hd, g[DM_RSSM_IN_G], g[DM_RSSM_IN_B], sk, skb,
                                      st));
-  DM_TRY(dm_colsum_launch(N, Hd, dx1s, Hd, g[DM_RSSM_Z_B], sk, skb, st));
   if (stacked) {
-    DM_TRY(wgrad(st, sk, skb, N, Hd, Z, dx1, Hd, a.zin, Z, g[DM_RSSM_Z_W]));
+    DM_TRY(wgrad(st, sk, skb, N, Hd, Z, dx1, Hd, a.zin, Z, g[DM_RSSM_Z_W], 0, g[DM_RSSM_Z_B]));
     DM_TRY(wgrad(st, sk, skb, N, Hd, A, dx1, Hd, action, A, g[DM_RSSM_A_W]));
   }
   DM_TRY(dm_wgrad_side_mark(sw, st_main));
```
